# dfm/emcee

Hardware: AMD Instinct MI355X
Metric: walker-updates/sec (whole node), 64-dim correlated Gaussian, StretchMove a=2 (higher is better)
Workload: dtype f64

## Files before the change

emcee_amd/_lib.py:

```python
import ctypes as C
import os

import numpy as np

HERE = os.path.dirname(os.path.abspath(__file__))
LIB_PATH = os.path.join(HERE, "libemx.so")

TARGET_HOST, TARGET_ISO, TARGET_DIAG, TARGET_DENSE, TARGET_ROSENBROCK, TARGET_BOX, TARGET_CALLBACK = range(7)
TARGET_FUSED_USER = 8
TARGET_FUSED_PT = 9
TARGET_FUSED_ENSEMBLE = 10
MOVE_STRETCH, MOVE_DE, MOVE_SNOOKER, MOVE_GAUSS = range(4)
MOVE_WALK, MOVE_KDE = 5, 6
KDE_BW_SCOTT, KDE_BW_SILVERMAN, KDE_BW_SCALAR = range(3)
GAUSS_VECTOR, GAUSS_RANDOM, GAUSS_SEQUENTIAL = range(3)
RNG_INPUTS, RNG_MT19937, RNG_PHILOX = range(3)
EXCHANGE_ALLGATHER, EXCHANGE_PULL, EXCHANGE_DIRECT, EXCHANGE_LOGPROB, EXCHANGE_REPLAY = range(5)


class MoveDesc(C.Structure):
    _fields_ = [("kind", C.c_int32), ("nsplits", C.c_int32), ("randomize_split", C.c_int32), ("reserved", C.c_int32),
                ("a", C.c_double), ("sigma", C.c_double), ("g0", C.c_double), ("gammas", C.c_double)]


# ... 67 lines not shown
    "emx_snapshot_save": (C.c_int, [_P, C.c_int32]),
    "emx_snapshot_read": (C.c_int, [_P, C.c_int32, _P, _P]),
    "emx_snapshot_restore": (C.c_int, [_P, C.c_int32]),
    "emx_snapshot_free": (C.c_int, [_P, C.c_int32]),
    "emx_set_target": (C.c_int, [_P, C.c_int32, _P, _P, C.c_double]),
    "emx_set_target_callback": (C.c_int, [_P, DEVICE_LOG_PROB_FN, _P]),
    "emx_set_target_fused": (C.c_int, [_P, FUSED_ENSEMBLE_FN, _P]),
    "emx_set_target_fused_blobs": (C.c_int, [_P, FUSED_ENSEMBLE_BLOBS_FN, _P, C.c_int32]),
    "emx_set_target_fused_small": (C.c_int, [_P, FUSED_BATCH_FN]),
    "emx_set_target_fused_data": (C.c_int, [_P, FUSED_ENSEMBLE_DATA_FN, _P, C.c_int64]),
    "emx_small_fused_check": (C.c_int, [C.c_int64, C.c_int32, C.c_int32, C.POINTER(MoveDesc), C.c_int32, C.c_int32, C.c_char_p, C.c_int32]),
    "emx_small_fused_pays": (C.c_int, [C.c_int64, C.c_int32, C.c_int32]),
    "emx_small_info": (C.c_int, [_P, C.POINTER(C.c_int64)]),
    "emx_get_blobs": (C.c_int, [_P, _P, C.POINTER(C.c_int32)]),
    "emx_set_blobs": (C.c_int, [_P, _dp]),
    "emx_eval_log_prob_blobs": (C.c_int, [_P, _dp, C.c_int64, _dp, _dp]),
    "emx_snapshot_read_blobs": (C.c_int, [_P, C.c_int32, _dp]),
    "emx_eval_state_log_prob": (C.c_int, [_P]),
    "emx_eval_log_prob": (C.c_int, [_P, _dp, C.c_int64, _dp]),
    "emx_set_moves": (C.c_int, [_P, C.c_int32, C.POINTER(MoveDesc), _dp]),
    "emx_set_rng_mode": (C.c_int, [_P, C.c_int32]),
    "emx_rng_set_mt19937": (C.c_int, [_P, _u32p, C.c_int32, C.c_int32, C.c_double]),
    "emx_rng_get_mt19937": (C.c_int, [_P, _u32p, C.POINTER(C.c_int32), C.POINTER(C.c_int32), C.POINTER(C.c_double)]),
    "emx_rng_set_philox": (C.c_int, [_P, C.c_uint64, C.c_uint64]),
    "emx_rng_get_philox": (C.c_int, [_P, C.POINTER(C.c_uint64), C.POINTER(C.c_uint64)]),
    "emx_chain_config": (C.c_int, [_P, C.c_int64]),
    "emx_chain_reset": (C.c_int, [_P]),
    "emx_run": (C.c_int, [_P, C.c_int64, C.c_int32, C.c_int32]),
    "emx_iteration": (C.c_int, [_P, C.POINTER(C.c_int64), C.POINTER(C.c_int64)]),
    "emx_graph_state": (C.c_int, [_P, C.POINTER(C.c_int32), C.POINTER(C.c_int32)]),
    "emx_chain_read": (C.c_int, [_P, C.c_int32, C.c_int64, C.c_int64, C.c_int64, _dp]),
    "emx_accepted_counts": (C.c_int, [_P, _dp]),
    "emx_step_begin": (C.c_int, [_P, C.c_int32, C.POINTER(C.c_int32), C.POINTER(C.c_int32)]),
    "emx_step_begin_with": (C.c_int, [_P, C.c_int32, C.c_int32, C.POINTER(C.c_int32)]),
    "emx_accept_proposals": (C.c_int, [_P, C.c_int32, _dp, _dp, _dp]),
    "emx_halfstep": (C.c_int, [_P, C.c_int32]),
    "emx_propose": (C.c_int, [_P, C.c_int32, _P, _P, C.POINTER(C.c_int64)]),
    "emx_accept": (C.c_int, [_P, C.c_int32, _dp]),
    "emx_step_end": (C.c_int, [_P]),
    "emx_plan_set": (C.c_int, [_P, C.c_int32, _ip, _ip, _ip, _ip, _ip, _dp, _dp]),
    "emx_plan_get": (C.c_int, [_P, _ip, _ip, _ip, _ip, _ip, _dp, _dp]),
    "emx_set_shard": (C.c_int, [_P, C.c_int32, C.c_int32]),
    "emx_set_shard_buffers": (C.c_int, [_P, _P, _P, C.c_int64]),
    "emx_device_ptr": (C.c_int, [_P, C.c_int32, C.POINTER(_P), C.POINTER(C.c_int64)]),
    "emx_shard_slots": (C.c_int, [_P, C.c_int32, C.POINTER(C.c_int64), C.POINTER(C.c_int64), C.POINTER(C.c_int64)]),
    "emx_scatter_gathered": (C.c_int, [_P, C.c_int32]),
    "emx_set_move_scale": (C.c_int, [_P, C.c_int32, C.c_void_p, C.c_int32]),
    "emx_get_move": (C.c_int, [_P, C.c_int32, C.POINTER(MoveDesc)]),
    "emx_plan_set_noise": (C.c_int, [_P, _dp, C.c_double]),
    "emx_set_exchange": (C.c_int, [_P, C.c_int32]),
    "emx_exchange_layout": (C.c_int, [_P, C.POINTER(C.c_int64), C.POINTER(C.c_int64)]),
    "emx_set_exchange_buffers": (C.c_int, [_P, _P, C.c_int64, _P, C.c_int64]),
    "emx_own_walkers": (C.c_int, [_P, C.POINTER(C.c_int64), C.POINTER(C.c_int64)]),
    "emx_pull_prepare": (C.c_int, [_P, C.c_int32, C.POINTER(C.c_int64)]),
    "emx_pull_apply": (C.c_int, [_P, C.c_int32]),
    "emx_logprob_begin": (C.c_int, [_P, C.c_int32, C.POINTER(C.c_int64)]),
    "emx_logprob_finish": (C.c_int, [_P, C.c_int32]),
    "emx_replay_begin": (C.c_int, [_P, C.c_int32, C.POINTER(C.c_int64)]),
    "emx_replay_finish": (C.c_int, [_P, C.c_int32]),
    "emx_replay_exchange": (C.c_int, [_P, C.c_int32]),
    "emx_replica_pack": (C.c_int, [_P, C.POINTER(C.c_int64)]),
    "emx_replica_unpack": (C.c_int, [_P]),
    "emx_direct_export": (C.c_int, [_P, _u8p]),
    "emx_direct_import": (C.c_int, [_P, _u8p]),
    "emx_direct_attach": (C.c_int, [_P, C.POINTER(C.c_void_p), C.POINTER(C.c_void_p)]),
    "emx_direct_halfstep": (C.c_int, [_P, C.c_int32, C.c_int32]),
    "emx_fft_load": (C.c_int, [C.c_char_p]),
    "emx_autocorr": (C.c_int, [_P, C.c_int64, C.c_int64, C.c_double, _dp, _ip, C.POINTER(C.c_int64)]),
    "emx_walkers_independent": (C.c_int, [C.c_int32, _dp, C.c_int64, C.c_int32, C.POINTER(C.c_int32), C.POINTER(C.c_double)]),
    "emx_walkers_independent_resident": (C.c_int, [C.c_void_p, C.POINTER(C.c_int32), C.POINTER(C.c_double)]),
    "emx_host_pull_capacity": (C.c_int64, [C.c_int64, C.c_int32, C.c_int32, C.c_int32]),
    "emx_comm_load": (C.c_int, [C.c_char_p]),
    "emx_comm_get_unique_id": (C.c_int, [_u8p]),
    "emx_comm_init": (C.c_int, [_P, C.c_int32, C.c_int32, _u8p]),
    "emx_comm_destroy": (C.c_int, [_P]),
    "emx_comm_count": (C.c_int, [_P, C.POINTER(C.c_int32)]),
    "emx_pipeline_stats": (C.c_int, [_P, _dp, C.POINTER(C.c_int64), C.POINTER(C.c_int32)]),
    "emx_pipeline_handovers": (C.c_int, [_P, C.POINTER(C.c_int64), C.POINTER(C.c_int64)]),
    "emx_persist_info": (C.c_int, [_P, C.POINTER(C.c_int64)]),
    "emx_mtdev_info": (C.c_int, [_P, C.POINTER(C.c_int64)]),
    "emx_mtdev_debug": (C.c_int, [_P, C.c_int32, C.c_int64, C.c_void_p, C.c_int64]),
    "emx_mtdev_tok_stats": (C.c_int, [_P, C.POINTER(C.c_int64)]),
    "emx_persist_local_launches": (C.c_int, [_P, C.POINTER(C.c_int64)]),
    "emx_host_mt_jump": (C.c_int, [_u32p, C.c_uint64, C.c_int32, _u32p]),
    "emx_host_persist_shape": (C.c_int, [C.c_int64, C.c_int32, C.c_int32, C.POINTER(C.c_int32), C.POINTER(C.c_int32)]),
    "emx_timer_start": (C.c_int, [_P]),
    "emx_timer_stop": (C.c_int, [_P, C.POINTER(C.c_float)]),
    "emx_profile_enable": (C.c_int, [_P, C.c_int32]),
    "emx_profile_read": (C.c_int, [_P, _f32p, C.POINTER(C.c_int32)]),
    "emx_mt_create": (_P, [_u32p, C.c_int32, C.c_int32, C.c_double]),
    "emx_mt_destroy": (None, [_P]),
    "emx_mt_get_state": (None, [_P, _u32p, C.POINTER(C.c_int32), C.POINTER(C.c_int32), C.POINTER(C.c_double)]),
    "emx_mt_random_sample": (None, [_P, C.c_int64, _dp]),
    "emx_mt_randint": (None, [_P, C.c_uint64, C.c_int64, _i64p]),
    "emx_mt_randn": (None, [_P, C.c_int64, _dp]),
    "emx_mt_shuffle_labels": (None, [_P, C.c_int64, C.c_int32, _ip]),
    "emx_mt_choice_cdf": (C.c_int32, [_P, _dp, C.c_int32]),
    "emx_host_plan_mt": (C.c_int, [_P, C.c_int64, C.c_int32, C.POINTER(MoveDesc), _ip, _ip, _ip, _ip, _ip, _dp, _dp]),
    "emx_host_plan_mt_stream": (C.c_int, [_P, C.c_int64, C.c_int32, C.c_int32, C.POINTER(MoveDesc), _dp, C.c_int64, C.c_int32, C.c_int32,
                                          _P, _P, _P, _P, _P, _P, _P, C.POINTER(C.c_double)]),
    "emx_host_split_draws": (C.c_int, [_P, C.c_int64, C.POINTER(MoveDesc), _ip, _ip, C.c_int32, _ip, _ip, _ip, _dp]),
    "emx_host_plan_philox": (C.c_int, [C.c_uint64, C.c_uint64, C.c_int64, C.POINTER(MoveDesc), _ip, _ip, _ip, _ip, _ip, _dp, _dp]),
    "emx_host_walk_kde_draws": (C.c_int64, [C.c_uint64, C.c_uint64, C.c_int64, C.c_int32, C.POINTER(MoveDesc), C.c_int32, _P, _dp]),
    "emx_host_move_choice_philox": (C.c_int32, [C.c_uint64, C.c_uint64, _dp, C.c_int32]),
    "emx_batch_check": (C.c_int, [C.c_int64, C.c_int32, C.c_int32, C.c_int32, C.POINTER(MoveDesc), C.c_char_p, C.c_int32]),
    "emx_batch_create": (C.c_int, [C.c_int32, C.c_int32, C.c_int64, C.c_int32, C.POINTER(_P)]),
    "emx_batch_destroy": (C.c_int, [_P]),
    "emx_batch_last_error": (C.c_char_p, [_P]),
    "emx_batch_set_tuning": (C.c_int, [_P, C.c_char_p, C.c_int64]),
    "emx_batch_set_target": (C.c_int, [_P, C.c_int32, _P, _P, _P, C.c_int32]),
    "emx_batch_set_moves": (C.c_int, [_P, C.c_int32, C.POINTER(MoveDesc), _dp]),
    "emx_batch_set_move_scale": (C.c_int, [_P, C.c_int32, _dp, C.c_int32]),
    "emx_batch_get_move": (C.c_int, [_P, C.c_int32, C.POINTER(MoveDesc)]),
    "emx_batch_set_philox": (C.c_int, [_P, _u64p, C.c_uint64]),
    "emx_batch_get_philox": (C.c_int, [_P, _u64p, C.POINTER(C.c_uint64)]),
    "emx_batch_set_state": (C.c_int, [_P, _dp, _P]),
    "emx_batch_get_state": (C.c_int, [_P, _P, _P]),
    "emx_batch_eval_state_log_prob": (C.c_int, [_P]),
    "emx_batch_chain_config": (C.c_int, [_P, C.c_int64]),
    "emx_batch_run": (C.c_int, [_P, C.c_int64, C.c_int32, C.c_int32]),
    "emx_batch_iteration": (C.c_int, [_P, C.POINTER(C.c_int64), C.POINTER(C.c_int64)]),
    "emx_batch_chain_read": (C.c_int, [_P, C.c_int32, C.c_int32, C.c_int32, C.c_int64, C.c_int64, C.c_int64, _dp]),
    "emx_batch_accepted_counts": (C.c_int, [_P, _dp]),
    "emx_batch_status": (C.c_int, [_P, _u32p]),
    "emx_batch_launch_info": (C.c_int, [_P, C.POINTER(C.c_int32), C.POINTER(C.c_int32), C.POINTER(C.c_int64)]),
    "emx_set_batch_target_callback": (C.c_int, [_P, BATCH_LOG_PROB_FN, _P]),
    "emx_set_batch_target_fused": (C.c_int, [_P, FUSED_BATCH_FN, C.c_int32, _P]),
    "emx_pt_set_tempering": (C.c_int, [_P, C.c_int32, _dp, _P, _P]),
    "emx_set_batch_prior_callback": (C.c_int, [_P, BATCH_LOG_PROB_FN, _P]),
    "emx_pt_set_swap_every": (C.c_int, [_P, C.c_int64]),
    "emx_pt_swap": (C.c_int, [_P]),
    "emx_pt_swap_counts": (C.c_int, [_P, _u64p, _u64p]),
    "emx_pt_mean_loglike": (C.c_int, [_P, C.c_int64, C.c_int64, C.c_int64, _dp]),
    "emx_pt_set_state": (C.c_int, [_P, _dp, _dp, _dp]),
    "emx_pt_get_state": (C.c_int, [_P, _dp, _dp]),
    "emx_host_pt_swap_draws": (C.c_int, [C.c_uint64, C.c_uint64, C.c_int64, C.c_int32, _ip, _dp]),
    "emx_pt_set_adaptation": (C.c_int, [_P, C.c_int32, C.c_double, C.c_double]),
    "emx_pt_get_ladder": (C.c_int, [_P, _P, C.POINTER(C.c_int64)]),
    "emx_pt_set_ladder": (C.c_int, [_P, _dp, C.POINTER(C.c_int64)]),
    "emx_host_pt_adapt_ladder": (C.c_int, [_dp, _i64p, C.c_int32, C.c_int64, C.c_double, C.c_double, C.c_int64, _dp]),
    "emx_pt_set_target_fused": (C.c_int, [_P, PT_FUSED_FN, C.c_int32, _P]),
    "emx_pt_set_target_fused_data": (C.c_int, [_P, PT_FUSED_FN, C.c_int32, _P, _i64p]),
    "emx_pt_fused_check": (C.c_int, [C.c_int32, C.c_int64, C.c_int32, C.c_int32, C.POINTER(MoveDesc), C.c_char_p, C.c_int32]),
    "emx_autocorr_batch": (C.c_int, [_P, C.c_int32, C.c_int32, C.c_int64, C.c_int64, C.c_double, _dp, _ip, C.POINTER(C.c_int64)]),
    "emx_summary_batch": (C.c_int, [_P, C.c_int32, C.c_int32, C.c_int64, C.c_int64, C.c_int64, _P, _P, C.c_int32, _P, _P, _P, _P,
                                    C.POINTER(C.c_int64)]),
    "emx_summary": (C.c_int, [_P, C.c_int32, C.c_int64, C.c_int64, C.c_int64, _P, _P, C.c_int32, _P, _P, _P, _P, C.POINTER(C.c_int64)]),
    "emx_summary_info": (C.c_int, [_P, C.POINTER(C.c_int64), C.POINTER(C.c_int64), C.POINTER(C.c_int64)]),
    "emx_host_order_stats": (C.c_int, [_dp, C.c_int64, C.c_int64, C.c_int32, _i64p, _dp]),
    "emx_chain_minmax": (C.c_int, [_P, C.c_int32, C.c_int64, C.c_int64, C.c_int64, _P, _P, _P]),
    "emx_histograms": (C.c_int, [_P, C.c_int32, C.c_int64, C.c_int64, C.c_int64, _P, _P, _P, _P, _P, C.c_int64, _P, _P, _P,
                                 C.POINTER(C.c_int64)]),
    "emx_set_batch_target_fused_blobs": (C.c_int, [_P, FUSED_BATCH_FN, C.c_int32, _P, C.c_int32]),
    "emx_set_batch_target_fused_data": (C.c_int, [_P, FUSED_BATCH_DATA_FN, C.c_int32, _P, _i64p]),
    "emx_set_batch_target_callback_blobs": (C.c_int, [_P, BATCH_LOG_PROB_BLOBS_FN, _P, C.c_int32]),
    "emx_check_batch_blobs": (C.c_int, [C.c_int64, C.c_int32, C.c_int32, C.c_int32, C.POINTER(MoveDesc), C.c_int32, C.c_char_p, C.c_int32]),
    "emx_get_blobs_batch": (C.c_int, [_P, _P, C.POINTER(C.c_int32)]),
    "emx_summary_batch_plane": (C.c_int, [_P, C.c_int32, C.c_int32, C.c_int32, C.c_int64, C.c_int64, C.c_int64, _P, _P, C.c_int32, _P, _P,
                                          _P, _P, C.POINTER(C.c_int64)]),
    "emx_chain_minmax_batch": (C.c_int, [_P, C.c_int32, C.c_int32, C.c_int32, C.c_int64, C.c_int64, C.c_int64, _P, _P, _P]),
    "emx_histograms_batch": (C.c_int, [_P, C.c_int32, C.c_int32, C.c_int32, C.c_int64, C.c_int64, C.c_int64, _P, _P, C.c_int64, _P, _P, _P,
                                       C.c_int64, C.c_int64, _P, _P, _P, C.POINTER(C.c_int64)]),
    "emx_histograms_batch_info": (C.c_int, [_P, C.POINTER(C.c_int64)]),
    "emx_rhat_batch": (C.c_int, [_P, C.c_int32, C.c_int32, C.c_int32, C.c_int64, C.c_int64, C.c_int64, C.c_int32, _P, _P,
                                 C.POINTER(C.c_int64), C.POINTER(C.c_int64)]),
    "emx_rhat": (C.c_int, [_P, C.c_int64, C.c_int64, C.c_int64, C.c_int32, _P, _P, C.POINTER(C.c_int64), C.POINTER(C.c_int64)]),
# ... 42 lines not shown
```

emcee_amd/csrc/emx.hip:

```cpp
#include <hip/hip_runtime.h>

#include <dlfcn.h>

#include <algorithm>
#include <chrono>
#include <cmath>
#include <cstdint>
#include <cstdio>
#include <cstring>
#include <deque>
#include <mutex>
#include <string>
#include <type_traits>
#include <vector>

#include "../../include/emx.h"
#include "emx_fused_ensemble.hpp"
#include "emx_fused_ensemble_data.hpp"
#include "emx_internal.hpp"
#include "emx_kernels.hpp"
#include "emx_launch.hpp"
#include "emx_mtdev.hpp"
#include "emx_mtjump.hpp"
#include "emx_mtpipe.hpp"
// ... 255 lines not shown
    double* evalblobs = nullptr;
    double* blob_plane = nullptr;
    double* snap_blobs[NSNAPSHOT] = {};
    int snap_nb[NSNAPSHOT] = {};
    void* cb_user = nullptr;
    int target = EMX_TARGET_HOST;
    double *tp0 = nullptr, *tp1 = nullptr;
    double tscale = 1.0;
    int Dp = 0;
    std::vector<emx_move_desc> moves;
    std::vector<double> cdf;
    std::vector<double*> mscale;
    double* disp = nullptr;
    double* noise_host = nullptr;
    hipEvent_t noise_ev = nullptr;
    bool noise_busy = false;
    unsigned long long* dbg = nullptr;
    int64_t dbg_blocks = 0;
    struct BulkPlans {
        char* host = nullptr;
        char* dev = nullptr;
        size_t bytes = 0;
        hipEvent_t done = nullptr;
        bool busy = false;
    } bulk[2];
    int bulk_pos = 0;
    int64_t tune_small = 1;
    int64_t tune_gauss_materialize = 0;
    double gfac = 1.0;
    int rng_mode = EMX_RNG_PHILOX;
    MT19937Legacy mt;
    uint64_t ph_seed = 0, ph_step = 0;
    struct PlanSlot {
        int32_t *order = nullptr, *p0 = nullptr, *p1 = nullptr, *p2 = nullptr;
        double *s0 = nullptr, *uacc = nullptr, *logu = nullptr, *fac = nullptr;
        char* host = nullptr;
        hipEvent_t consumed = nullptr;
        hipEvent_t consumed_ref = nullptr;
        hipEvent_t uploaded = nullptr;
        hipEvent_t uploaded_ref = nullptr;
        unsigned last_seq = 0;
        int64_t fetch_step = -1;
        bool busy = false, host_written = false;
        int move_idx = 0;
        PipeStepInfo pinfo;
    } ring[PLAN_RING + MTDEV_SLOTS];
    MtPlanPipeline* pipe = nullptr;
    int64_t pipe_taken = 0;
    int pipe_ring0 = 0;
    int pipe_nsinks = PIPE_SINKS;
    std::deque<int64_t> pipe_uploads;
    bool pipe_defer = false;
    std::vector<std::pair<int64_t, int>> pipe_deferred;
    hipEvent_t pipe_batch_ev[8] = {};
    int pipe_batch_n = 0, pipe_cons_n = 0;
    unsigned long long* pipe_done = nullptr;
    unsigned* pipe_arrived = nullptr;
    hipStream_t up_stream = nullptr;
    int64_t tune_mt_device_finish = 1;
    int64_t tune_persist_exact_mix = 1;
    int64_t pipe_raw_steps = 0;
    int64_t tune_mt_pipeline = -1;
    MtDevProducer* mtdev = nullptr;
    int64_t mtdev_taken = 0;
    int64_t tune_persist_local = 1;
    int64_t tune_persist_exact_max = 32768;
    int64_t tune_persist_exact_regen_max = 131072;
    int64_t tune_persist_exact_steps = 16;
    int64_t tune_fetch_avoid = 1;
    int64_t tune_fetch_blocks = 64;
    bool pipe_fetch_local = false;
    int64_t tune_fetch_delay_us = 0;
    int64_t tune_persist_span = 1;
    int64_t tune_persist_mix = 1;
    int persist_mix_fits = -1;
    int64_t tune_persist_slab = 1;
    int64_t persist_slab_launches = 0;
    int64_t tune_persist_rows_late = 1;
    int64_t tune_persist_stagger = -1;
    int64_t tune_persist_max_halfsteps = PERSIST_MAX_ITERS;
    int64_t tune_mt_device_min_regen = 786432;
    int64_t tune_mt_regen_min = 16384;
    int64_t pipe_regen_steps = 0;
    int64_t tune_persist_odd = 1;
    int64_t tune_persist_slab_skew = 1;
    int64_t tune_persist_slab_local_max = 4096;
    int64_t call_steps = 1;
    int64_t tune_persist_exact = 1;
    int64_t tune_persist_valu = 1;
    int64_t tune_persist_local_max = 8192;
    int64_t tune_slab = 1;
    int64_t tune_slab_skew = 1;
    int64_t tune_mt_device = 1;
    int64_t tune_mt_device_min = 147456;
    int64_t tune_mt_lookahead = 2;
    int64_t tune_mt_tok_wshift = 11, tune_mt_tok_tail = 2048;
    int64_t mtdev_steps_total = 0, mtdev_starts = 0;
    bool mtdev_defer_release = false;
    int64_t mtdev_release_pending = -1;
    MtDevStats mtdev_stats_last;
    int ring_pos = 0;
    struct Prepared {
        int move, S, slot;
        bool lean;
        int gcol;
        uint64_t step;
        NativeArgs nat;
        double cursor_before;
    };
    std::deque<Prepared> prepared;
    int64_t prep_hint = 1;
    std::vector<uint8_t> labels_scratch;
    struct Cur {
        bool active = false;
        int move = 0, S = 2, slot = 0;
        bool store = false;
        bool native = false;
        bool lean = false;
        bool devplan = false;
        int gcol = 0;
        std::vector<int32_t> off;
        NativeArgs nat{};
    } cur;
    double *chain = nullptr, *chain_lp = nullptr;
    int64_t cap = 0, stored = 0, proposals = 0;
    EnsSummary* summary = nullptr;
    RhatScratch* rhat = nullptr;
    int64_t tune_summary_compact = 1;
    int64_t tune_hist_chunk_rows = 0;
    double *qout = nullptr, *fout = nullptr, *newlp = nullptr;
    double* tp1_full = nullptr;
    double *evalX = nullptr, *evallp = nullptr;
    double* wk_work = nullptr;
    int rank = 0, world = 1;
    double *sendbuf = nullptr, *gathered = nullptr;
    int64_t sendbuf_rows = 0, gathered_rows = 0;
    bool own_shard_bufs = false;
    void* comm = nullptr;
    int64_t send_doubles = 0, recv_doubles = 0;
    int exchange = EMX_EXCHANGE_ALLGATHER;
    PlanSlot cplan;
    int64_t cplan_rows = 0;
    int32_t* pull_counts = nullptr;
    int pull_parity = 0;
    int64_t pull_cap_armed = 0;
    double* pull_armed_buf = nullptr;
    int64_t pull_cap_cur = 0;
    int pull_split = -1;
    double* peerX[EMX_MAX_PEERS] = {};
    unsigned long long* peer_flags[EMX_MAX_PEERS] = {};
    bool peer_ipc_x[EMX_MAX_PEERS] = {}, peer_ipc_f[EMX_MAX_PEERS] = {};
    unsigned long long* my_flags = nullptr;
    bool peers_ready = false;
    PeerTable* peer_table = nullptr;
    unsigned long long direct_epoch = 0;
    int32_t* direct_counts = nullptr;
    bool direct_planned = false;
    int64_t tune_direct_timeout_ms = 5000;
    int32_t* replay_counts = nullptr;
    int replay_parity = 0;
    int replay_split = -1;
    int64_t replay_recv_off = 0;
    int64_t replay_buf = 0;
    int replay_push_parity = 0;
    double* launch_declp = nullptr;
    bool launch_push = false;
    bool replay_pushed = false;
    int64_t launch_push_off = 0;
    bool eval_check_bad = false;
    bool direct_dead = false;
    bool direct_first_barrier = false;
    struct GraphSlot {
        hipGraph_t graph = nullptr;
        hipGraphExec_t exec = nullptr;
        bool valid = false;
        int64_t spw = -1, wpb = -1, bpc = -1;
        int target = -1;
    } gslot[2];
    StepDesc* d_desc = nullptr;
    GraphCounters* d_ctr = nullptr;
    GraphCounters* h_ctr = nullptr;
    hipEvent_t thr_ev[4] = {nullptr, nullptr, nullptr, nullptr};
    int64_t tune_throttle = 64;
    bool graph_disabled = false;
    bool graph_warm = false;
    int64_t tune_graph = 0;
    int64_t tune_persist_gauss_wpb = 0;
    int64_t tune_persist_test_skew = 0;
    int64_t tune_persist = 1, tune_persist_timeout_ms = 2000, tune_persist_min_walkers = 512;
    int persist_wpb = 8;
    int64_t persist_launches = 0, persist_halfsteps = 0;
    struct PersistCapture {
        HalfStepArgs a;
        dim3 grid, block;
        size_t lds;
        int move, dpb, lean;
        bool dense, got;
    };
    PersistCapture* persist_cap = nullptr;
    unsigned* persist_bar = nullptr;
    unsigned* persist_started = nullptr;
    unsigned persist_lepoch = 0;
    unsigned persist_hepoch = 0;
    int64_t persist_local_launches = 0;
    unsigned* persist_ver = nullptr;
    unsigned persist_epoch = 0;
    unsigned persist_grid = 0;
    struct PersistLog {
        unsigned seq;
        uint64_t ph_step;
        int64_t i0, steps, stored0, proposals0;
        int32_t thin_by, store;
        int64_t pipe_step0 = -1;
        const void* pipe_id = nullptr;
    };
    std::deque<PersistLog> plog;
    unsigned persist_seq = 0;
    int64_t persist_recovered = 0;
    int8_t persist_fits[4] = {-1, -1, -1, -1};
    int64_t tune_replay_two_pass = 0;
    int64_t tune_full_plan = 0;
    int64_t tune_spw = 0, tune_bpc = 2, tune_wpb = 0, tune_ablate = 0, tune_dense_wide = 0;
    hipEvent_t ev0 = nullptr, ev1 = nullptr;
    std::vector<hipEvent_t> prof;
    int prof_max = 0, prof_n = 0;
    std::string err;
    emx_fused_ensemble_data_fn fused_data_fn = nullptr;
    int64_t fused_ndata = 0;
    int64_t tune_fused_data_rows = 0;
};

static void graph_invalidate(emx_ctx* c);
static void apply_env_tuning(emx_ctx* c);
static int pipe_stop(emx_ctx* c);
#define PIPE_STOP(ctx)                        \
    do {                                      \
        const int _rps = pipe_stop(ctx);      \
        if (_rps) return _rps;                \
    } while (0)
static void direct_detach(emx_ctx* c);
static int direct_ensure(emx_ctx* c);
static void exchange_free(emx_ctx* c);
static int replay_ensure(emx_ctx* c);
static int flags_ensure(emx_ctx* c);
static int persist_settle(emx_ctx* c);
static hipError_t wait_stream(hipStream_t s);

static void drop_prepared(emx_ctx* c) {
    for (auto it = c->prepared.rbegin(); it != c->prepared.rend(); ++it)
        if (it->move < (int)c->moves.size() && c->moves[it->move].kind == EMX_MOVE_GAUSS) c->moves[it->move].gammas = it->cursor_before;
    c->prepared.clear();
}

#define FAIL(ctx, code, ...)                         \
    do {                                             \
        char _b[512];                                \
        snprintf(_b, sizeof(_b), __VA_ARGS__);       \
        if (ctx) (ctx)->err = _b; else g_err = _b;   \
        return (code);                               \
    } while (0)

#define HIPOK(ctx, expr)                                                                          \
    do {                                                                                          \
        hipError_t _e = (expr);                                                                   \
        if (_e != hipSuccess) FAIL(ctx, -2, "%s failed: %s (%s:%d)", #expr, hipGetErrorString(_e), __FILE__, __LINE__); \
    } while (0)

#define NEED(ctx, cond, ...)               \
    do {                                   \
        if (!(cond)) FAIL(ctx, -1, __VA_ARGS__); \
    } while (0)

namespace {

int prefetch_depth_host(int G, int V, int CH, int move, bool dense);

inline int lean_kind(const HalfStepArgs& a, int G, int V, int CH, int move, bool dense) {
    const int WPW = 64 / G, PF = prefetch_depth_host(G, V, CH, move, dense);
    const int spw = (dense && PF * WPW < 16) ? 16 : PF * WPW;
    const bool common = !a.ablate && !a.desc && !a.sendbuf && !a.disp && !a.skew_sleep && (EMX_OPT_STAMPS || !a.dbg) && (a.target != TGT_NONE || !dense) &&
                        (!EMX_LEAN_FOLD_D || a.D == G * V * CH) && a.spw == spw && a.t_lo == 0;
    if (!common) return 0;
    if (a.npeer) return a.declp ? 0 : 2;
    if (a.declp) return 4;
    return a.t_hi_dev ? 3 : 1;
}

template <int MOVE>
hipError_t launch_valu(const Shape& sh, dim3 grid, dim3 block, hipStream_t st, const HalfStepArgs& a) {
    if constexpr (MOVE == MOVE_STRETCH) {
        if (sh.G == 8 && sh.V == 2 && sh.CH == 2) {
            const int lk = lean_kind(a, 8, 2, 2, MOVE, false);
            if (lk == 1) return launch_one<8, 2, 2, MOVE, 0, 1>(grid, block, 0, st, a);
            if (lk == 2 || lk == 3) return launch_one<8, 2, 2, MOVE, 0, 2>(grid, block, 0, st, a);
            if (lk == 4) return launch_one<8, 2, 2, MOVE, 0, 4>(grid, block, 0, st, a);
        }
        if (sh.G == 8 && sh.V == 2 && sh.CH == 4) {
            const int lk = lean_kind(a, 8, 2, 4, MOVE, false);
            if (lk == 2 || lk == 3) return launch_one<8, 2, 4, MOVE, 0, 2>(grid, block, 0, st, a);
        }
        if (sh.G == 64 && sh.V == 2 && sh.CH == 8) {
            const int lk = lean_kind(a, 64, 2, 8, MOVE, false);
            if (lk == 1) return launch_one<64, 2, 8, MOVE, 0, 1>(grid, block, 0, st, a);
            if (lk == 2 || lk == 3) return launch_one<64, 2, 8, MOVE, 0, 2>(grid, block, 0, st, a);
            if (lk == 4) return launch_one<64, 2, 8, MOVE, 0, 4>(grid, block, 0, st, a);
        }
    }
    if constexpr (MOVE != MOVE_EVAL) {
#define EMX_LEAN_CASE(g, v, c)                                                                         \
    if (sh.G == g && sh.V == v && sh.CH == c && lean_kind(a, g, v, c, MOVE, false) == 1)                \
        return launch_one<g, v, c, MOVE, 0, 1>(grid, block, 0, st, a);
        EMX_LEAN_CASE(4, 1, 1) EMX_LEAN_CASE(8, 1, 1) EMX_LEAN_CASE(8, 1, 2) EMX_LEAN_CASE(8, 1, 4) EMX_LEAN_CASE(16, 1, 4)
        EMX_LEAN_CASE(32, 1, 4) EMX_LEAN_CASE(64, 1, 4) EMX_LEAN_CASE(64, 1, 8) EMX_LEAN_CASE(4, 2, 1) EMX_LEAN_CASE(8, 2, 1)
        EMX_LEAN_CASE(8, 2, 4) EMX_LEAN_CASE(16, 2, 4) EMX_LEAN_CASE(32, 2, 4) EMX_LEAN_CASE(64, 2, 4)
        if constexpr (MOVE == MOVE_STRETCH || MOVE == MOVE_GAUSS) {
            EMX_LEAN_CASE(64, 1, 16) EMX_LEAN_CASE(64, 2, 16)
        }
        if constexpr (MOVE != MOVE_STRETCH) {
            EMX_LEAN_CASE(8, 2, 2) EMX_LEAN_CASE(64, 2, 8)
        }
#undef EMX_LEAN_CASE
    }
#define EMX_CASE(g, v, c) \
    if (sh.G == g && sh.V == v && sh.CH == c) return launch_one<g, v, c, MOVE, 0>(grid, block, 0, st, a);
    EMX_CASE(4, 1, 1) EMX_CASE(8, 1, 1) EMX_CASE(8, 1, 2) EMX_CASE(8, 1, 4) EMX_CASE(16, 1, 4) EMX_CASE(32, 1, 4)
    EMX_CASE(64, 1, 4) EMX_CASE(64, 1, 8)
    EMX_CASE(4, 2, 1) EMX_CASE(8, 2, 1) EMX_CASE(8, 2, 2) EMX_CASE(8, 2, 4) EMX_CASE(16, 2, 4) EMX_CASE(32, 2, 4)
    EMX_CASE(64, 2, 4) EMX_CASE(64, 2, 8)
    if constexpr (MOVE == MOVE_STRETCH || MOVE == MOVE_EVAL || MOVE == MOVE_GAUSS) {
        EMX_CASE(64, 1, 16) EMX_CASE(64, 2, 16)
    }
#undef EMX_CASE
    return hipErrorInvalidValue;
}
// ... 663 lines not shown
    c->cdf.assign(1, 1.0);
    apply_env_tuning(c);
    *out = c;
    return 0;
}

static void apply_env_tuning(emx_ctx* c) {
    const char* e = getenv("EMX_TUNE");
    if (!e || !*e) return;
    std::string s(e);
    size_t pos = 0;
    while (pos < s.size()) {
        size_t end = s.find(',', pos);
        if (end == std::string::npos) end = s.size();
        const std::string kv = s.substr(pos, end - pos);
        const size_t eq = kv.find('=');
        if (eq != std::string::npos) emx_set_tuning(c, kv.substr(0, eq).c_str(), atoll(kv.c_str() + eq + 1));
        pos = end + 1;
    }
}

int emx_destroy(emx_ctx* c) {
    if (!c) return 0;
    pipe_stop(c);
    c->plog.clear();
    hipSetDevice(c->device);
    if (c->stream) hipStreamSynchronize(c->stream);
    if (c->comm && g_rccl.CommDestroy) g_rccl.CommDestroy(c->comm), c->comm = nullptr;
    if (c->status_host) hipHostFree(c->status_host);
    if (c->xfer_host) hipHostFree(c->xfer_host);
    for (int k = 0; k < 2; ++k) {
        if (c->bounce[k]) hipHostFree(c->bounce[k]);
        if (c->bounce_ev[k]) hipEventDestroy(c->bounce_ev[k]);
    }
    void* ptrs[] = {c->X, c->lp, c->acc, c->acc_count, c->iota, c->qout, c->fout, c->newlp, c->evalX, c->wk_work,
                    c->evallp, c->tp0, c->tp1, c->tp1_full, c->chain, c->chain_lp, c->own_shard_bufs ? c->sendbuf : nullptr,
                    c->own_shard_bufs ? c->gathered : nullptr};
    for (void* p : ptrs)
        if (p) hipFree(p);
    for (double* s : c->snap)
        if (s) hipFree(s);
    for (double* s : c->snap_blobs)
        if (s) hipFree(s);
    for (double* s : {c->blobs, c->evalblobs, c->blob_plane})
        if (s) hipFree(s);
    emx_internal_ens_summary_release(c->summary);
    emx_internal_rhat_release(c->rhat);

    for (auto& s : c->ring) {
        if (s.order) hipFree(s.order);
        if (s.host) hipHostFree(s.host);
        if (s.uploaded) hipEventDestroy(s.uploaded);
        s.uploaded_ref = nullptr;
        if (s.consumed) hipEventDestroy(s.consumed);
    }
    for (auto& e : c->pipe_batch_ev)
        if (e) hipEventDestroy(e);
    if (c->pipe_done) hipHostFree(c->pipe_done);
    if (c->pipe_arrived) hipFree(c->pipe_arrived);
    for (auto& g : c->gslot) {
        if (g.exec) hipGraphExecDestroy(g.exec);
        if (g.graph) hipGraphDestroy(g.graph);
    }
    {
        auto& p = c->cplan;
        void* q[] = {p.order, p.p0, p.p1, p.p2, p.s0, p.uacc, p.logu, p.fac, c->pull_counts, c->replay_counts};
        for (void* x : q)
            if (x) hipFree(x);
    }
    for (double* q : c->mscale)
        if (q) hipFree(q);
    for (auto& bp : c->bulk) {
        if (bp.host) hipHostFree(bp.host);
        if (bp.dev) hipFree(bp.dev);
        if (bp.done) hipEventDestroy(bp.done);
    }
    if (c->disp) hipFree(c->disp);
    if (c->dbg) hipFree(c->dbg);
    if (c->noise_host) hipHostFree(c->noise_host);
    if (c->noise_ev) hipEventDestroy(c->noise_ev);
    if (c->persist_bar) hipFree(c->persist_bar);
    if (c->persist_started) hipHostFree(c->persist_started);
    if (c->persist_ver) hipFree(c->persist_ver);
    if (c->d_desc) hipFree(c->d_desc);
    if (c->d_ctr) hipFree(c->d_ctr);
    if (c->h_ctr) hipHostFree(c->h_ctr);
    for (auto e : c->thr_ev)
        if (e) hipEventDestroy(e);
    if (c->ev0) hipEventDestroy(c->ev0);
    if (c->ev1) hipEventDestroy(c->ev1);
    for (auto e : c->prof) hipEventDestroy(e);
    direct_detach(c);
    if (c->my_flags) hipFree(c->my_flags);
    if (c->peer_table) hipFree(c->peer_table);
    if (c->direct_counts) hipFree(c->direct_counts);
    if (c->up_stream) hipStreamDestroy(c->up_stream);
    if (c->own_stream) hipStreamDestroy(c->own_stream);
    delete c;
    return 0;
}

int emx_set_stream(emx_ctx* c, void* s) {
    NEED(c, c, "null ctx");
    HIPOK(c, hipStreamSynchronize(c->stream));
    c->stream = s ? (hipStream_t)s : c->own_stream;
    return 0;
}

static const bool g_spin_sync = !(getenv("EMX_SPIN_SYNC") && atoi(getenv("EMX_SPIN_SYNC")) == 0);

static hipError_t wait_stream(hipStream_t s) {
    if (g_spin_sync) {
        const auto t0 = std::chrono::steady_clock::now();
        for (int it = 0;; ++it) {
            const hipError_t e = hipStreamQuery(s);
            if (e != hipErrorNotReady) return e;
            if ((it & 63) == 63 && std::chrono::steady_clock::now() - t0 > std::chrono::milliseconds(2)) break;
        }
    }
    return hipStreamSynchronize(s);
}

static hipError_t wait_event(hipEvent_t ev) {
    if (g_spin_sync) {
        const auto t0 = std::chrono::steady_clock::now();
        for (int it = 0;; ++it) {
            const hipError_t e = hipEventQuery(ev);
            if (e != hipErrorNotReady) return e;
            if ((it & 63) == 63 && std::chrono::steady_clock::now() - t0 > std::chrono::milliseconds(2)) break;
        }
    }
    return hipEventSynchronize(ev);
}

int emx_sync(emx_ctx* c) {
    HIPOK(c, hipSetDevice(c->device));
    HIPOK(c, wait_stream(c->stream));
    return persist_settle(c);
}

int emx_status(emx_ctx* c, uint32_t* bits) {
    HIPOK(c, wait_stream(c->stream));
    {
        const int rcs = persist_settle(c);
        if (rcs) return rcs;
    }
    uint32_t b = 0;
    for (int k = 0; k < 6; ++k)
        if (__atomic_exchange_n(&c->status_host[k], 0u, __ATOMIC_ACQ_REL)) b |= 1u << k;
    if (b & ST_EXCHANGE_TIMEOUT) c->direct_dead = true;
    if (b & ST_EXCHANGE_TIMEOUT) c->persist_grid = 0;
    *bits = b;
    return 0;
}

int emx_set_tuning(emx_ctx* c, const char* key, int64_t v) {
    if (!strcmp(key, "spw")) {
        c->tune_spw = v;
        return 0;
    }
    if (!strcmp(key, "phase_clock")) {
        if (v && !c->dbg) {
            c->dbg_blocks = 4096;
            HIPOK(c, hipMalloc((void**)&c->dbg, (size_t)c->dbg_blocks * 16 * 8));
            HIPOK(c, hipMemset(c->dbg, 0, (size_t)c->dbg_blocks * 16 * 8));
        }
// ... 42 lines not shown
    if (!strcmp(key, "waves_per_block")) {
        c->tune_wpb = (v == 1 || v == 2 || v == 4 || v == 8) ? v : 0;
        return 0;
    }
    if (!strcmp(key, "dense_wide")) {
        c->tune_dense_wide = v == 2 ? 2 : (v ? 1 : 0);
        graph_invalidate(c);
        return 0;
    }
    if (!strcmp(key, "mt_device")) {
        PIPE_STOP(c);
        c->tune_mt_device = v < 0 ? 0 : (v > 2 ? 2 : v);
        return 0;
    }
    if (!strcmp(key, "mt_device_min_walkers")) {
        PIPE_STOP(c);
        c->tune_mt_device_min = v < 8192 ? 8192 : v;
        return 0;
    }
    if (!strcmp(key, "mt_tok_wshift") || !strcmp(key, "mt_tok_tail")) {
        PIPE_STOP(c);
        (key[7] == 'w' ? c->tune_mt_tok_wshift : c->tune_mt_tok_tail) = v;
        return 0;
    }
    if (!strcmp(key, "mt_device_lookahead")) {
        c->tune_mt_lookahead = v < 0 ? 0 : (v > 2 ? 2 : v);
        return 0;
    }
    if (!strcmp(key, "slab")) {
        c->tune_slab = v < 0 ? 0 : (v > 2 ? 2 : v);
        return 0;
    }
    if (!strcmp(key, "persist_exact_mix")) {
        PIPE_STOP(c);
        c->tune_persist_exact_mix = v ? 1 : 0;
        return 0;
    }
    if (!strcmp(key, "mt_device_finish")) {
        PIPE_STOP(c);
        c->tune_mt_device_finish = v ? 1 : 0;
        return 0;
    }
    if (!strcmp(key, "slab_skew")) {
        c->tune_slab_skew = v < 0 ? 0 : (v > 4 ? 4 : v);
        return 0;
    }
    if (!strcmp(key, "persist")) {
        c->tune_persist = v ? 1 : 0;
        return 0;
    }
    if (!strcmp(key, "persist_slab_skew")) {
        c->tune_persist_slab_skew = v < 0 ? 0 : (v > 4 ? 4 : v);
        return 0;
    }
    if (!strcmp(key, "persist_slab_local_max_walkers")) {
        c->tune_persist_slab_local_max = v;
        return 0;
    }
    if (!strcmp(key, "summary_compact")) {
        c->tune_summary_compact = v < 0 ? 0 : (v > 2 ? 2 : v);
        return 0;
    }
    if (!strcmp(key, "hist_chunk_rows")) {
        c->tune_hist_chunk_rows = v < 0 ? 0 : v;
        return 0;
    }
    if (!strcmp(key, "persist_odd")) {
        c->tune_persist_odd = v ? 1 : 0;
        return 0;
    }
    if (!strcmp(key, "persist_exact_regen_max_walkers")) {
        PIPE_STOP(c);
        c->tune_persist_exact_regen_max = v;
        return 0;
    }
    if (!strcmp(key, "mt_device_min_walkers_regen")) {
        PIPE_STOP(c);
        c->tune_mt_device_min_regen = v;
        return 0;
    }
    if (!strcmp(key, "mt_regen_min_walkers")) {
        PIPE_STOP(c);
        c->tune_mt_regen_min = v < 0 ? 0 : v;
        return 0;
    }
    if (!strcmp(key, "persist_rows_late")) {
        c->tune_persist_rows_late = v < 0 ? 0 : v > 2 ? 2 : v;
        return 0;
    }
    if (!strcmp(key, "persist_stagger")) {
        c->tune_persist_stagger = v < 0 ? -1 : v > 1279 ? 1279 : v;
        return 0;
    }
    if (!strcmp(key, "persist_max_halfsteps")) {
        c->tune_persist_max_halfsteps = v;
        return 0;
    }
    if (!strcmp(key, "persist_slab")) {
        c->tune_persist_slab = (v == 1 || v == 2) ? v : 0;
        return 0;
    }
    if (!strcmp(key, "persist_local")) {
        c->tune_persist_local = v ? 1 : 0;
        return 0;
    }
    if (!strcmp(key, "persist_exact")) {
        PIPE_STOP(c);
        c->tune_persist_exact = v ? 1 : 0;
        return 0;
    }
    if (!strcmp(key, "persist_exact_max_walkers")) {
        PIPE_STOP(c);
        c->tune_persist_exact_max = v;
        return 0;
    }
    if (!strcmp(key, "persist_exact_steps")) {
        c->tune_persist_exact_steps = std::max<int64_t>(1, std::min<int64_t>(v, 16));
        return 0;
    }
    if (!strcmp(key, "fetch_blocks")) {
        c->tune_fetch_blocks = std::max<int64_t>(0, std::min<int64_t>(v, 65536));
        return 0;
    }
    if (!strcmp(key, "fetch_avoid")) {
        c->tune_fetch_avoid = v ? 1 : 0;
        return 0;
    }
    if (!strcmp(key, "test_fetch_delay_us")) {
        c->tune_fetch_delay_us = std::max<int64_t>(0, std::min<int64_t>(v, 100000));
        return 0;
    }
    if (!strcmp(key, "persist_span")) {
        c->tune_persist_span = v ? 1 : 0;
        return 0;
    }
    if (!strcmp(key, "persist_mix")) {
        c->tune_persist_mix = v ? 1 : 0;
        return 0;
    }
    if (!strcmp(key, "persist_valu")) {
        c->tune_persist_valu = v ? 1 : 0;
        return 0;
    }
    if (!strcmp(key, "persist_local_max_walkers")) {
        c->tune_persist_local_max = v;
        return 0;
    }
    if (!strcmp(key, "persist_gauss_wpb")) {
        c->tune_persist_gauss_wpb = (v == 1 || v == 2 || v == 4 || v == 8) ? v : 0;
        return 0;
    }
    if (!strcmp(key, "persist_test_skew")) {
        c->tune_persist_test_skew = v;
        return 0;
    }
    if (!strcmp(key, "persist_timeout_ms")) {
        c->tune_persist_timeout_ms = v > 0 ? v : 2000;
        return 0;
    }
    if (!strcmp(key, "persist_min_walkers")) {
        c->tune_persist_min_walkers = v > 0 ? v : 2;
        return 0;
    }
    if (!strcmp(key, "replay_two_pass")) {
        c->tune_replay_two_pass = v ? 1 : 0;
        return 0;
// ... 991 lines not shown
    bool any_raw = false;
    int max_nseg = 0;
    F.N = (int32_t)c->N;
    F.D = c->D;
    F.n = (int)c->pipe_deferred.size();
    hipEvent_t waited = nullptr;
    for (int k = 0; k < F.n; ++k) {
        auto& s = c->ring[c->pipe_deferred[k].second];
        bool by_event = s.busy && s.consumed_ref != waited;
        if (s.busy && s.last_seq != 0u && c->persist_started && (int)(c->persist_seq - s.last_seq) > 0) {
            const double w0 = tr_now();
            const double limit = 2e6 * (double)std::max<int64_t>(1, c->tune_persist_timeout_ms);
            while ((int)(__atomic_load_n(c->persist_started, __ATOMIC_ACQUIRE) - s.last_seq) <= 0 && tr_now() - w0 < limit) {}
            if ((int)(__atomic_load_n(c->persist_started, __ATOMIC_ACQUIRE) - s.last_seq) > 0) by_event = false;
        }
        if (by_event) {
            HIPOK(c, hipStreamWaitEvent(c->up_stream, s.consumed_ref, 0));
            waited = s.consumed_ref;
        }
        F.host[k] = s.host;
        F.dev[k] = (char*)s.order;
        F.stretch[k] = c->moves[(size_t)std::max(0, s.move_idx)].kind == EMX_MOVE_STRETCH;
        F.peers[k] = !(F.stretch[k] && c->world == 1);
        const PipeStepInfo& pi = s.pinfo;
        F.kind[k] = pi.regen ? 2 : (pi.raw ? 1 : 0);
        F.nkey[k] = pi.regen ? pi.regen_nseg * 624 : 0;
        if (pi.raw) {
            any_raw = true;
            PlanRawArgs& R = RB.st[k];
            R.dev = (char*)s.order;
            R.a = c->moves[(size_t)std::max(0, s.move_idx)].a;
            R.N = (int32_t)c->N;
            R.D = c->D;
            R.S = pi.S;
            R.wr_words = pi.wr_ring;
            R.wr_p1 = pi.regen ? 1 : 0;
            for (int q = 0; q <= pi.S && q <= PLAN_RAW_SPLITS; ++q) R.off[q] = pi.off[q];
            c->pipe_raw_steps++;
        }
        if (pi.regen) {
            PlanRegenArgs& G = GB.st[k];
            G.dev = (char*)s.order;
            G.N = (int32_t)c->N;
            G.ns0 = pi.off[1] - pi.off[0];
            G.off = pi.regen_off;
            G.nseg = pi.regen_nseg;
            max_nseg = std::max(max_nseg, pi.regen_nseg);
            c->pipe_regen_steps++;
        }
    }
    F.delay_ticks = (unsigned)(c->tune_fetch_delay_us * 100);
    F.arrived = c->pipe_arrived;
    F.avoid_xcc = (c->persist_bar && c->tune_fetch_avoid) ? c->persist_bar + 9 * PERSIST_BAR_STRIDE + 4 : nullptr;
    F.host_done = c->pipe_done;
    F.done_value = (unsigned long long)(c->pipe_deferred.back().first + 1);
    F.pieces_x = (int32_t)((c->N + 255) / 256);
    unsigned nwg = (unsigned)F.pieces_x * (unsigned)F.n;
    if (!c->pipe_fetch_local && c->tune_fetch_blocks > 0) nwg = std::min<unsigned>(nwg, (unsigned)c->tune_fetch_blocks);
    hipLaunchKernelGGL(k_plan_fetch, dim3(nwg), dim3(256), 0, c->up_stream, F);
    if (max_nseg > 0) hipLaunchKernelGGL(k_plan_regen_batch, dim3((unsigned)max_nseg, (unsigned)F.n), dim3(256), 0, c->up_stream, GB);
    if (any_raw) hipLaunchKernelGGL(k_plan_raw_batch, dim3((unsigned)F.pieces_x, (unsigned)F.n), dim3(256), 0, c->up_stream, RB);
    HIPOK(c, hipGetLastError());
    hipEvent_t& ev = c->pipe_batch_ev[c->pipe_batch_n & 3];
    if (!ev) HIPOK(c, hipEventCreateWithFlags(&ev, hipEventDisableTiming));
    c->pipe_batch_n++;
    HIPOK(c, hipEventRecord(ev, c->up_stream));
    HIPOK(c, hipStreamWaitEvent(c->stream, ev, 0));
    for (auto& d : c->pipe_deferred) {
        c->ring[d.second].uploaded_ref = ev;
    }
    c->pipe_deferred.clear();
    return 0;
}

int emx_step_begin(emx_ctx* c, int32_t store, int32_t* move_out, int32_t* S_out) {
    return step_begin_impl(c, store, -1, move_out, S_out);
}

int emx_step_begin_with(emx_ctx* c, int32_t store, int32_t move_index, int32_t* S_out) {
    NEED(c, move_index >= 0 && move_index < (int)c->moves.size(), "bad move index");
    return step_begin_impl(c, store, move_index, nullptr, S_out);
}

static int native_prepare_batch(emx_ctx* c, uint64_t first_step, int nb, int forced_move, hipStream_t st) {
    const int nm = (int)c->moves.size();
    NativeBatchArgs B{};
    B.N = (int32_t)c->N;
    B.D = c->D;
    B.nb = nb;
    B.lean = (c->target != EMX_TARGET_HOST && c->world == 1 && !c->sendbuf && !c->comm && !c->tune_full_plan) ? 1 : 0;
    B.ablate = (int32_t)(c->tune_ablate >> 8);
    bool only_stretch = true;
    for (int b = 0; b < nb; ++b) {
        const uint64_t step = first_step + (uint64_t)b;
        const int mi = forced_move >= 0 ? forced_move : philox_move_choice(c->ph_seed, step, c->cdf.data(), nm);
        const emx_move_desc& m = c->moves[mi];
        only_stretch = only_stretch && m.kind == EMX_MOVE_STRETCH;
        emx_ctx::PlanSlot* ps;
        int rc = acquire_slot(c, &ps, false);
        if (rc) return rc;
        emx_ctx::Prepared pr{};
        pr.move = mi;
        pr.S = m.nsplits;
        pr.slot = c->ring_pos;
        pr.step = step;
        pr.nat.seed = c->ph_seed;
        pr.nat.step = step;
        pr.nat.pk = make_perm_key((uint64_t)c->N, c->ph_seed, step);
        pr.cursor_before = m.gammas;
        pr.lean = B.lean != 0;
        if (m.kind == EMX_MOVE_GAUSS) {
            B.gmode[b] = m.reserved;
            B.gcol[b] = (int32_t)((int64_t)m.gammas % c->D);
            pr.gcol = B.gcol[b];
            if (m.reserved == EMX_GAUSS_SEQUENTIAL) c->moves[mi].gammas = (double)(((int64_t)m.gammas + 1) % c->D);
        }
        c->prepared.push_back(pr);
        B.nat[b] = pr.nat;
        B.order[b] = ps->order;
        B.p0[b] = ps->p0;
        B.p1[b] = ps->p1;
        B.p2[b] = ps->p2;
        B.s0[b] = ps->s0;
        B.uacc[b] = ps->uacc;
        B.logu[b] = ps->logu;
        B.fac[b] = ps->fac;
        B.a[b] = m.a;
        B.sigma[b] = m.sigma;
        B.g0[b] = m.g0;
        B.move[b] = m.kind;
        B.S[b] = m.nsplits;
    }
    if (only_stretch && B.lean && !B.ablate && !B.desc)
        hipLaunchKernelGGL(k_native_plan_batch_stretch, dim3((unsigned)((c->N + 255) / 256), (unsigned)nb), dim3(256), 0, st, B);
    else
        hipLaunchKernelGGL(k_native_plan_batch, dim3((unsigned)((c->N + 255) / 256), (unsigned)nb), dim3(256), 0, st, B);
    HIPOK(c, hipGetLastError());
    return 0;
}

static int step_begin_impl(emx_ctx* c, int32_t store, int32_t forced_move, int32_t* move_out, int32_t* S_out) {
    HIPOK(c, hipSetDevice(c->device));
    NEED(c, !c->cur.active, "emx_step_begin: previous step not ended");
    if (store) NEED(c, c->stored < c->cap, "chain capacity exhausted (call emx_chain_config)");
    auto& cur = c->cur;
    cur.store = store != 0;
    cur.native = false;
    cur.devplan = false;
    const int nm = (int)c->moves.size();
    const bool devp = forced_move < 0 && mtdev_eligible(c);
    if (c->mtdev && !devp) {
        const int rcm = mtdev_stop(c);
        if (rcm) return rcm;
    }
    if (c->pipe && (devp || forced_move >= 0 || !pipe_eligible(c))) PIPE_STOP(c);
    if (devp) {
        if (!c->mtdev) {
            int rc0 = mtdev_start(c);
            if (rc0) return rc0;
        }
        int rc = mtdev_take(c);
        if (rc) return rc;
    } else if (c->rng_mode == EMX_RNG_MT19937 && forced_move < 0 && (c->pipe || ((c->N >= 8192 || persist_exact_ok(c)) && pipe_eligible(c)))) {
        if (!c->pipe) {
            int rc0 = pipe_start(c);
            if (rc0) return rc0;
        }
        int rc = pipe_take(c);
        if (rc) return rc;
    } else if (c->rng_mode == EMX_RNG_MT19937) {
        cur.move = forced_move >= 0 ? forced_move : c->mt.choice_cdf(c->cdf.data(), nm);
        const emx_move_desc& mv = c->moves[cur.move];
        NEED(c, !is_walk_kde(mv.kind), "WalkMove / KDEMove steps run on the device in the Philox rng mode only");
        cur.S = mv.nsplits;
        NEED(c, c->N >= 2 && (mv.kind != EMX_MOVE_DE || c->N - (c->N + cur.S - 1) / cur.S >= 2),
             "complement too small for this move");
        emx_ctx::PlanSlot* ps;
        int rc = acquire_slot(c, &ps, true);
        if (rc) return rc;
        cur.slot = c->ring_pos;
        cur.off.assign(cur.S + 1, 0);
        const size_t N = (size_t)c->N;
        const HostPlan hp(ps->host, N);
        if (mv.kind == EMX_MOVE_GAUSS) {
            if (!c->noise_host) {
                HIPOK(c, hipHostMalloc((void**)&c->noise_host, N * (size_t)c->D * 8, hipHostMallocDefault));
                HIPOK(c, hipEventCreateWithFlags(&c->noise_ev, hipEventDisableTiming));
            }
            if (c->noise_busy) {
                HIPOK(c, hipEventSynchronize(c->noise_ev));
                c->noise_busy = false;
            }
            const double f = make_exact_gauss(c->mt, c->N, c->D, mv, c->moves[cur.move].gammas, cur.off.data(), hp.order, hp.p0,
                                              hp.p1, hp.p2, hp.s0, hp.uacc, c->noise_host);
            rc = upload_plan(c, *ps);
            if (rc) return rc;
            rc = gauss_upload_normals(c, cur.move, c->noise_host, f, true);
            if (rc) return rc;
        } else {
            rc = make_exact_plan(c->mt, c->N, c->D, mv, c->labels_scratch, cur.off.data(), hp.order, hp.p0, hp.p1, hp.p2, hp.s0,
                                 hp.uacc);
            NEED(c, rc == 0, "plan generation failed");
            rc = upload_plan(c, *ps);
            if (rc) return rc;
        }
    } else if (c->rng_mode == EMX_RNG_PHILOX) {
        if (forced_move >= 0) drop_prepared(c);
        if (!c->prepared.empty() && c->prepared.front().step != c->ph_step) drop_prepared(c);
        if (c->prepared.empty()) {
            int64_t nbw = forced_move >= 0 ? 1 : c->prep_hint;
            const int nb = (int)std::max<int64_t>(1, std::min<int64_t>(nbw, NATIVE_BATCH_MAX));
            const int rc = native_prepare_batch(c, c->ph_step, nb, forced_move, c->stream);
            if (rc) return rc;
        }
        const emx_ctx::Prepared pr = c->prepared.front();
        c->prepared.pop_front();
        cur.move = pr.move;
        cur.S = pr.S;
        cur.native = true;
        cur.lean = pr.lean;
        cur.gcol = pr.gcol;
        cur.nat = pr.nat;
        cur.slot = pr.slot;
        cur.off.assign(cur.S + 1, 0);
        for (int s = 0; s < cur.S; ++s) cur.off[s + 1] = cur.off[s] + (int32_t)((c->N - s + cur.S - 1) / cur.S);
        if (c->moves[cur.move].kind == EMX_MOVE_GAUSS) {
            int rc = gauss_native_disp(c, cur.move, pr.step, c->ring[pr.slot].p0);
            if (rc) return rc;
        }
    } else {
        cur.move = -1;
        cur.S = 0;
        cur.slot = -1;
    }
    cur.active = true;
    if (move_out) *move_out = cur.move;
    if (S_out) *S_out = cur.S;
    return 0;
}

static int complete_lean_plan(emx_ctx* c) {
    auto& cur = c->cur;
    if (!cur.active || !cur.native || !cur.lean) return 0;
    NEED(c, cur.move >= 0 && cur.slot >= 0, "no plan available");
    auto& ps = c->ring[cur.slot];
    const emx_move_desc& m = c->moves[cur.move];
    NativeBatchArgs B{};
    B.N = (int32_t)c->N;
    B.D = c->D;
    B.nb = 1;
    B.lean = 0;
    B.nat[0] = cur.nat;
    B.order[0] = ps.order;
    B.p0[0] = ps.p0;
    B.p1[0] = ps.p1;
    B.p2[0] = ps.p2;
    B.s0[0] = ps.s0;
    B.uacc[0] = ps.uacc;
    B.logu[0] = ps.logu;
    B.fac[0] = ps.fac;
    B.a[0] = m.a;
    B.sigma[0] = m.sigma;
    B.g0[0] = m.g0;
    B.move[0] = m.kind;
    B.S[0] = m.nsplits;
    if (m.kind == EMX_MOVE_GAUSS) {
        B.gmode[0] = m.reserved;
        B.gcol[0] = cur.gcol;
    }
    hipLaunchKernelGGL(k_native_plan_batch, dim3((unsigned)((c->N + 255) / 256), 1u), dim3(256), 0, c->stream, B);
    HIPOK(c, hipGetLastError());
    cur.lean = false;
    return 0;
}

int emx_plan_set(emx_ctx* c, int32_t move_index, const int32_t* off, const int32_t* order, const int32_t* p0,
                 const int32_t* p1, const int32_t* p2, const double* s0, const double* uacc) {
    NEED(c, c->cur.active, "emx_plan_set outside a step");
    NEED(c, move_index >= 0 && move_index < (int)c->moves.size(), "bad move index");
    NEED(c, !is_walk_kde(c->moves[move_index].kind), "WalkMove / KDEMove steps run on the device in the Philox rng mode only");
    auto& cur = c->cur;
    cur.move = move_index;
    cur.S = c->moves[move_index].nsplits;
    cur.native = false;
    cur.off.assign(off, off + cur.S + 1);
    NEED(c, cur.off[0] == 0 && cur.off[cur.S] == c->N, "plan offsets must cover all walkers");
    emx_ctx::PlanSlot* ps;
    int rc = acquire_slot(c, &ps, true);
    if (rc) return rc;
    cur.slot = c->ring_pos;
    const size_t N = (size_t)c->N;
    const HostPlan hp(ps->host, N);
    memcpy(hp.order, order, N * 4);
    memcpy(hp.p0, p0, N * 4);
    memcpy(hp.p1, p1 ? p1 : order, N * 4);
    memcpy(hp.p2, p2 ? p2 : order, N * 4);
    if (s0) memcpy(hp.s0, s0, N * 8); else memset(hp.s0, 0, N * 8);
    memcpy(hp.uacc, uacc, N * 8);
    return upload_plan(c, *ps);
}

int emx_plan_get(emx_ctx* c, int32_t* off, int32_t* order, int32_t* p0, int32_t* p1, int32_t* p2, double* s0,
                 double* uacc) {
    NEED(c, c->cur.active, "emx_plan_get outside a step");
    auto& cur = c->cur;
    const size_t N = (size_t)c->N;
    memcpy(off, cur.off.data(), (cur.S + 1) * 4);
    if (cur.native) {
        NEED(c, cur.slot >= 0, "no plan available");
        auto& ps = c->ring[cur.slot];
        {
            const int rcl = complete_lean_plan(c);
            if (rcl) return rcl;
        }
        HIPOK(c, hipMemcpyAsync(order, ps.order, N * 4, hipMemcpyDeviceToHost, c->stream));
        HIPOK(c, hipMemcpyAsync(p0, ps.p0, N * 4, hipMemcpyDeviceToHost, c->stream));
        HIPOK(c, hipMemcpyAsync(p1, ps.p1, N * 4, hipMemcpyDeviceToHost, c->stream));
        HIPOK(c, hipMemcpyAsync(p2, ps.p2, N * 4, hipMemcpyDeviceToHost, c->stream));
        HIPOK(c, hipMemcpyAsync(s0, ps.s0, N * 8, hipMemcpyDeviceToHost, c->stream));
        HIPOK(c, hipMemcpyAsync(uacc, ps.uacc, N * 8, hipMemcpyDeviceToHost, c->stream));
        HIPOK(c, hipStreamSynchronize(c->stream));
        return 0;
    }
    NEED(c, cur.slot >= 0, "no plan available");
    auto& ps = c->ring[cur.slot];
    if (cur.devplan) {
        HIPOK(c, hipMemcpyAsync(order, ps.order, N * 4, hipMemcpyDeviceToHost, c->stream));
        HIPOK(c, hipMemcpyAsync(p0, ps.p0, N * 4, hipMemcpyDeviceToHost, c->stream));
        HIPOK(c, hipMemcpyAsync(s0, ps.s0, N * 8, hipMemcpyDeviceToHost, c->stream));
        HIPOK(c, hipMemcpyAsync(uacc, ps.uacc, N * 8, hipMemcpyDeviceToHost, c->stream));
        HIPOK(c, hipStreamSynchronize(c->stream));
        memcpy(p1, order, N * 4);
        memcpy(p2, order, N * 4);
        return 0;
    }
    const HostPlan hp(ps.host, N);
    memcpy(order, hp.order, N * 4);
    memcpy(p0, hp.p0, N * 4);
    if (cur.move >= 0 && c->moves[cur.move].kind == EMX_MOVE_STRETCH) {
        memcpy(p1, hp.order, N * 4);
        memcpy(p2, hp.order, N * 4);
    } else {
        memcpy(p1, hp.p1, N * 4);
        memcpy(p2, hp.p2, N * 4);
    }
    memcpy(s0, hp.s0, N * 8);
    memcpy(uacc, hp.uacc, N * 8);
    return 0;
}

int emx_plan_set_noise(emx_ctx* c, const double* normals, double factor) {
    HIPOK(c, hipSetDevice(c->device));
    auto& cur = c->cur;
    NEED(c, cur.active && cur.move >= 0 && c->moves[cur.move].kind == EMX_MOVE_GAUSS,
         "emx_plan_set_noise follows emx_plan_set of a Gaussian move");
// ... 606 lines not shown
    if (persist_local_ok(c, m)) return true;
    if (c->target != EMX_TARGET_DENSE_GAUSS) return persist_valu_wide_ok(c, m);
    const int wpb = persist_shape(c, m.nsplits);
    return wpb != 0 && persist_grid_fits(c, m, wpb);
}

static bool persist_mix_member(const emx_move_desc& m) {
    return (m.kind == EMX_MOVE_DE && m.nsplits == 2) || (m.kind == EMX_MOVE_SNOOKER && m.nsplits == 4);
}
static bool persist_mix_local(const emx_ctx* c) {
    for (const auto& m : c->moves)
        if (persist_mix_member(m) && !persist_local_ok(c, m)) return false;
    return persist_shape_local_of(c->N, 2, c->num_cu) != 0;
}
static bool persist_mix_ok(const emx_ctx* cc) {
    emx_ctx* c = const_cast<emx_ctx*>(cc);
    if (!c->tune_persist_mix || c->target != EMX_TARGET_DENSE_GAUSS || c->Dp > 64 || (c->D & 1)) return false;
    if (c->rng_mode != EMX_RNG_PHILOX && !(c->rng_mode == EMX_RNG_MT19937 && persist_exact_ok(c))) return false;
    bool de = false, sn = false;
    for (const auto& m : c->moves) {
        if (!persist_mix_member(m)) continue;
        if (!persist_move_ok(c, m)) return false;
        de = de || m.kind == EMX_MOVE_DE;
        sn = sn || m.kind == EMX_MOVE_SNOOKER;
    }
    if (!de || !sn || (c->N % 64) != 0) return false;
    if (persist_mix_local(c)) return true;
    const int wpb = persist_shape(c, 2);
    if (wpb == 0) return false;
    if (c->persist_mix_fits < 0) {
        int per_cu = 0;
        const hipError_t e = persist_mix_occupancy(c->Dp / 16, 64 * wpb, dense_lds_bytes(c->Dp, wpb), &per_cu);
        c->persist_mix_fits = (e != hipSuccess || (int64_t)per_cu * c->num_cu >= c->N / 2 / 16 / wpb) ? 1 : 0;
    }
    return c->persist_mix_fits != 0;
}

static bool persist_exact_ok(const emx_ctx* c) {
    if (small_eligible(c) && c->call_steps < 4) return false;
    {
        const bool dense = c->target == EMX_TARGET_DENSE_GAUSS && (c->Dp <= 64 || persist_slab_ok(c)) && !dense_is_wide(c);
        bool valu = c->target == EMX_TARGET_ISO_GAUSS || c->target == EMX_TARGET_DIAG_GAUSS || c->target == EMX_TARGET_ROSENBROCK || c->target == EMX_TARGET_BOX;
        if (valu) {
            const Shape sh = pick_shape(c->D, c->D);
            valu = persist_valu_shape(sh);
        }
        if (!dense && !valu) return false;
    }
    if (!(c->rng_mode == EMX_RNG_MT19937 && c->tune_persist_exact != 0 && !c->moves.empty() && c->tune_mt_pipeline != 0 &&
          c->N >= c->tune_persist_min_walkers && !mtdev_eligible(c) &&
          MtPlanPipeline::supports((int32_t)c->moves.size(), c->moves.data())))
        return false;
    if (c->moves.size() > 1 && !c->tune_persist_exact_mix) return false;
    for (const auto& m : c->moves) {
        const bool known = ((m.kind == EMX_MOVE_STRETCH || m.kind == EMX_MOVE_DE) && m.nsplits == 2) || (m.kind == EMX_MOVE_SNOOKER && m.nsplits == 4);
        if (!known && c->moves.size() > 1) return false;
        if (persist_local_ok(c, m)) continue;
        const int64_t nmax = (regen_ctx_ok(c) && m.kind == EMX_MOVE_STRETCH) ? std::max(c->tune_persist_exact_max, c->tune_persist_exact_regen_max) : c->tune_persist_exact_max;
        if (c->N > nmax || persist_shape(c, m.nsplits) == 0) return false;
        if (!(c->target == EMX_TARGET_DENSE_GAUSS || persist_valu_wide_ok(c, m))) return false;
    }
    return true;
}

static bool persist_wanted(const emx_ctx* c) {
    if (!c->tune_persist) return false;
    if (!(c->rng_mode == EMX_RNG_PHILOX || persist_exact_ok(c)) || c->world != 1 || c->comm || c->sendbuf || c->peers_ready || c->moves.empty()) return false;
    if (c->target != EMX_TARGET_DENSE_GAUSS || dense_is_wide(c) || (c->Dp > 64 && !persist_slab_ok(c))) return false;
    if (c->tune_ablate || (c->dbg && !EMX_OPT_STAMPS) || c->tune_spw || c->tune_wpb || c->tune_graph) return false;
    if (c->N < c->tune_persist_min_walkers) return false;
    bool any = false;
    for (const auto& m : c->moves) {
        if (is_walk_kde(m.kind)) return false;
        any = any || persist_move_ok(c, m);
    }
    if (!any) return false;
    if (c->Dp > 64) return true;
    const Shape sh = pick_shape(c->D, c->Dp);
    const int dpb = c->Dp / 16;
    if (sh.V == 1) return c->tune_persist_odd != 0 && (dpb <= 2 ? (sh.G == 8 && sh.CH == 2 * dpb) : (sh.G == 16 && sh.CH == 4));
    return sh.G == 8 && sh.V == 2 && sh.CH == (dpb == 1 ? 1 : dpb == 2 ? 2 : 4);
}

static bool persist_valu_wanted(const emx_ctx* c) {
    if (!c->tune_persist || !c->tune_persist_local || !c->tune_persist_valu) return false;
    if (!(c->rng_mode == EMX_RNG_PHILOX || persist_exact_ok(c)) || c->world != 1 || c->comm || c->sendbuf || c->peers_ready || c->moves.empty()) return false;
    if (c->target != EMX_TARGET_ISO_GAUSS && c->target != EMX_TARGET_DIAG_GAUSS && c->target != EMX_TARGET_ROSENBROCK && c->target != EMX_TARGET_BOX)
        return false;
    if (c->tune_ablate || c->dbg || c->tune_spw || c->tune_wpb || c->tune_graph) return false;
    if (c->N < c->tune_persist_min_walkers) return false;
    const Shape sh = pick_shape(c->D, c->D);
    if (!persist_valu_shape(sh)) return false;
    bool any = false;
    for (const auto& m : c->moves) {
        if (is_walk_kde(m.kind)) return false;
        any = any || persist_local_ok(c, m) || persist_valu_wide_ok(c, m);
    }
    return any;
}

static bool persist_gauss_wanted(const emx_ctx* c) {
    if (!c->tune_persist || c->tune_gauss_materialize) return false;
    if (c->rng_mode != EMX_RNG_PHILOX || c->world != 1 || c->comm || c->sendbuf || c->peers_ready || c->moves.size() != 1) return false;
    if (c->moves[0].kind != EMX_MOVE_GAUSS) return false;
    if (c->target != EMX_TARGET_DENSE_GAUSS || c->Dp > 64 || dense_is_wide(c)) return false;
    if (c->tune_ablate || c->dbg || c->tune_spw || c->tune_wpb || c->tune_graph) return false;
    if (c->N < c->tune_persist_min_walkers || (c->N % 16) != 0) return false;
    const Shape sh = pick_shape(c->D, c->Dp);
    const int dpb = c->Dp / 16;
    return sh.G == 8 && sh.V == 2 && sh.CH == (dpb == 1 ? 1 : dpb == 2 ? 2 : 4);
}

static int run_persist_gauss(emx_ctx* c, int64_t i0, int64_t total, int32_t thin_by, int32_t store, int64_t* done) {
    *done = 0;
    const int64_t tiles = c->N / 16;
    int wpb = c->tune_persist_gauss_wpb > 0 ? (int)c->tune_persist_gauss_wpb : 4;
    while (wpb > 1 && (tiles % wpb) != 0) wpb >>= 1;
    c->persist_wpb = wpb;
    PersistGaussArgs P{};
    emx_ctx::PersistCapture cap{};
    int64_t steps = 0;
    while (i0 + steps < total && steps < PERSIST_GAUSS_MAX_STEPS) {
        if (steps > 0 && c->prepared.empty()) break;
        c->prep_hint = NATIVE_BATCH_MAX;
        const int st = store && ((i0 + steps + 1) % thin_by == 0);
        int mvi, S;
        int rc = emx_step_begin(c, st, &mvi, &S);
        if (rc) return rc;
        cap.got = false;
        c->persist_cap = &cap;
        rc = do_halfstep(c, 0, c->target);
        c->persist_cap = nullptr;
        if (!rc && (S != 1 || !cap.dense || cap.move != MOVE_GAUSS || cap.a.disp || cap.dpb != c->Dp / 16)) {
            c->err = "persistent Gaussian steps: launch shape not eligible";
            rc = -1;
        }
        if (rc) {
            c->cur.active = false;
            return rc;
        }
        if (steps == 0) P.base = cap.a;
        PersistGaussStep& G = P.st[steps];
        G.p0 = cap.a.p0;
        G.logu = cap.a.logu;
        G.chain = cap.a.chain;
        G.chain_lp = cap.a.chain_lp;
        G.gstep = cap.a.gstep;
        G.gfac = cap.a.gfac;
        rc = emx_step_end(c);
        if (rc) return rc;
        ++steps;
    }
    P.nsteps = (int32_t)steps;
    const dim3 grid((unsigned)(tiles / wpb)), block(64u * (unsigned)wpb);
    const size_t lds = dense_lds_bytes(c->Dp, wpb);
    hipEvent_t e0 = nullptr, e1 = nullptr;
    const bool prof = c->prof_max > 0 && c->prof_n < c->prof_max;
    if (prof) {
        e0 = c->prof[2 * c->prof_n];
        e1 = c->prof[2 * c->prof_n + 1];
        HIPOK(c, hipEventRecord(e0, c->stream));
    }
    const hipError_t e = launch_hot_persist_gauss(c->Dp / 16, grid, block, lds, c->stream, P);
    if (e != hipSuccess) FAIL(c, -2, "persistent Gaussian launch failed: %s", hipGetErrorString(e));
    if (prof) {
        HIPOK(c, hipEventRecord(e1, c->stream));
        c->prof_n++;
    }
    c->persist_launches++;
    c->persist_halfsteps += steps;
    *done = steps;
    return 0;
}

static std::mutex g_persist_mu;
static hipEvent_t g_persist_ev[MAX_DEVICES] = {};
static const emx_ctx* g_persist_last[MAX_DEVICES] = {};

static int run_persist(emx_ctx* c, int64_t i0, int64_t total, int32_t thin_by, int32_t store, int64_t* done) {
    *done = 0;
    if (__atomic_load_n(&c->status_host[3], __ATOMIC_ACQUIRE)) {
        const int rcs = persist_settle(c);
        if (rcs) return rcs;
        if (__atomic_load_n(&c->status_host[3], __ATOMIC_ACQUIRE)) {
            c->persist_grid = 0;
            FAIL(c, -8, "persistent kernel: a device-wide barrier timed out in the middle of a launch; read emx_status, "
                        "or turn the persistent path off with tuning \"persist\" = 0");
        }
        return 0;
    }
    if (c->plog.size() >= 4096) {
        if (hipStreamQuery(c->stream) == hipSuccess && !__atomic_load_n(&c->status_host[3], __ATOMIC_ACQUIRE)) {
            c->plog.clear();
        } else if (c->plog.size() >= 65536) {
            const int rcs = persist_settle(c);
            if (rcs) return rcs;
        }
    }
    if (!c->persist_bar) {
        HIPOK(c, hipMalloc((void**)&c->persist_bar, PERSIST_BAR_WORDS * sizeof(unsigned)));
        HIPOK(c, hipHostMalloc((void**)&c->persist_started, 64, hipHostMallocDefault));
        *c->persist_started = 0u;
        HIPOK(c, hipMemsetAsync(c->persist_bar, 0, PERSIST_BAR_WORDS * sizeof(unsigned), c->stream));
        c->persist_epoch = 0;
    }
    if (!c->persist_ver) {
        HIPOK(c, hipMalloc((void**)&c->persist_ver, (size_t)c->N * 4));
        HIPOK(c, hipMemsetAsync(c->persist_ver, 0, (size_t)c->N * 4, c->stream));
    }
    PersistArgs P{};
    emx_ctx::PersistCapture cap{};
    dim3 grid, block;
    size_t lds = 0;
    int n = 0;
    int64_t steps = 0;
    const bool mtmode = c->rng_mode == EMX_RNG_MT19937;
    const bool devp = mtmode && mtdev_eligible(c);
    std::vector<int> used_slots;
    c->pipe_defer = mtmode && !devp;
    struct Undefer2 {
        emx_ctx* c;
        ~Undefer2() { c->pipe_defer = false; }
    } undefer2{c};
    c->mtdev_defer_release = devp;
    c->mtdev_release_pending = -1;
    struct Undefer {
        emx_ctx* c;
        ~Undefer() { c->mtdev_defer_release = false; }
    } undefer{c};
    emx_ctx::PersistLog lg{};
    lg.ph_step = c->ph_step;
    lg.i0 = i0;
    lg.stored0 = c->stored;
    lg.proposals0 = c->proposals;
    lg.thin_by = thin_by;
    lg.store = store;
    if (mtmode && !devp) {
        lg.pipe_step0 = c->pipe ? c->pipe_taken : 0;
        lg.pipe_id = c->pipe;
    }
    int launch_move = -1;
    int launch_S = 2;
    bool launch_local = false;
    bool launch_mix = false;
    double launch_gammas = 0.0;
    int batches_touched = (!mtmode && !c->prepared.empty() && c->prepared.front().step == c->ph_step) ? 1 : 0;
    while (i0 + steps < total) {
        if (!mtmode && (c->prepared.empty() || c->prepared.front().step != c->ph_step)) {
            if (batches_touched >= 2) break;
            ++batches_touched;
        }
        int next_move = -1;
        if (steps > 0 && !mtmode)
            next_move = !c->prepared.empty() ? c->prepared.front().move : philox_move_choice(c->ph_seed, c->ph_step, c->cdf.data(), (int)c->moves.size());
        if (steps > 0 && mtmode && !devp && c->moves.size() > 1) {
            PipeStepInfo peek;
            if (!c->pipe || !c->pipe->wait_ready(c->pipe_taken, peek, pipe_poll, c))
                FAIL(c, -7, "exact-mode plan pipeline stopped before step %lld", (long long)c->pipe_taken);
            next_move = peek.move;
        }
        int need = launch_S;
        if (launch_mix && next_move >= 0) need = c->moves[next_move].nsplits;
        if (n + need > (int)std::min<int64_t>(PERSIST_MAX_ITERS, std::max<int64_t>(4, c->tune_persist_max_halfsteps))) break;
        if (devp) {
            if (steps > 0 && c->mtdev && c->mtdev_taken % MTDEV_BATCH == 0) break;
        } else if (mtmode) {
            if (steps >= std::min<int64_t>(c->tune_persist_exact_steps, c->pipe_nsinks / 2)) break;
            if (steps > 0 && next_move >= 0) {
                if (!launch_mix && c->moves[next_move].kind != launch_move) break;
                if (!launch_mix && launch_move == EMX_MOVE_SNOOKER && c->moves[next_move].gammas != launch_gammas) break;
                if (launch_mix && !persist_mix_member(c->moves[next_move])) break;
                if (!persist_move_ok(c, c->moves[next_move])) break;
            }
        } else {
            if (steps > 0 && c->prepared.empty() && !c->tune_persist_span) break;
            if (steps > 0 && !launch_mix && c->moves[next_move].kind != launch_move) break;
            if (steps > 0 && !launch_mix && launch_move == EMX_MOVE_SNOOKER && c->moves[next_move].gammas != launch_gammas) break;
            if (steps > 0 && launch_mix && !persist_mix_member(c->moves[next_move])) break;
            if (steps > 0 && !persist_move_ok(c, c->moves[next_move])) break;
        }
        c->prep_hint = NATIVE_BATCH_MAX;
        const int st = store && ((i0 + steps + 1) % thin_by == 0);
        int mvi, S;
        int rc = emx_step_begin(c, st, &mvi, &S);
        if (rc) return rc;
        if (launch_move < 0) {
            launch_move = c->moves[mvi].kind;
            launch_gammas = c->moves[mvi].gammas;
            launch_S = S;
            launch_local = persist_local_ok(c, c->moves[mvi]);
            c->persist_wpb = launch_local ? persist_shape_local_of(c->N, S, c->num_cu) : persist_shape(c, S);
            if (persist_mix_ok(c) && (launch_move == EMX_MOVE_DE || launch_move == EMX_MOVE_SNOOKER)) {
                launch_mix = true;
                launch_local = persist_mix_local(c);
                c->persist_wpb = launch_local ? persist_shape_local_of(c->N, 2, c->num_cu) : persist_shape(c, 2);
            }
        }
        for (int s = 0; s < S; ++s) {
            cap.got = false;
            c->persist_cap = &cap;
            rc = do_halfstep(c, s, c->target);
            c->persist_cap = nullptr;
            const bool valu = c->target != EMX_TARGET_DENSE_GAUSS;
            const bool move_ok = launch_mix ? (cap.move == MOVE_DE || cap.move == MOVE_SNOOKER) : cap.move == launch_move;
            if (!rc && (!cap.got || cap.dense == valu || (!valu && cap.dpb != c->Dp / 16) || !move_ok ||
                        (int)cap.block.x != 64 * c->persist_wpb || (valu && !launch_local && !persist_valu_wide_ok(c, c->moves[mvi])))) {
                c->err = "persistent half-steps: launch shape not eligible";
                rc = -1;
            }
            if (rc) {
                c->cur.active = false;
                return rc;
            }
            if (n == 0) {
                P.base = cap.a;
                grid = cap.grid;
                block = cap.block;
                lds = cap.lds;
            }
            PersistIter& I = P.it[n++];
            {
                const char* blk = reinterpret_cast<const char*>(cap.a.order);
                const size_t NN = (size_t)c->N;
                NEED(c, (const void*)cap.a.p0 == (const void*)(blk + NN * 4) && (const void*)cap.a.s0 == (const void*)(blk + NN * 8) &&
                            (const void*)cap.a.p1 == (const void*)(blk + NN * 24) && (const void*)cap.a.p2 == (const void*)(blk + NN * 28) &&
                            (const void*)cap.a.logu == (const void*)(blk + NN * 32) && (const void*)cap.a.fac == (const void*)(blk + NN * 40),
                     "persistent half-steps: the plan slot is not one block in the expected layout");
                I.plan = blk;
            }
            I.chain = cap.a.chain;
            I.chain_lp = cap.a.chain_lp;
            I.pos0 = cap.a.pos0;
            I.split = cap.a.split;
            I.kind = cap.move;
            I.gammas = cap.a.gammas;
            I.shift = (launch_mix && S == 4) ? 1 : 0;
        }
        if (mtmode && !devp && c->cur.slot >= 0) used_slots.push_back(c->cur.slot);
        rc = emx_step_end(c);
        if (rc) return rc;
        ++steps;
    }
    if (mtmode && !devp) {
        c->pipe_fetch_local = launch_local;
        const int rcf = pipe_fetch_deferred(c);
        if (rcf) return rcf;
    }
    c->pipe_defer = false;
    if (launch_mix) grid = dim3((unsigned)(c->N / 2 / 16 / c->persist_wpb));
    if (launch_local) grid.x *= 8;
    if (grid.x != c->persist_grid) {
        HIPOK(c, hipMemsetAsync(c->persist_bar, 0, PERSIST_BAR_WORDS * sizeof(unsigned), c->stream));
        c->persist_epoch = 0;
        c->persist_lepoch = 0;
        c->persist_hepoch = 0;
        c->persist_grid = grid.x;
    }
    P.niter = n;
    P.bar = c->persist_bar;
    P.started_host = c->persist_started;
    P.ver = c->persist_ver;
    P.epoch0 = c->persist_epoch + (unsigned)c->tune_persist_test_skew;
    P.lepoch0 = c->persist_lepoch;
    P.hepoch0 = c->persist_hepoch + (unsigned)c->tune_persist_test_skew;
    if (launch_local) {
        c->persist_lepoch += (unsigned)(n - 1);
        c->persist_hepoch += 1u;
    }
    P.timeout_ticks = 100000000ull * (unsigned long long)std::max<int64_t>(1, c->tune_persist_timeout_ms) / 1000ull;
    const bool fam_dense64 = c->target == EMX_TARGET_DENSE_GAUSS && c->Dp <= 64;
    P.stagger = c->tune_persist_stagger >= 0 ? (int32_t)c->tune_persist_stagger
                : (launch_local || store || !fam_dense64) ? 0
                : (launch_mix || launch_move == EMX_MOVE_DE) ? 528
                : launch_move == EMX_MOVE_STRETCH ? 516 : 0;
    c->persist_epoch += (unsigned)n;
    P.seq = ++c->persist_seq;
    lg.seq = P.seq;
    lg.steps = steps;
    if (!mtmode || (!devp && lg.pipe_id != nullptr)) c->plog.push_back(lg);
    hipEvent_t e0 = nullptr, e1 = nullptr;
    const bool prof = c->prof_max > 0 && c->prof_n < c->prof_max;
    if (prof) {
        e0 = c->prof[2 * c->prof_n];
        e1 = c->prof[2 * c->prof_n + 1];
    }
    {
        std::lock_guard<std::mutex> lk(g_persist_mu);
        const int dev = c->device;
        if (dev >= 0 && dev < MAX_DEVICES) {
            if (!g_persist_ev[dev]) HIPOK(c, hipEventCreateWithFlags(&g_persist_ev[dev], hipEventDisableTiming));
            if (g_persist_last[dev] && g_persist_last[dev] != c) HIPOK(c, hipStreamWaitEvent(c->stream, g_persist_ev[dev], 0));
        }
        if (prof) HIPOK(c, hipEventRecord(e0, c->stream));
        hipError_t e;
        const bool rows_late = store && (c->tune_persist_rows_late == 2 ||
                                         (c->tune_persist_rows_late == 1 && (launch_local || c->N / 2 / 16 >= 8 * (int64_t)c->num_cu)));
        if (c->target != EMX_TARGET_DENSE_GAUSS) {
            const Shape shv = pick_shape(c->D, c->D);
            e = launch_persist_valu(shv.G, shv.V, shv.CH, launch_move, launch_local ? 1 : 0, grid, block, c->stream, P);
        } else if (launch_mix) {
            e = launch_persist_mix(c->Dp / 16, launch_local ? 1 : 0, grid, block, lds, c->stream, P);
        } else if (c->Dp > 64) {
            P.base.ablate = c->tune_persist_slab_skew ? 256 | (int32_t)((c->tune_persist_slab_skew - 1) << 9) : 0;
            e = launch_persist_slab(c->Dp / 16, launch_move, launch_local ? 1 : 0, c->D & 1, grid, block, lds, c->stream, P);
            c->persist_slab_launches++;
        } else if (c->D & 1) {
            e = launch_persist_dense_odd(c->Dp / 16, launch_move, launch_local ? 1 : 0, grid, block, lds, c->stream, P);
        } else {
            e = launch_hot_persist_dense(c->Dp / 16, launch_move, launch_local ? 1 : 0, rows_late ? 1 : 0, grid, block, lds, c->stream, P);
        }
        if (launch_local) c->persist_local_launches++;
        if (e != hipSuccess) FAIL(c, -2, "persistent half-step launch failed: %s", hipGetErrorString(e));
        if (prof) {
            HIPOK(c, hipEventRecord(e1, c->stream));
            c->prof_n++;
        }
        if (dev >= 0 && dev < MAX_DEVICES) {
            HIPOK(c, hipEventRecord(g_persist_ev[dev], c->stream));
            g_persist_last[dev] = c;
        }
    }
    if (!used_slots.empty()) {
        hipEvent_t& ev = c->pipe_batch_ev[4 + (c->pipe_cons_n & 3)];
        if (!ev) HIPOK(c, hipEventCreateWithFlags(&ev, hipEventDisableTiming));
        c->pipe_cons_n++;
        HIPOK(c, hipEventRecord(ev, c->stream));
        for (int sl : used_slots) {
            c->ring[sl].consumed_ref = ev;
            c->ring[sl].busy = true;
            c->ring[sl].last_seq = P.seq;
        }
    }
    if (mtmode && !devp) pipe_poll(c);
    c->mtdev_defer_release = false;
    if (c->mtdev_release_pending >= 0 && c->mtdev) {
        const int rcr = c->mtdev->release_batch(c->mtdev_release_pending, c->stream);
        c->mtdev_release_pending = -1;
        if (rcr) FAIL(c, rcr, "%s", c->mtdev->error().c_str());
    }
    c->persist_launches++;
    c->persist_halfsteps += n;
    *done = steps;
    return 0;
}

static int persist_settle(emx_ctx* c) {
    if (c->plog.empty()) return 0;
    HIPOK(c, hipSetDevice(c->device));
    HIPOK(c, wait_stream(c->stream));
    if (!__atomic_load_n(&c->status_host[3], __ATOMIC_ACQUIRE) || !c->persist_bar) {
        c->plog.clear();
        return 0;
    }
    unsigned w[4] = {0, 0, 0, 0};
    HIPOK(c, hipMemcpy(w, c->persist_bar + 9 * PERSIST_BAR_STRIDE, sizeof(w), hipMemcpyDeviceToHost));
    if (w[1] != 1u) {
        c->plog.clear();
        return 0;
    }
    const unsigned done_seq = w[3];
    std::deque<emx_ctx::PersistLog> redo;
    for (const auto& e : c->plog)
        if ((int)(e.seq - done_seq) > 0) redo.push_back(e);
    c->plog.clear();
    const bool exact_redo = !redo.empty() && redo.front().pipe_step0 >= 0;
    if (exact_redo && (c->pipe == nullptr || c->pipe != redo.front().pipe_id || c->pipe_taken - redo.front().pipe_step0 > 60 || c->cur.active))
        return 0;
    HIPOK(c, hipMemsetAsync(c->persist_bar, 0, PERSIST_BAR_WORDS * sizeof(unsigned), c->stream));
    c->persist_epoch = 0;
    c->persist_lepoch = 0;
    c->persist_hepoch = 0;
    c->persist_grid = 0;
    __atomic_store_n(&c->status_host[3], 0u, __ATOMIC_RELEASE);
    if (redo.empty()) return 0;
    NEED(c, !c->cur.active, "persistent launches to redo, but a step is open");
    const int64_t stored_end = c->stored, proposals_end = c->proposals;
    const uint64_t ph_end = c->ph_step;
    for (const auto& m : c->moves) NEED(c, m.kind != EMX_MOVE_GAUSS, "persistent launches to redo in a mixture with a Gaussian move");
    drop_prepared(c);
    if ((w[2] & (w[2] - 1u)) != 0u)
        c->tune_persist_local = 0;
    else
        c->tune_persist = 0;
    if (exact_redo) {
        MT19937Legacy before = c->mt;
        c->pipe->finish(redo.front().pipe_step0, before);
        delete c->pipe;
        c->pipe = nullptr;
        c->pipe_uploads.clear();
        c->pipe_deferred.clear();
        c->mt = before;
    }
// ... 39 lines not shown
    const MtDevStats& st = c->mtdev ? c->mtdev->stats() : c->mtdev_stats_last;
    out[0] = st.windows;
    out[1] = st.tok_rounds;
    out[2] = st.tail_groups;
    out[3] = st.tail_rounds;
    for (int k = 0; k < 4; ++k) out[4 + k] = st.tok_ticks[k];
    return 0;
}

int emx_mtdev_debug(emx_ctx* c, int32_t what, int64_t arg, void* out, int64_t n) {
    NEED(c, c->mtdev != nullptr, "emx_mtdev_debug: no device producer is alive");
    int rc = -1;
    if (what == 0) {
        rc = c->mtdev->debug_stream((uint64_t)arg, n, (uint32_t*)out);
    } else if (what == 1) {
        NEED(c, n >= c->N, "emx_mtdev_debug: output too small");
        rc = c->mtdev->debug_targets(arg, (uint32_t*)out);
    } else if (what == 2) {
        const int S = c->moves[0].nsplits;
        NEED(c, n >= 3 * S + 1, "emx_mtdev_debug: output too small");
        rc = c->mtdev->debug_positions(arg, (uint64_t*)out, (uint64_t*)out + 3 * S);
    } else {
        FAIL(c, -1, "emx_mtdev_debug: unknown item %d", what);
    }
    if (rc) FAIL(c, rc, "%s", c->mtdev->error().c_str());
    return 0;
}

int emx_host_mt_jump(const uint32_t key[624], uint64_t stride_words, int32_t k, uint32_t out_key[624]) {
    if (k < 1 || stride_words < 1) return -1;
    const uint32_t* g = nullptr;
    if (!mt_jump_polys(stride_words, k, &g)) return -1;
    std::vector<uint32_t> win((size_t)MT_WINDOW + MT_N), cur(key, key + MT_N), nxt(MT_N);
    for (size_t have = 0; have < win.size(); have += MT_N) {
        mt_twist_block(cur.data(), nxt.data());
        cur.swap(nxt);
        memcpy(win.data() + have, cur.data(), std::min<size_t>(MT_N, win.size() - have) * 4);
    }
    mt_apply_jump(g + (size_t)(k - 1) * MT_POLY_WORDS, win.data(), out_key);
    return 0;
}

int emx_host_persist_shape(int64_t nwalkers, int32_t nsplits, int32_t num_cu, int32_t* waves_per_group, int32_t* groups) {
    const int wpb = persist_shape_of(nwalkers, nsplits, num_cu);
    *waves_per_group = wpb;
    *groups = wpb ? (int32_t)(nwalkers / nsplits / 16 / wpb) : 0;
    return 0;
}

int emx_persist_info(emx_ctx* c, int64_t out[4]) {
    const int64_t keep = c->call_steps;
    c->call_steps = (int64_t)1 << 40;
    out[0] = (persist_wanted(c) || persist_gauss_wanted(c) || persist_valu_wanted(c)) ? 1 : 0;
    c->call_steps = keep;
    out[1] = c->persist_launches;
    out[2] = c->persist_halfsteps;
    out[3] = c->persist_recovered;
    return 0;
}

int emx_small_info(emx_ctx* c, int64_t out[4]) {
    out[0] = c->small_launches;
    out[1] = c->small_steps;
    out[2] = out[3] = 0;
    return 0;
}

int emx_small_fused_pays(int64_t nwalkers, int32_t ndim, int32_t rng_mode) { return small_fused_pays(nwalkers, ndim, rng_mode) ? 1 : 0; }

int emx_small_fused_check(int64_t nwalkers, int32_t ndim, int32_t nmoves, const emx_move_desc* moves, int32_t rng_mode, int32_t nblobs,
                          char* msg, int32_t msglen) {
    char buf[320];
    const char* why = small_fused_refusal(nwalkers, ndim, nmoves, moves, rng_mode, nblobs, buf, sizeof buf);
    if (!why) return 0;
    if (msg && msglen > 0) snprintf(msg, (size_t)msglen, "%s", why);
    return -1;
}

int emx_persist_local_launches(emx_ctx* c, int64_t* n) {
    *n = c->persist_local_launches;
    return 0;
}

int emx_run(emx_ctx* c, int64_t nsteps, int32_t thin_by, int32_t store) {
    HIPOK(c, hipSetDevice(c->device));
    NEED(c, thin_by >= 1, "Invalid thinning argument");
    NEED(c, !c->cur.active, "emx_run: a step begun with emx_step_begin is still open");
    const int64_t total = nsteps * thin_by;
    c->call_steps = total;
    const bool devp = mtdev_eligible(c);
    if (c->mtdev && !devp) {
        const int rcm = mtdev_stop(c);
        if (rcm) return rcm;
    }
    const bool piped = !devp && pipe_eligible(c) && c->target != EMX_TARGET_HOST && (c->pipe || total >= 2);
    if (c->pipe && !piped) PIPE_STOP(c);
    if (c->pipe && persist_exact_ok(c) != (c->pipe_nsinks == PLAN_RING)) PIPE_STOP(c);
    if (piped && !c->pipe) {
        const int rc = pipe_start(c);
        if (rc) return rc;
    }
    const int rc = run_impl(c, nsteps, thin_by, store);
    c->call_steps = 1;
    if (rc && (c->pipe || c->mtdev)) pipe_stop(c);
    return rc;
}

static int run_impl(emx_ctx* c, int64_t nsteps, int32_t thin_by, int32_t store) {
    NEED(c, thin_by >= 1, "Invalid thinning argument");
    NEED(c, c->rng_mode != EMX_RNG_INPUTS, "emx_run needs an RNG mode that generates plans");
    NEED(c, c->target != EMX_TARGET_HOST, "emx_run needs a device target");
    const bool push_replay = c->exchange == EMX_EXCHANGE_REPLAY && c->peers_ready;
    NEED(c, (c->world == 1 && !c->sendbuf) || c->comm || push_replay || (c->world == 1 && c->exchange == EMX_EXCHANGE_REPLAY),
         "emx_run on a sharded context needs emx_comm_init (or drive emx_halfstep / the collective from the host layer)");
    NEED(c, c->exchange != EMX_EXCHANGE_DIRECT || c->world == 1 || c->peers_ready,
         "direct exchange: the peers' arrays are not mapped yet (emx_direct_export / emx_direct_import, or emx_direct_attach)");
    c->direct_first_barrier = true;
    if (store) NEED(c, c->stored + nsteps <= c->cap, "chain capacity exhausted (call emx_chain_config)");
    const int64_t total = nsteps * thin_by;
    const bool valu_on = persist_valu_wanted(c);
    const bool small_on = small_eligible(c) && !valu_on;
    const bool persist_on = (persist_wanted(c) && !small_on && !(store && c->Dp == 16)) || valu_on;
    const bool persist_gauss_on = persist_gauss_wanted(c) && !small_on;
    bool ctr_synced = false;
    int64_t next_mark = c->tune_throttle > 0 ? c->tune_throttle : total + 1;
    int marks = 0;
    for (int64_t i = 0; i < total;) {
        if (i >= next_mark) {
            const int slot = marks & 3;
            if (!c->thr_ev[slot]) HIPOK(c, hipEventCreateWithFlags(&c->thr_ev[slot], hipEventDisableTiming));
            HIPOK(c, hipEventRecord(c->thr_ev[slot], c->stream));
            if (marks >= 2) {
                hipEvent_t old = c->thr_ev[(marks - 2) & 3];
                while (hipEventQuery(old) == hipErrorNotReady) {
                }
            }
            ++marks;
            next_mark += c->tune_throttle;
        }
        if (small_on) {
            drop_prepared(c);
            int64_t chunk = std::min<int64_t>(total - i, 4096);
            if (c->rng_mode == EMX_RNG_MT19937)
                chunk = std::min<int64_t>(chunk, std::max<int64_t>(8, (4 << 20) / (32 * c->N)));
            const int rc = run_small(c, i, chunk, thin_by, store);
            if (rc) return rc;
            i += chunk;
            ctr_synced = false;
            continue;
        }
        if (persist_gauss_on) {
            int64_t done = 0;
            const int rc = run_persist_gauss(c, i, total, thin_by, store, &done);
            if (rc) return rc;
            i += done;
            ctr_synced = false;
            continue;
        }
        if (persist_on && c->tune_persist && c->rng_mode == EMX_RNG_MT19937) {
            if (persist_move_ok(c, c->moves[0])) {
                int64_t done = 0;
                const int rc = run_persist(c, i, total, thin_by, store, &done);
                if (rc) return rc;
                i += done;
                ctr_synced = false;
                if (done > 0) continue;
            }
        } else if (persist_on && c->tune_persist) {
            if (!c->prepared.empty() && c->prepared.front().step != c->ph_step) drop_prepared(c);
            if (c->prepared.empty()) {
                const int rcp = native_prepare_batch(c, c->ph_step, NATIVE_BATCH_MAX, -1, c->stream);
                if (rcp) return rcp;
// ... 875 lines not shown
        c->direct_planned = true;
    }
    if (barrier && G > 1) {
        PeerBarrierArgs b{};
        for (int q = 0; q < G; ++q) {
            NEED(c, c->peer_flags[q], "direct exchange: no barrier flags for rank %d", q);
            b.peer_flags[q] = c->peer_flags[q];
        }
        b.my_flags = c->my_flags;
        b.dead = c->direct_counts + 64;
        b.status = c->status;
        b.epoch = ++c->direct_epoch;
        b.timeout_ticks = (unsigned long long)c->tune_direct_timeout_ms * (c->direct_first_barrier ? 6ull : 1ull) * 100000ull;
        c->direct_first_barrier = false;
        b.rank = c->rank;
        b.npeer = (int32_t)G;
        hipLaunchKernelGGL(k_peer_barrier, dim3(1), dim3(64), 0, c->stream, b);
        HIPOK(c, hipGetLastError());
    }
    const int ns = cur.off[split + 1] - cur.off[split];
    if (ns <= 0) return 0;
    const int64_t bmax = (N + G - 1) / G;
    const double mean = (double)ns / G;
    int64_t bound = (int64_t)std::ceil(mean + 8.0 * std::sqrt(mean) + 64.0);
    bound = std::max<int64_t>(1, std::min<int64_t>(bound, std::min<int64_t>(bmax, ns)));
    double *chain = nullptr, *chain_lp = nullptr;
    if (cur.store) {
        chain = c->chain + (size_t)c->stored * N * c->D;
        chain_lp = c->chain_lp + (size_t)c->stored * N;
    }
    return launch_split(c, mv.kind, c->target, cur.S, split, cur.off[split], (int)bound, 0, (int)bound, &mv, &c->cplan, nullptr, c->X,
                        c->lp, chain, chain_lp, nullptr, nullptr, c->direct_counts + split);
}

static void block_args(emx_ctx* c, BlockArgs& a, double* rec) {
    a.X = c->X;
    a.lp = c->lp;
    a.acc = c->acc;
    a.acc_count = c->acc_count;
    a.rec = rec;
    a.N = (int32_t)c->N;
    a.D = c->D;
    a.G = c->world;
    a.rank = c->rank;
    a.bmax = (int32_t)((c->N + c->world - 1) / c->world);
}

int emx_replica_pack(emx_ctx* c, int64_t* records_per_rank) {
    HIPOK(c, hipSetDevice(c->device));
    NEED(c, c->exchange != EMX_EXCHANGE_ALLGATHER, "emx_replica_pack is for the block-ownership exchanges (pull, direct)");
    int rc = c->exchange == EMX_EXCHANGE_PULL ? pull_ensure(c) : direct_ensure(c);
    if (rc) return rc;
    BlockArgs a{};
    block_args(c, a, c->sendbuf);
    hipLaunchKernelGGL(k_block_pack, dim3((unsigned)((a.bmax + 15) / 16)), dim3(256), 0, c->stream, a);
    HIPOK(c, hipGetLastError());
    if (records_per_rank) *records_per_rank = a.bmax;
    return 0;
}

int emx_replica_unpack(emx_ctx* c) {
    HIPOK(c, hipSetDevice(c->device));
    NEED(c, c->exchange != EMX_EXCHANGE_ALLGATHER && c->gathered, "emx_replica_unpack is for the block-ownership exchanges (pull, direct)");
    BlockArgs a{};
    block_args(c, a, c->gathered);
    const int64_t nrec = (int64_t)a.G * a.bmax;
    hipLaunchKernelGGL(k_block_unpack, dim3((unsigned)((nrec + 15) / 16)), dim3(256), 0, c->stream, a);
    HIPOK(c, hipGetLastError());
    return 0;
}

int emx_device_ptr(emx_ctx* c, int32_t which, void** ptr, int64_t* nbytes) {
    switch (which) {
        case 0: *ptr = c->X; *nbytes = c->N * c->D * 8; return 0;
        case 1: *ptr = c->lp; *nbytes = c->N * 8; return 0;
        case 2: *ptr = c->sendbuf; *nbytes = c->send_doubles * 8; return 0;
        case 3: *ptr = c->gathered; *nbytes = c->recv_doubles * 8; return 0;
        case 4: *ptr = c->chain; *nbytes = c->stored * c->N * c->D * 8; return 0;
        case 5: *ptr = c->chain_lp; *nbytes = c->stored * c->N * 8; return 0;
        case 6: *ptr = c->disp; *nbytes = c->disp ? c->N * c->D * 8 : 0; return 0;
        case 7: *ptr = c->dbg; *nbytes = c->dbg ? c->dbg_blocks * 16 * 8 : 0; return 0;
        case 8: *ptr = c->my_flags; *nbytes = c->my_flags ? EMX_MAX_PEERS * 8 : 0; return 0;
    }
    FAIL(c, -1, "unknown device pointer id %d", which);
}

int emx_shard_slots(emx_ctx* c, int32_t split, int64_t* lo, int64_t* hi, int64_t* ns) {
    auto& cur = c->cur;
    NEED(c, cur.active && split >= 0 && split < cur.S, "emx_shard_slots outside a planned step");
    *ns = cur.off[split + 1] - cur.off[split];
    shard_range(*ns, c->rank, c->world, *lo, *hi);
    return 0;
}

int emx_scatter_gathered(emx_ctx* c, int32_t split) { return scatter_gathered(c, split, c->sendbuf_rows); }

static int scatter_gathered(emx_ctx* c, int32_t split, int64_t block_rows) {
    HIPOK(c, hipSetDevice(c->device));
    auto& cur = c->cur;
    NEED(c, cur.active && c->gathered, "emx_scatter_gathered needs an active sharded step");
    NEED(c, split >= 0 && split < cur.S, "split out of range");
    const int ns = cur.off[split + 1] - cur.off[split];
    const int64_t rec = c->D + 2;
    for (int r = 0; r < c->world; ++r) {
        if (r == c->rank) continue;
        int64_t lo, hi;
        shard_range(ns, r, c->world, lo, hi);
        if (hi <= lo) continue;
        ScatterArgs a{};
        a.X = c->X;
        a.lp = c->lp;
        a.acc = c->acc;
        a.acc_count = c->acc_count;
        if (cur.store) {
            a.chain = c->chain + (size_t)c->stored * c->N * c->D;
            a.chain_lp = c->chain_lp + (size_t)c->stored * c->N;
        }
        a.gathered = c->gathered + ((int64_t)r * block_rows - lo) * rec;
        a.order = cur.slot >= 0 ? c->ring[cur.slot].order : nullptr;
        a.N = (int32_t)c->N;
        a.D = c->D;
        a.S = cur.S;
        a.split = split;
        a.pos0 = cur.off[split];
        a.t_lo = (int32_t)lo;
        a.t_hi = (int32_t)hi;
        hipLaunchKernelGGL(k_scatter_rows, dim3((unsigned)((hi - lo + 3) / 4)), dim3(256), 0, c->stream, a);
        HIPOK(c, hipGetLastError());
    }
    return 0;
}

int emx_comm_load(const char* librccl_path) {
    std::string err;
    const int rc = rccl_load(librccl_path, err);
    if (rc) g_err = err;
    return rc;
}

int emx_comm_get_unique_id(uint8_t id[128]) {
    std::string err;
    if (rccl_load(nullptr, err)) {
        g_err = err;
        return -5;
    }
    RcclId u;
    const int e = g_rccl.GetUniqueId(&u);
    if (e != 0) {
        g_err = "ncclGetUniqueId failed";
        return -6;
    }
    memcpy(id, u.internal, 128);
    return 0;
}

int emx_comm_init(emx_ctx* c, int32_t rank, int32_t world, const uint8_t id[128]) {
    HIPOK(c, hipSetDevice(c->device));
    std::string err;
    if (rccl_load(nullptr, err)) FAIL(c, -5, "%s", err.c_str());
    NEED(c, !c->comm, "communicator already initialised");
    int rc = emx_set_shard(c, rank, world);
    if (rc) return rc;
    if (c->exchange == EMX_EXCHANGE_PULL) {
        rc = pull_ensure(c);
        if (rc) return rc;
    } else if (c->exchange == EMX_EXCHANGE_DIRECT) {
// ... 314 lines not shown
```

emcee_amd/csrc/emx_hot.hip:

```cpp
#include "emx_launch.hpp"

namespace emx {

hipError_t launch_hot_stretch_dense64(int lean, dim3 grid, dim3 block, size_t lds, hipStream_t st, const HalfStepArgs& a) {
    if (lean == 2) return launch_one<8, 2, 4, MOVE_STRETCH, 4, 2>(grid, block, lds, st, a);
    if (lean == 3) return launch_one<8, 2, 4, MOVE_STRETCH, 4, 3>(grid, block, lds, st, a);
    if (lean == 4) return launch_one<8, 2, 4, MOVE_STRETCH, 4, 4>(grid, block, lds, st, a);
    return launch_one<8, 2, 4, MOVE_STRETCH, 4, 1>(grid, block, lds, st, a);
}

template <int G, int V, int CH, int DPB, int MOVE, bool LOCAL = false, bool ROWS_LATE = false>
static hipError_t launch_persist(dim3 grid, dim3 block, size_t lds, hipStream_t st, const PersistArgs& P) {
    auto kern = k_persist<G, V, CH, DPB, MOVE, LOCAL, ROWS_LATE>;
    static size_t lds_granted[MAX_DEVICES] = {};
    int dev = 0;
    if (lds > 48 * 1024 && hipGetDevice(&dev) == hipSuccess && dev >= 0 && dev < MAX_DEVICES && lds > lds_granted[dev]) {
        hipError_t e = hipFuncSetAttribute((const void*)kern, hipFuncAttributeMaxDynamicSharedMemorySize, (int)lds);
        if (e != hipSuccess) return e;
        lds_granted[dev] = lds;
    }
    hipLaunchKernelGGL(kern, grid, block, lds, st, P);
    return hipGetLastError();
}

hipError_t launch_hot_persist_dense(int dpb, int move, int local, int rows_late, dim3 grid, dim3 block, size_t lds, hipStream_t st, const PersistArgs& P) {
    if (rows_late && move == MOVE_STRETCH) {
#define EMX_SCASE(b, ch)                                                                                       \
    if (dpb == b)                                                                                              \
        return local ? launch_persist<8, 2, ch, b, MOVE_STRETCH, true, true>(grid, block, lds, st, P)          \
                     : launch_persist<8, 2, ch, b, MOVE_STRETCH, false, true>(grid, block, lds, st, P);
        EMX_SCASE(1, 1) EMX_SCASE(2, 2) EMX_SCASE(3, 4) EMX_SCASE(4, 4)
#undef EMX_SCASE
        return hipErrorInvalidValue;
    }
    if (local) {
#define EMX_LCASE(b, ch)                                                                                           \
    if (dpb == b)                                                                                                  \
        return move == MOVE_DE        ? launch_persist<8, 2, ch, b, MOVE_DE, true>(grid, block, lds, st, P)        \
               : move == MOVE_SNOOKER ? launch_persist<8, 2, ch, b, MOVE_SNOOKER, true>(grid, block, lds, st, P)   \
                                      : launch_persist<8, 2, ch, b, MOVE_STRETCH, true>(grid, block, lds, st, P);
        EMX_LCASE(1, 1) EMX_LCASE(2, 2) EMX_LCASE(3, 4) EMX_LCASE(4, 4)
#undef EMX_LCASE
        return hipErrorInvalidValue;
    }
#define EMX_CASE(b, ch)                                                                                            \
    if (dpb == b)                                                                                                  \
        return move == MOVE_DE        ? launch_persist<8, 2, ch, b, MOVE_DE>(grid, block, lds, st, P)              \
               : move == MOVE_SNOOKER ? launch_persist<8, 2, ch, b, MOVE_SNOOKER>(grid, block, lds, st, P)         \
                                      : launch_persist<8, 2, ch, b, MOVE_STRETCH>(grid, block, lds, st, P);
    EMX_CASE(1, 1) EMX_CASE(2, 2) EMX_CASE(3, 4) EMX_CASE(4, 4)
#undef EMX_CASE
    return hipErrorInvalidValue;
}

template <int G, int V, int CH, int DPB, int MOVE>
static hipError_t persist_occupancy(int threads, size_t lds, int* per_cu) {
    auto kern = k_persist<G, V, CH, DPB, MOVE>;
    if (lds > 48 * 1024) {
        const hipError_t e = hipFuncSetAttribute((const void*)kern, hipFuncAttributeMaxDynamicSharedMemorySize, (int)lds);
        if (e != hipSuccess) return e;
    }
    return hipOccupancyMaxActiveBlocksPerMultiprocessor(per_cu, kern, threads, lds);
}

hipError_t hot_persist_occupancy(int dpb, int move, int threads, size_t lds, int* per_cu) {
#define EMX_CASE(b, ch)                                                                                     \
    if (dpb == b)                                                                                           \
        return move == MOVE_DE        ? persist_occupancy<8, 2, ch, b, MOVE_DE>(threads, lds, per_cu)       \
               : move == MOVE_SNOOKER ? persist_occupancy<8, 2, ch, b, MOVE_SNOOKER>(threads, lds, per_cu)  \
                                      : persist_occupancy<8, 2, ch, b, MOVE_STRETCH>(threads, lds, per_cu);
    EMX_CASE(1, 1) EMX_CASE(2, 2) EMX_CASE(3, 4) EMX_CASE(4, 4)
#undef EMX_CASE
    return hipErrorInvalidValue;
}

hipError_t launch_hot_persist_gauss(int dpb, dim3 grid, dim3 block, size_t lds, hipStream_t st, const PersistGaussArgs& P) {
#define EMX_CASE(b, ch)                                                                                              \
    if (dpb == b) {                                                                                                  \
        auto kern = k_persist_gauss<8, 2, ch, b>;                                                                    \
        static size_t lds_granted[MAX_DEVICES] = {};                                                                 \
        int dev = 0;                                                                                                 \
        if (lds > 48 * 1024 && hipGetDevice(&dev) == hipSuccess && dev >= 0 && dev < MAX_DEVICES && lds > lds_granted[dev]) { \
            hipError_t e = hipFuncSetAttribute((const void*)kern, hipFuncAttributeMaxDynamicSharedMemorySize, (int)lds); \
            if (e != hipSuccess) return e;                                                                           \
            lds_granted[dev] = lds;                                                                                  \
        }                                                                                                            \
        hipLaunchKernelGGL(kern, grid, block, lds, st, P);                                                           \
        return hipGetLastError();                                                                                    \
    }
    EMX_CASE(1, 1) EMX_CASE(2, 2) EMX_CASE(3, 4) EMX_CASE(4, 4)
#undef EMX_CASE
    return hipErrorInvalidValue;
}

}
```

emcee_amd/csrc/emx_kernels.hpp:

```cpp
#pragma once
#include <hip/hip_runtime.h>

#include <cstdint>
#include <type_traits>

#include "emx_planlog.hpp"
#include "emx_rng.hpp"

#ifndef EMX_OPT_RED4
#define EMX_OPT_RED4 1
#endif
#ifndef EMX_OPT_RTILE
#define EMX_OPT_RTILE 1
#endif
#ifndef EMX_LEAN_FOLD_D
#define EMX_LEAN_FOLD_D 0
#endif
#ifndef EMX_LEAN_FOLD_SPW
#define EMX_LEAN_FOLD_SPW 1
#endif
#ifndef EMX_OPT_SKEW
#define EMX_OPT_SKEW 1
#endif
#ifndef EMX_SNOOKER_BUDGET
// ... 1148 lines not shown
            if (wall_clock64() - t0 > P.timeout_ticks) {
                raise_status(P.base.status, ST_EXCHANGE_TIMEOUT);
                __hip_atomic_store(go + 1, 2u, __ATOMIC_RELAXED, __HIP_MEMORY_SCOPE_AGENT);
                break;
            }
        }
        if (wall) wall[1] = wall_clock64();
    }
    __syncthreads();
}

__device__ __forceinline__ void persist_stagger_wait(int stagger, int wib) {
    const int how = stagger >> 8, cnt = stagger & 255;
    const int units = how == 0 ? (wib >> 2) : how == 1 ? (wib & 1) : how == 2 ? ((wib >> 1) & 1) : (wib & 3);
    for (int s = 0; s < cnt * units; ++s) __builtin_amdgcn_s_sleep(1);
}

template <bool LOCAL = false>
__device__ __forceinline__ bool persist_handshake(const PersistArgs& P) {
    __shared__ int ok_s;
    if (threadIdx.x == 0) {
        const unsigned k = LOCAL ? P.hepoch0 + 1u : P.epoch0 + 1u;
        const int xcd = LOCAL ? 0 : (int)(blockIdx.x & 7);
        const unsigned per = LOCAL ? gridDim.x >> 3 : (gridDim.x + 7 - xcd) / 8;
        unsigned* xctr = P.bar + xcd * PERSIST_BAR_STRIDE;
        unsigned* gctr = P.bar + 8 * PERSIST_BAR_STRIDE;
        unsigned* go = P.bar + 9 * PERSIST_BAR_STRIDE;
        int ok = 1;
        const unsigned long long v0 = __hip_atomic_load(reinterpret_cast<unsigned long long*>(go), __ATOMIC_RELAXED, __HIP_MEMORY_SCOPE_AGENT);
        if ((v0 >> 32) != 0ull) {
            ok = 0;
        } else {
            unsigned xcc = 0;
            if constexpr (LOCAL) {
                asm volatile("s_getreg_b32 %0, hwreg(HW_REG_XCC_ID)" : "=s"(xcc));
                __hip_atomic_fetch_or(go + 2, 1u << (xcc & 15u), __ATOMIC_RELAXED, __HIP_MEMORY_SCOPE_AGENT);
                asm volatile("s_waitcnt vmcnt(0)" ::: "memory");
            }
            const unsigned old = __hip_atomic_fetch_add(xctr, 1u, __ATOMIC_RELAXED, __HIP_MEMORY_SCOPE_AGENT);
            if (old == k * per - 1) {
                bool open = true;
                unsigned o2 = k * 8 - 1;
                if constexpr (LOCAL) {
                    const unsigned m = __hip_atomic_load(go + 2, __ATOMIC_RELAXED, __HIP_MEMORY_SCOPE_AGENT);
                    open = (m & (m - 1u)) == 0u;
                    if (open) {
                        __hip_atomic_store(go + 2, 0u, __ATOMIC_RELAXED, __HIP_MEMORY_SCOPE_AGENT);
                    } else {
                        raise_status(P.base.status, ST_EXCHANGE_TIMEOUT);
                        __hip_atomic_store(go + 1, 1u, __ATOMIC_RELAXED, __HIP_MEMORY_SCOPE_AGENT);
                    }
                } else {
                    o2 = __hip_atomic_fetch_add(gctr, 1u, __ATOMIC_RELAXED, __HIP_MEMORY_SCOPE_AGENT);
                }
                if (open && o2 == k * 8 - 1) {
                    __hip_atomic_store(go + 4, LOCAL ? (xcc & 15u) + 1u : 0u, __ATOMIC_RELAXED, __HIP_MEMORY_SCOPE_AGENT);
                    __hip_atomic_store(go + 3, P.seq, __ATOMIC_RELAXED, __HIP_MEMORY_SCOPE_AGENT);
                    if (P.started_host) __hip_atomic_store(P.started_host, P.seq, __ATOMIC_RELAXED, __HIP_MEMORY_SCOPE_SYSTEM);
                    __hip_atomic_store(go, k, __ATOMIC_RELAXED, __HIP_MEMORY_SCOPE_AGENT);
                }
            }
            const unsigned long long t0 = wall_clock64();
            for (;;) {
                const unsigned long long v = __hip_atomic_load(reinterpret_cast<unsigned long long*>(go), __ATOMIC_RELAXED, __HIP_MEMORY_SCOPE_AGENT);
                if ((v >> 32) != 0ull) {
                    ok = 0;
                    break;
                }
                if ((int)((unsigned)v - k) >= 0) break;
                if (wall_clock64() - t0 > P.timeout_ticks) {
                    raise_status(P.base.status, ST_EXCHANGE_TIMEOUT);
                    __hip_atomic_store(go + 1, 1u, __ATOMIC_RELAXED, __HIP_MEMORY_SCOPE_AGENT);
                    ok = 0;
                    break;
                }
            }
        }
        ok_s = ok;
    }
    __syncthreads();
    return ok_s != 0;
}

template <int G, int V, int CH, int DPB, int MOVE = MOVE_STRETCH, bool LOCAL = false, bool ROWS_LATE = false>
static __global__ __launch_bounds__(512) void k_persist(const PersistArgs P) {
    static_assert(MOVE == MOVE_STRETCH || MOVE == MOVE_DE || MOVE == MOVE_SNOOKER, "the red / blue moves");
    if (LOCAL && (blockIdx.x & 7u) != 0u) return;
    const unsigned bid = LOCAL ? blockIdx.x >> 3 : blockIdx.x, ngroups = LOCAL ? gridDim.x >> 3 : gridDim.x;
    constexpr int CPOL = EMX_CPOL_SC1;
    constexpr int CPOL_ST = LOCAL ? 0 : EMX_CPOL_SC1;
    constexpr bool DE = MOVE == MOVE_DE || MOVE == MOVE_SNOOKER;
    constexpr bool SN = MOVE == MOVE_SNOOKER;
    constexpr bool DEFER = !DE;
    constexpr int WPW = 64 / G;
    constexpr int PPT = 16 / WPW;
    constexpr int PF = PPT;
    static_assert(EMX_OPT_RTILE && EMX_OPT_RED4, "the persistent kernel is the one-tile-per-batch form");
    constexpr int Dp = DPB * 16, KK = Dp / 4, RT = Dp + 2;
    static_assert(G * V * CH >= Dp, "row layout must cover the padded dimension");
    extern __shared__ __attribute__((aligned(16))) double smem[];
    const HalfStepArgs& A = P.base;
    const int lane = threadIdx.x & 63;
    const int wib = threadIdx.x >> 6;
    const int sub = lane / G;
    const int gl = lane % G;
    const int D = A.D;
    double* Sfrag = smem;
    double* muS = smem + dense_img_doubles(Dp);
    double* tile = muS + Dp + (size_t)wib * (16 * RT + 32);
    double* qfS = tile + 16 * RT;
    double* facS = qfS + 16;
    {
        constexpr int IMG2 = (dense_img_doubles(Dp) + Dp) / 2;
        const double2* img = reinterpret_cast<const double2*>(A.tp1);
        double2* dst = reinterpret_cast<double2*>(smem);
        for (int e = threadIdx.x; e < IMG2; e += blockDim.x) dst[e] = img[e];
    }
    Row<G, V, CH> mu;
    load_row<G, V, CH>(mu, A.tp0, D, gl);
    if (!persist_handshake<LOCAL>(P)) return;
    const int wave = (int)bid * (blockDim.x >> 6) + wib;
    const int t0 = wave * 16;
    unsigned long long pst[6] = {0, 0, 0, 0, 0, 0}, pt = 0;
    const bool prof = EMX_OPT_STAMPS && A.dbg && wib == EMX_STAMP_WAVE;
    if (prof) {
        pt = __builtin_readcyclecounter();
        if (lane == 0) A.dbg[(size_t)bid * 16 + 11] = wall_clock64();
    }
#define EMX_PSTAMP(k_)                                                   \
    do {                                                                 \
        if (prof) {                                                      \
            const unsigned long long t_ = __builtin_readcyclecounter(); \
            pst[k_] += t_ - pt;                                          \
            pt = t_;                                                     \
        }                                                                \
    } while (0)
    const __amdgpu_buffer_rsrc_t Xr = __builtin_amdgcn_make_buffer_rsrc((void*)A.X, 0, A.N * D * 8, 0x00020000);
    const int myrow = (lane >> 4) + 4 * (lane & 3);
    const bool mine = (lane & 15) < 4;

    int wi[PF], ja[PF], jb[DE ? PF : 1], jc[SN ? PF : 1], my_i;
    double s0v[PF], facv[PF], my_logu, my_lpo;
    Row<G, V, CH> xi[PF];
    {
        const PersistCols I(P.it[0], (size_t)P.base.N);
        const int pbase = I.pos0 + t0;
#pragma unroll
        for (int k = 0; k < PF; ++k) {
            const int pos = pbase + k * WPW + sub;
            wi[k] = I.order[pos];
            ja[k] = I.p0[pos];
            if constexpr (DE) jb[k] = I.p1[pos];
            if constexpr (SN) jc[k] = I.p2[pos];
            s0v[k] = SN ? 0.0 : I.s0[pos];
            facv[k] = I.fac[pos];
        }
        my_i = I.order[pbase + myrow];
        my_logu = I.logu[pbase + myrow];
#pragma unroll
        for (int k = 0; k < PF; ++k) load_row_agent<G, V, CH, CPOL>(xi[k], Xr, wi[k], D, gl);
        my_lpo = load_agent(A.lp + my_i);
    }
    Row<G, V, CH> crow[DEFER ? PF : 1];
    int cwi[PF], cmy_i = 0;
    double clp = 0.0;
    double *cchain = nullptr, *cchain_lp = nullptr;
#pragma unroll
    for (int k = 0; k < PF; ++k) {
        if (DEFER || k == 0) crow[DEFER ? k : 0] = xi[k];
        cwi[k] = 0;
    }
    for (int n = 0; n < P.niter; ++n) {
        const PersistCols I(P.it[n], (size_t)P.base.N);
        Row<G, V, CH> xa[PF], xb[DE ? PF : 1], xc[SN ? PF : 1];
        persist_stagger_wait(P.stagger, wib);
#pragma unroll
        for (int k = 0; k < PF; ++k) {
            load_row_agent<G, V, CH, CPOL>(xa[k], Xr, ja[k], D, gl);
            if constexpr (DE) load_row_agent<G, V, CH, CPOL>(xb[k], Xr, jb[k], D, gl);
            if constexpr (SN) load_row_agent<G, V, CH, CPOL>(xc[k], Xr, jc[k], D, gl);
        }
        const bool more = n + 1 < P.niter;
        const PersistCols J(P.it[more ? n + 1 : n], (size_t)P.base.N);
        const bool pre = more && J.split != 0;
        const unsigned stamp = P.epoch0 + (unsigned)n + 1u;
        int wi_n[PF], ja_n[PF], jb_n[DE ? PF : 1], jc_n[SN ? PF : 1], my_i_n;
        double s0_n[PF], fac_n[PF], my_logu_n;
        {
            const int pbase = J.pos0 + t0;
#pragma unroll
            for (int k = 0; k < PF; ++k) {
                const int pos = pbase + k * WPW + sub;
                wi_n[k] = J.order[pos];
                ja_n[k] = J.p0[pos];
                if constexpr (DE) jb_n[k] = J.p1[pos];
                if constexpr (SN) jc_n[k] = J.p2[pos];
                s0_n[k] = SN ? 0.0 : J.s0[pos];
                fac_n[k] = J.fac[pos];
            }
            my_i_n = J.order[pbase + myrow];
            my_logu_n = J.logu[pbase + myrow];
        }
        if (prof) { asm volatile("s_waitcnt vmcnt(0)" ::: "memory"); }
        EMX_PSTAMP(0);
        Row<G, V, CH> qk[PF];
#pragma unroll
        for (int k = 0; k < PF; ++k) {
            const int srow = k * WPW + sub;
            double factor = facv[k];
            Row<G, V, CH> q;
            make_proposal<G, V, CH, MOVE>(xi[k], xa[k], xb[DE ? k : 0], xc[SN ? k : 0], s0v[k], A.gammas, D, gl, q, factor, ja[k]);
            bool bl = false;
#pragma unroll
            for (int c = 0; c < CH; ++c)
#pragma unroll
                for (int v = 0; v < V; ++v) bl |= !(fabs(q.x[c][v]) <= 1.79769313486231570815e308);
            const bool badq = group_any<G>(bl, sub);
            if (badq && gl == 0) raise_status(A.status, ST_BAD_COORD);
            const int trow = srow & 15;
#pragma unroll
            for (int c = 0; c < CH; ++c)
#pragma unroll
                for (int v = 0; v < V; ++v) {
                    const int d = (c * G + gl) * V + v;
                    if (d < Dp) tile[trow * RT + d] = !badq ? q.x[c][v] - mu.x[c][v] : 0.0;
                }
            qk[k] = q;
            if (gl == 0) facS[trow] = badq ? -__builtin_inf() : factor;
        }
        if (DEFER && cchain) {
#pragma unroll
            for (int k = 0; k < PF; ++k) store_row_stream<G, V, CH>(crow[k], cchain + (size_t)cwi[k] * D, D, gl);
            if (mine) cchain_lp[cmy_i] = clp;
            cchain = nullptr;
        }
        if (I.chain) {
#pragma unroll
            for (int k = 0; k < PF; ++k) {
                if constexpr (DEFER)
                    crow[k] = xi[k];
                else
                    store_row_stream<G, V, CH>(xi[k], I.chain + (size_t)wi[k] * D, D, gl);
            }
        }
        double my_lpo_n = 0.0;
        if (!ROWS_LATE && more) {
#pragma unroll
            for (int k = 0; k < PF; ++k) load_row_agent<G, V, CH, CPOL>(xi[k], Xr, wi_n[k], D, gl);
            my_lpo_n = load_agent(A.lp + my_i_n);
        }
        EMX_WAVE_SYNC();
        EMX_PSTAMP(1);
        double my_qf;
        {
            const int am = lane & 15, ak = lane >> 4;
            typedef double d4 __attribute__((ext_vector_type(4)));
            double afr[KK];
#pragma unroll
            for (int kk = 0; kk < KK; ++kk) afr[kk] = tile[am * RT + 4 * kk + ak];
            double part[4] = {0.0, 0.0, 0.0, 0.0};
#pragma unroll
            for (int nb = 0; nb < DPB; ++nb) {
                d4 accv = {0.0, 0.0, 0.0, 0.0};
#pragma unroll
                for (int kk = 4 * nb; kk < KK; ++kk)
                    accv = __builtin_amdgcn_mfma_f64_16x16x4f64(afr[kk], Sfrag[(dense_block(DPB, nb, kk >> 2) * 4 + (kk & 3)) * 64 + lane], accv, 0, 0, 0);
#pragma unroll
                for (int r = 0; r < 4; ++r) part[r] = fma(accv[r], accv[r], part[r]);
            }
            my_qf = row16_sum4(part[0], part[1], part[2], part[3], lane);
        }
        if (ROWS_LATE && more) {
            __builtin_amdgcn_sched_barrier(0);
#pragma unroll
            for (int k = 0; k < PF; ++k) load_row_agent<G, V, CH, CPOL>(xi[k], Xr, wi_n[k], D, gl);
            my_lpo_n = load_agent(A.lp + my_i_n);
            __builtin_amdgcn_sched_barrier(0);
        }
        if (prof) { asm volatile("s_nop 0" ::: "memory"); }
        EMX_PSTAMP(2);
        bool acc = false;
        if (mine) {
            const double lpn = -0.5 * my_qf;
            if (lpn != lpn) raise_status(A.status, ST_NAN_LOGP);
            const double lnpdiff = facS[myrow] + lpn - my_lpo;
            acc = lnpdiff > my_logu;
            store_scope<LOCAL>(A.acc + my_i, (uint8_t)(acc ? 1 : 0));
            if (acc) {
                store_scope<LOCAL>(A.lp + my_i, lpn);
                store_scope<LOCAL>(P.ver + my_i, stamp);
            }
            if (I.chain_lp) {
                if constexpr (DEFER)
                    clp = acc ? lpn : my_lpo;
                else
                    I.chain_lp[my_i] = acc ? lpn : my_lpo;
                if (acc) store_scope<LOCAL>(A.acc_count + my_i, load_agent(A.acc_count + my_i) + 1u);
            }
        }
        const unsigned long long am64 = __ballot(acc);
#pragma unroll
        for (int pp = 0; pp < PPT; ++pp) {
            const int row = pp * WPW + sub;
            const bool ac = (am64 >> ((row & 3) * 16 + (row >> 2))) & 1ull;
            if (ac) {
                store_row_agent<G, V, CH, CPOL_ST>(qk[pp], Xr, wi[pp], D, gl);
                if (I.chain) {
                    if constexpr (DEFER)
                        crow[pp] = qk[pp];
                    else
                        store_row_stream<G, V, CH>(qk[pp], I.chain + (size_t)wi[pp] * D, D, gl);
                }
            }
        }
        if (DEFER && I.chain) {
            cchain = I.chain;
            cchain_lp = I.chain_lp;
            cmy_i = my_i;
#pragma unroll
            for (int k = 0; k < PF; ++k) cwi[k] = wi[k];
        }
        EMX_WAVE_SYNC();
        EMX_PSTAMP(3);
        if (prof) {
            asm volatile("s_waitcnt vmcnt(0)" ::: "memory");
            EMX_PSTAMP(4);
        }
        if (!more) break;
        if constexpr (LOCAL)
            persist_barrier_local(P, P.lepoch0 + (unsigned)n + 1u, bid, ngroups);
        else
            persist_barrier(P, P.epoch0 + (unsigned)n + 2u,
                            (EMX_OPT_STAMPS && A.dbg) ? A.dbg + 4096 + ((size_t)n * ngroups + bid) * 2 : nullptr);
        EMX_PSTAMP(5);
#pragma unroll
        for (int k = 0; k < PF; ++k) {
            wi[k] = wi_n[k];
            ja[k] = ja_n[k];
            if constexpr (DE) jb[k] = jb_n[k];
            if constexpr (SN) jc[k] = jc_n[k];
            s0v[k] = s0_n[k];
            facv[k] = fac_n[k];
        }
        my_i = my_i_n;
        my_logu = my_logu_n;
        my_lpo = my_lpo_n;
        if (!pre) {
            unsigned vk[PF];
#pragma unroll
            for (int k = 0; k < PF; ++k) vk[k] = load_agent(P.ver + wi[k]);
            const unsigned vm = load_agent(P.ver + my_i);
#pragma unroll
            for (int k = 0; k < PF; ++k)
                if (vk[k] == stamp) load_row_agent<G, V, CH, CPOL>(xi[k], Xr, wi[k], D, gl);
            if (vm == stamp) my_lpo = load_agent(A.lp + my_i);
        }
    }
    if (DEFER && cchain) {
#pragma unroll
        for (int k = 0; k < PF; ++k) store_row_stream<G, V, CH>(crow[k], cchain + (size_t)cwi[k] * D, D, gl);
        if (mine) cchain_lp[cmy_i] = clp;
    }
    if (prof && lane == 0) {
        unsigned long long* o = A.dbg + (size_t)bid * 16;
#pragma unroll
        for (int k = 0; k < 6; ++k) o[k] = pst[k];
        o[6] = (unsigned long long)P.niter;
        o[12] = wall_clock64();
    }
#undef EMX_PSTAMP
}

constexpr int SMALL_MAX_MOVES = 8;
struct GaussGen {
    unsigned long long gseed, gstep;
    double gfac, gsigma;
    const double* gscale;
};
constexpr int PERSIST_GAUSS_MAX_STEPS = 16;
struct PersistGaussStep {
    const int32_t* p0;
    const double* logu;
    double *chain, *chain_lp;
    unsigned long long gstep;
    double gfac;
};
struct PersistGaussArgs {
    HalfStepArgs base;
    PersistGaussStep st[PERSIST_GAUSS_MAX_STEPS];
    int32_t nsteps;
};

template <int G, int V, int CH, int DPB>
static __global__ __launch_bounds__(512) void k_persist_gauss(const PersistGaussArgs P) {
    constexpr int MOVE = MOVE_GAUSS;
    constexpr int WPW = 64 / G;
    constexpr int PPT = 16 / WPW;
    constexpr int Dp = DPB * 16, KK = Dp / 4, RT = Dp + 2;
    static_assert(EMX_OPT_RTILE && EMX_OPT_RED4 && G * V * CH >= Dp, "the one-tile-per-batch form");
    extern __shared__ __attribute__((aligned(16))) double smem[];
    const HalfStepArgs& A = P.base;
    const int lane = threadIdx.x & 63;
    const int wib = threadIdx.x >> 6;
    const int sub = lane / G;
    const int gl = lane % G;
    const int D = A.D;
    double* Sfrag = smem;
    double* muS = smem + dense_img_doubles(Dp);
    double* tile = muS + Dp + (size_t)wib * (16 * RT + 32);
    double* facS = tile + 16 * RT + 16;
    {
        constexpr int IMG2 = (dense_img_doubles(Dp) + Dp) / 2;
        const double2* img = reinterpret_cast<const double2*>(A.tp1);
        double2* dst = reinterpret_cast<double2*>(smem);
        for (int e = threadIdx.x; e < IMG2; e += blockDim.x) dst[e] = img[e];
    }
    Row<G, V, CH> mu;
    load_row<G, V, CH>(mu, A.tp0, D, gl);
    __syncthreads();
    const int wave = blockIdx.x * (blockDim.x >> 6) + wib;
    const int w0 = wave * 16;
    const int myrow = (lane >> 4) + 4 * (lane & 3);
    const bool mine = (lane & 15) < 4;
    const int my_i = w0 + myrow;
    Row<G, V, CH> xi[PPT];
#pragma unroll
    for (int k = 0; k < PPT; ++k) load_row<G, V, CH>(xi[k], A.X + (size_t)(w0 + k * WPW + sub) * D, D, gl);
    double my_lp = A.lp[my_i];
    bool my_acc = false;
    for (int s = 0; s < P.nsteps; ++s) {
        const PersistGaussStep& S = P.st[s];
        GaussGen gg;
        gg.gseed = A.gseed;
        gg.gstep = S.gstep;
        gg.gfac = S.gfac;
        gg.gsigma = A.gsigma;
        gg.gscale = A.gscale;
        const double my_logu = S.logu[my_i];
        Row<G, V, CH> qk[PPT];
#pragma unroll
        for (int k = 0; k < PPT; ++k) {
            const int i = w0 + k * WPW + sub;
            const int col = S.p0[i];
            Row<G, V, CH> xa, q;
            gauss_disp_row<G, V, CH>(xa, gg, i, col, D, gl);
            double factor = 0.0;
            make_proposal<G, V, CH, MOVE>(xi[k], xa, xa, xa, 0.0, A.gammas, D, gl, q, factor, col);
            bool bl = false;
#pragma unroll
            for (int c = 0; c < CH; ++c)
// ... 901 lines not shown
    const double lp_old = A.lp[i];
    if (nlp != nlp) raise_status(A.status, ST_NAN_LOGP);
    const double lnpdiff = A.fout[t] + nlp - lp_old;
    const bool accept = lnpdiff > plan_log(uacc);
    const double* q = A.qout + (size_t)t * A.D;
    double* xr = A.X + (size_t)i * A.D;
    if (accept)
        for (int d = lane; d < A.D; d += 64) xr[d] = q[d];
    if (A.chain)
        for (int d = lane; d < A.D; d += 64) __builtin_nontemporal_store(accept ? q[d] : xr[d], &A.chain[(size_t)i * A.D + d]);
    if (lane == 0) {
        if (accept) A.lp[i] = nlp;
        A.acc[i] = accept ? 1 : 0;
        if (A.chain_lp) {
            A.chain_lp[i] = accept ? nlp : lp_old;
            if (accept) A.acc_count[i] += 1u;
        }
    }
}

struct GaussDispArgs {
    double* disp;
    const double* scale;
    const int32_t* col;
    double sigma, f;
    uint64_t seed, step;
    int32_t N, D, mode;
};

static __global__ __launch_bounds__(256) void k_gauss_disp(const GaussDispArgs A) {
    const long long tid = (long long)blockIdx.x * blockDim.x + threadIdx.x;
    const int npair = (A.D + 1) / 2;
    if (A.mode == GAUSS_VECTOR) {
        if (tid >= (long long)A.N * npair) return;
        const int w = (int)(tid / npair), pr = (int)(tid - (long long)w * npair);
        double n0, n1;
        native_gauss_pair(A.seed, A.step, w, pr, n0, n1);
        const int d0 = 2 * pr, d1 = d0 + 1;
        const double s0 = A.f * (A.scale ? A.scale[d0] : A.sigma);
        A.disp[(size_t)w * A.D + d0] = s0 * n0;
        if (d1 < A.D) {
            const double s1 = A.f * (A.scale ? A.scale[d1] : A.sigma);
            A.disp[(size_t)w * A.D + d1] = s1 * n1;
        }
    } else {
        if (tid >= A.N) return;
        const int w = (int)tid, d = A.col[w];
        double n0, n1;
        native_gauss_pair(A.seed, A.step, w, d >> 1, n0, n1);
        const double sc = A.f * (A.scale ? A.scale[d] : A.sigma);
        A.disp[(size_t)w * A.D + d] = sc * ((d & 1) ? n1 : n0);
    }
}

static __global__ __launch_bounds__(256) void k_gauss_scale(const GaussDispArgs A) {
    const long long tid = (long long)blockIdx.x * blockDim.x + threadIdx.x;
    if (tid >= (long long)A.N * A.D) return;
    const int d = (int)(tid % A.D);
    const double sc = A.f * (A.scale ? A.scale[d] : A.sigma);
    A.disp[tid] = sc * A.disp[tid];
}

#ifndef EMX_NATIVE_BATCH
#define EMX_NATIVE_BATCH 16
#endif
constexpr int NATIVE_BATCH_MAX = EMX_NATIVE_BATCH;
struct NativeBatchArgs {
    NativeArgs nat[NATIVE_BATCH_MAX];
    int32_t* order[NATIVE_BATCH_MAX];
    int32_t* p0[NATIVE_BATCH_MAX];
    int32_t* p1[NATIVE_BATCH_MAX];
    int32_t* p2[NATIVE_BATCH_MAX];
    double* s0[NATIVE_BATCH_MAX];
    double* uacc[NATIVE_BATCH_MAX];
    double* logu[NATIVE_BATCH_MAX];
    double* fac[NATIVE_BATCH_MAX];
    double a[NATIVE_BATCH_MAX], sigma[NATIVE_BATCH_MAX], g0[NATIVE_BATCH_MAX];
    int32_t move[NATIVE_BATCH_MAX], S[NATIVE_BATCH_MAX];
    int32_t gmode[NATIVE_BATCH_MAX], gcol[NATIVE_BATCH_MAX];
    int32_t N, D, nb;
    int32_t lean;
    int32_t ablate;
    const StepDesc* desc;
};

template <bool ONLY_STRETCH>
static __device__ __forceinline__ void native_plan_batch_body(const NativeBatchArgs& B) {
    const int b = blockIdx.y;
    const int pos = blockIdx.x * blockDim.x + threadIdx.x;
    if (pos >= B.N || (EMX_EXPERIMENTS && !ONLY_STRETCH && (B.ablate & 4))) return;
    const int N = B.N, S = B.S[b];
    int split = 0, t = pos;
    const SplitSizes sz = split_sizes(N, S);
    for (int s = 0; s < S; ++s) {
        const int n = sz.of(s);
        if (t < n) { split = s; break; }
        t -= n;
    }
    int i, a0, a1, a2;
    double z, u;
    const int mv = ONLY_STRETCH ? MOVE_STRETCH : B.move[b];
    const NativeArgs nat = (!ONLY_STRETCH && B.desc) ? B.desc[b].nat : B.nat[b];
    if (mv == MOVE_GAUSS)
        native_gauss_slot(nat, B.D, B.gmode[b], B.gcol[b], pos, i, a0, a1, a2, z, u);
    else if (mv == MOVE_WALK || mv == MOVE_KDE)
        native_slot<MOVE_EVAL>(nat, N, S, split, t, B.a[b], B.sigma[b], B.g0[b], i, a0, a1, a2, z, u);
    else if (mv == MOVE_STRETCH)
        native_slot<MOVE_STRETCH>(nat, N, S, split, t, B.a[b], B.sigma[b], B.g0[b], i, a0, a1, a2, z, u);
    else if (mv == MOVE_DE)
        native_slot<MOVE_DE>(nat, N, S, split, t, B.a[b], B.sigma[b], B.g0[b], i, a0, a1, a2, z, u);
    else
        native_slot<MOVE_SNOOKER>(nat, N, S, split, t, B.a[b], B.sigma[b], B.g0[b], i, a0, a1, a2, z, u);
    const bool full = ONLY_STRETCH ? false : !B.lean;
    if (EMX_EXPERIMENTS && !ONLY_STRETCH && (B.ablate & 2)) {
        if (i + a0 + a1 + a2 == -12345 && z + u == 1.2345e-300) B.order[b][pos] = i;
        return;
    }
    if (EMX_EXPERIMENTS && !ONLY_STRETCH && (B.ablate & 1)) {
        B.order[b][pos] = i;
        B.p0[b][pos] = a0;
        B.s0[b][pos] = z;
        B.logu[b][pos] = u;
        B.fac[b][pos] = z;
        return;
    }
    B.order[b][pos] = i;
    B.p0[b][pos] = a0;
    if (full || mv == MOVE_DE || mv == MOVE_SNOOKER) B.p1[b][pos] = a1;
    if (full || mv == MOVE_SNOOKER) B.p2[b][pos] = a2;
    if (full || mv != MOVE_SNOOKER) B.s0[b][pos] = z;
    if (full) B.uacc[b][pos] = u;
    B.logu[b][pos] = plan_log_uniform(u);
    B.fac[b][pos] = (mv == MOVE_STRETCH) ? ((double)B.D - 1.0) * plan_log(z) : 0.0;
}

static __global__ __launch_bounds__(256) void k_native_plan_batch(const NativeBatchArgs B) { native_plan_batch_body<false>(B); }

static __global__ __launch_bounds__(256) void k_native_plan_batch_stretch(const NativeBatchArgs B) { native_plan_batch_body<true>(B); }

static __global__ void k_graph_set(GraphCounters* ctr, unsigned long long step_base, long long stored_base) {
    ctr->step_base = step_base;
    ctr->stored_base = stored_base;
}

static __global__ void k_graph_advance(GraphCounters* ctr, StepDesc* desc, unsigned long long seed, int N, int nb, int store) {
    const int b = threadIdx.x;
    const unsigned long long base = ctr->step_base;
    const long long sb = ctr->stored_base;
    __syncthreads();
    if (b < nb) {
        desc[b].nat.seed = seed;
        desc[b].nat.step = base + (unsigned long long)b;
        desc[b].nat.pk = make_perm_key((uint64_t)N, seed, base + (unsigned long long)b);
        desc[b].stored_idx = store ? sb + b : -1;
    }
    if (b == 0) {
        ctr->step_base = base + (unsigned long long)nb;
        if (store) ctr->stored_base = sb + nb;
    }
}

struct ScatterArgs {
    double* X;
    double* lp;
    uint8_t* acc;
    uint32_t* acc_count;
    double* chain;
    double* chain_lp;
    const double* gathered;
    const int32_t* order;
    int32_t N, D, S, split, pos0, t_lo, t_hi;
};

static __global__ __launch_bounds__(256) void k_scatter_rows(const ScatterArgs A) {
    const int lane = threadIdx.x & 63;
    const int t = A.t_lo + blockIdx.x * (blockDim.x >> 6) + (threadIdx.x >> 6);
    if (t >= A.t_hi) return;
    const int i = A.order[A.pos0 + t];
    const double* src = A.gathered + (size_t)t * (A.D + 2);
    double* dst = A.X + (size_t)i * A.D;
    for (int d = lane; d < A.D; d += 64) dst[d] = src[d];
// ... 379 lines not shown
```

emcee_amd/csrc/emx_launch.hpp:

```cpp
#pragma once
#include <hip/hip_runtime.h>

#include "emx_kernels.hpp"

namespace emx {

constexpr int MAX_DEVICES = 64;

template <int G, int V, int CH, int MOVE, int DPB, int LEAN = 0>
hipError_t launch_one(dim3 grid, dim3 block, size_t lds, hipStream_t st, const HalfStepArgs& a) {
    auto kern = k_halfstep<G, V, CH, MOVE, DPB, LEAN>;
    static size_t lds_granted[MAX_DEVICES] = {};
    int dev = 0;
    if (lds > 48 * 1024 && hipGetDevice(&dev) == hipSuccess && dev >= 0 && dev < MAX_DEVICES && lds > lds_granted[dev]) {
        hipError_t e = hipFuncSetAttribute((const void*)kern, hipFuncAttributeMaxDynamicSharedMemorySize, (int)lds);
        if (e != hipSuccess) return e;
        lds_granted[dev] = lds;
    }
    hipLaunchKernelGGL(kern, grid, block, lds, st, a);
    return hipGetLastError();
}

hipError_t launch_hot_stretch_dense64(int lean, dim3 grid, dim3 block, size_t lds, hipStream_t st, const HalfStepArgs& a);
hipError_t launch_hot_persist_dense(int dpb, int move, int local, int rows_late, dim3 grid, dim3 block, size_t lds, hipStream_t st, const PersistArgs& P);
hipError_t hot_persist_occupancy(int dpb, int move, int threads, size_t lds, int* per_cu);
hipError_t launch_hot_persist_gauss(int dpb, dim3 grid, dim3 block, size_t lds, hipStream_t st, const PersistGaussArgs& P);
hipError_t launch_persist_mix(int dpb, int local, dim3 grid, dim3 block, size_t lds, hipStream_t st, const PersistArgs& P);
hipError_t persist_mix_occupancy(int dpb, int threads, size_t lds, int* per_cu);
hipError_t launch_persist_valu(int G, int V, int CH, int move, int local, dim3 grid, dim3 block, hipStream_t st, const PersistArgs& P);
hipError_t launch_slab_dense(int dpb, int move, dim3 grid, dim3 block, size_t lds, hipStream_t st, const HalfStepArgs& a);
size_t slab_lds_bytes(int Dp, int waves);
hipError_t launch_persist_dense_odd(int dpb, int move, int local, dim3 grid, dim3 block, size_t lds, hipStream_t st, const PersistArgs& P);
hipError_t persist_dense_odd_occupancy(int dpb, int move, int threads, size_t lds, int* per_cu);
hipError_t launch_persist_slab(int dpb, int move, int local, int odd, dim3 grid, dim3 block, size_t lds, hipStream_t st, const PersistArgs& P);
hipError_t persist_slab_occupancy(int dpb, int move, int odd, int threads, size_t lds, int* per_cu);

struct WideLpArgs {
    const double* rows;
    const int32_t* order;
    const double* img;
    double* out;
    uint32_t* status;
    const int32_t* t_hi_dev;
    int32_t D, Dp, pos0, t_lo, t_hi, scatter, check_bad;
    int32_t single_role;
};
struct WideCommitArgs {
    double* X;
    double* lp;
    uint8_t* acc;
    uint32_t* acc_count;
    double* chain;
    double* chain_lp;
    double* sendbuf;
    const double* qout;
    const double* fout;
    const double* newlp;
    const int32_t* order;
    const double* logu;
    const int32_t* t_hi_dev;
    uint32_t* status;
    double* declp;
    int32_t D, pos0, t_lo, t_hi;
};
hipError_t launch_wide_lp(const WideLpArgs& a, int nrows_bound, int num_cu, hipStream_t st);
hipError_t launch_wide_commit(const WideCommitArgs& a, int nrows_bound, int num_cu, hipStream_t st);

}
```

emcee_amd/device.py:

```python
import ctypes as C

import numpy as np

from . import _lib
from ._lib import EmxError, MoveDesc

__all__ = ["DeviceEnsemble", "EmxError"]

_STATUS_NAN_LOGP = 1
_STATUS_BAD_COORD = 2
_STATUS_EXCHANGE_OVERFLOW = 4
_STATUS_EXCHANGE_TIMEOUT = 8
_STATUS_PLAN_PRODUCER = 16
_STATUS_SINGULAR_COV = 32


def _blob_shape(b):
    return b[..., 0] if b.shape[-1] == 1 else b


def _as_f64(a, shape=None):
    a = np.ascontiguousarray(a, dtype=np.float64)
    if shape is not None and a.shape != shape:
        raise ValueError("expected array of shape %s, got %s" % (shape, a.shape))
# ... 548 lines not shown

    def replay_finish(self, split):
        self._ck(self.lib.emx_replay_finish(self.ctx, int(split)))

    def direct_export(self):
        h = np.zeros(128, dtype=np.uint8)
        self._ck(self.lib.emx_direct_export(self.ctx, h))
        return h

    def direct_import(self, handles):
        h = np.ascontiguousarray(handles, dtype=np.uint8).reshape(-1)
        self._ck(self.lib.emx_direct_import(self.ctx, h))

    def direct_attach(self, coords_ptrs, flags_ptrs=None):
        n = len(coords_ptrs)
        a = (C.c_void_p * n)(*[C.c_void_p(p) for p in coords_ptrs])
        f = None if flags_ptrs is None else (C.c_void_p * n)(*[C.c_void_p(p) for p in flags_ptrs])
        self._ck(self.lib.emx_direct_attach(self.ctx, a, f))

    def direct_halfstep(self, split, barrier=False):
        self._ck(self.lib.emx_direct_halfstep(self.ctx, int(split), int(bool(barrier))))

    def replica_pack(self):
        n = C.c_int64()
        self._ck(self.lib.emx_replica_pack(self.ctx, C.byref(n)))
        return n.value

    def replica_unpack(self):
        self._touch()
        self._ck(self.lib.emx_replica_unpack(self.ctx))

    @staticmethod
    def rccl_unique_id():
        lib = _lib.load()
        DeviceEnsemble._load_rccl(lib)
        uid = np.zeros(128, dtype=np.uint8)
        rc = lib.emx_comm_get_unique_id(uid)
        if rc != 0:
            raise EmxError((lib.emx_last_error(None) or b"ncclGetUniqueId failed").decode())
        return uid

    @staticmethod
    def _load_rccl(lib):
        import os
        path = os.environ.get("EMX_RCCL_LIB")
        if not path:
            try:
                import torch
                cand = os.path.join(os.path.dirname(torch.__file__), "lib", "librccl.so")
                path = cand if os.path.exists(cand) else None
            except Exception:
                path = None
        rc = lib.emx_comm_load(path.encode() if path else None)
        if rc != 0:
            raise EmxError((lib.emx_last_error(None) or b"cannot load librccl").decode())

    def comm_init(self, rank, world, unique_id):
        self._load_rccl(self.lib)
        uid = np.ascontiguousarray(unique_id, dtype=np.uint8)
        self._ck(self.lib.emx_comm_init(self.ctx, int(rank), int(world), uid))

    def comm_destroy(self):
        self._ck(self.lib.emx_comm_destroy(self.ctx))

    def pipeline_stats(self):
        out = np.zeros(6)
        n, k = C.c_int64(0), C.c_int32(0)
        self._ck(self.lib.emx_pipeline_stats(self.ctx, out, C.byref(n), C.byref(k)))
        if n.value <= 0:
            return None
        return {"steps_produced": n.value, "finisher_threads": k.value, "wall_us": out[0], "generator_us": out[1], "tokenizer_us": out[2],
                "finishers_us_summed": out[3], "tokenizer_waited_for_words_us": out[4], "tokenizer_waited_for_consumer_us": out[5]}

    def pipeline_handovers(self):
        raw, regen = C.c_int64(0), C.c_int64(0)
        self._ck(self.lib.emx_pipeline_handovers(self.ctx, C.byref(raw), C.byref(regen)))
        return {"raw_steps": int(raw.value), "regen_steps": int(regen.value)}

    def persist_info(self):
        out = (C.c_int64 * 4)()
        self._ck(self.lib.emx_persist_info(self.ctx, out))
        loc = C.c_int64(0)
        self._ck(self.lib.emx_persist_local_launches(self.ctx, C.byref(loc)))
        return {"qualifies": bool(out[0]), "launches": int(out[1]), "halfsteps": int(out[2]), "recovered": int(out[3]),
                "local_launches": int(loc.value)}

    def small_info(self):
        out = (C.c_int64 * 4)()
        self._ck(self.lib.emx_small_info(self.ctx, out))
        return {"launches": int(out[0]), "steps": int(out[1])}

    def mtdev_info(self):
        out = (C.c_int64 * 8)()
        self._ck(self.lib.emx_mtdev_info(self.ctx, out))
        return {"qualifies": bool(out[0]), "alive": bool(out[1]), "steps": int(out[2]), "rounds": int(out[3]), "segments": int(out[4]),
                "batches": int(out[5]), "windows": int(out[6]), "poly_us": int(out[7])}

    def mtdev_tok_stats(self):
        out = (C.c_int64 * 8)()
        self._ck(self.lib.emx_mtdev_tok_stats(self.ctx, out))
        return {"windows": int(out[0]), "rounds": int(out[1]), "tail_groups": int(out[2]), "tail_rounds": int(out[3]),
                "wait_us": out[4] / 100.0, "chunk_us": out[5] / 100.0, "tail_us": out[6] / 100.0, "kernel_us": out[7] / 100.0}

    def mtdev_debug(self, what, arg, n=0):
        if what == 0:
            out = np.empty(int(n), dtype=np.uint32)
        elif what == 1:
            out = np.empty(self.nwalkers, dtype=np.uint32)
        else:
            out = np.empty(int(n), dtype=np.uint64)
        self._ck(self.lib.emx_mtdev_debug(self.ctx, int(what), int(arg), out.ctypes.data, out.size))
        return out

    def comm_count(self):
        n = C.c_int32(0)
        self._ck(self.lib.emx_comm_count(self.ctx, C.byref(n)))
        return n.value

    def timer_start(self):
        self._ck(self.lib.emx_timer_start(self.ctx))

    def timer_stop(self):
        ms = C.c_float()
        self._ck(self.lib.emx_timer_stop(self.ctx, C.byref(ms)))
        return ms.value

    def profile_enable(self, max_launches):
        self._ck(self.lib.emx_profile_enable(self.ctx, int(max_launches)))

    def profile_read(self, max_launches):
        out = np.empty(max_launches, dtype=np.float32)
        n = C.c_int32(max_launches)
        self._ck(self.lib.emx_profile_read(self.ctx, out, C.byref(n)))
        return out[: n.value]
```

include/emx.h:

```cpp
#ifndef EMX_H
#define EMX_H
#include <stdint.h>

#ifdef __cplusplus
extern "C" {
#endif

typedef struct emx_ctx emx_ctx;

enum emx_target_kind {
    EMX_TARGET_HOST = 0,
    EMX_TARGET_ISO_GAUSS = 1,
    EMX_TARGET_DIAG_GAUSS = 2,
    EMX_TARGET_DENSE_GAUSS = 3,
    EMX_TARGET_ROSENBROCK = 4,
    EMX_TARGET_BOX = 5,
    EMX_TARGET_DEVICE_CALLBACK = 6,
    EMX_TARGET_FUSED_USER = 8,
    EMX_TARGET_FUSED_PT = 9,
    EMX_TARGET_FUSED_ENSEMBLE = 10
};

enum emx_move_kind {
    EMX_MOVE_STRETCH = 0, EMX_MOVE_DE = 1, EMX_MOVE_SNOOKER = 2,
// ... 117 lines not shown
int emx_halfstep(emx_ctx* ctx, int32_t split);
int emx_propose(emx_ctx* ctx, int32_t split, double* q_out, double* factors_out , int64_t* ns_out);
int emx_accept(emx_ctx* ctx, int32_t split, const double* new_log_prob);
int emx_accept_proposals(emx_ctx* ctx, int32_t split, const double* q, const double* factors,
                         const double* new_log_prob);
int emx_step_end(emx_ctx* ctx);
int emx_plan_set(emx_ctx* ctx, int32_t move_index, const int32_t* off, const int32_t* order, const int32_t* p0,
                 const int32_t* p1, const int32_t* p2, const double* s0, const double* uacc);
int emx_plan_get(emx_ctx* ctx, int32_t* off, int32_t* order, int32_t* p0, int32_t* p1, int32_t* p2, double* s0,
                 double* uacc);
int emx_plan_set_noise(emx_ctx* ctx, const double* normals, double factor);

int emx_set_shard(emx_ctx* ctx, int32_t rank, int32_t world);
int emx_set_shard_buffers(emx_ctx* ctx, void* sendbuf, void* gathered, int64_t rows_per_rank);
int emx_device_ptr(emx_ctx* ctx, int32_t which, void** ptr, int64_t* nbytes);
int emx_shard_slots(emx_ctx* ctx, int32_t split, int64_t* t_lo, int64_t* t_hi, int64_t* ns);
int emx_scatter_gathered(emx_ctx* ctx, int32_t split);

#define EMX_EXCHANGE_ALLGATHER 0
#define EMX_EXCHANGE_PULL 1
#define EMX_EXCHANGE_DIRECT 2
#define EMX_EXCHANGE_LOGPROB 3
#define EMX_EXCHANGE_REPLAY 4
int emx_set_exchange(emx_ctx* ctx, int32_t kind);
int emx_exchange_layout(emx_ctx* ctx, int64_t* send_doubles, int64_t* recv_doubles);
int emx_set_exchange_buffers(emx_ctx* ctx, void* send, int64_t send_doubles, void* recv, int64_t recv_doubles);
int emx_own_walkers(emx_ctx* ctx, int64_t* lo, int64_t* hi);
int emx_pull_prepare(emx_ctx* ctx, int32_t split, int64_t* records_per_peer);
int emx_pull_apply(emx_ctx* ctx, int32_t split);
int emx_replica_pack(emx_ctx* ctx, int64_t* records_per_rank);
int emx_replica_unpack(emx_ctx* ctx);

int emx_direct_export(emx_ctx* ctx, uint8_t handles[128]);
int emx_direct_import(emx_ctx* ctx, const uint8_t* handles );
int emx_direct_attach(emx_ctx* ctx, void* const* peer_coords , void* const* peer_flags );
int emx_direct_halfstep(emx_ctx* ctx, int32_t split, int32_t barrier);

int emx_logprob_begin(emx_ctx* ctx, int32_t split, int64_t* per_rank);
int emx_logprob_finish(emx_ctx* ctx, int32_t split);

int emx_replay_begin(emx_ctx* ctx, int32_t split, int64_t* rows_per_rank);
int emx_replay_finish(emx_ctx* ctx, int32_t split);
int emx_replay_exchange(emx_ctx* ctx, int32_t split);

int emx_comm_load(const char* librccl_path );
int emx_comm_get_unique_id(uint8_t id[128]);
int emx_comm_init(emx_ctx* ctx, int32_t rank, int32_t world, const uint8_t id[128]);
int emx_comm_destroy(emx_ctx* ctx);
int emx_comm_count(emx_ctx* ctx, int32_t* ranks_out);

int emx_fft_load(const char* libhipfft_path );
int emx_autocorr(emx_ctx* ctx, int64_t discard, int64_t thin, double c, double* tau_out, int32_t* window_out,
                 int64_t* nsamples_out);
int emx_summary(emx_ctx* ctx, int32_t plane, int64_t start, int64_t stop, int64_t stride, double* mean_out, double* cov_out,
                int32_t nranks, const int64_t* ranks, double* order_out, double* map_coords_out, double* map_log_prob_out,
                int64_t* nsamples_out);
int emx_summary_info(emx_ctx* ctx, int64_t* selection_reads_out, int64_t* listed_out, int64_t* list_reads_out);
int emx_rhat(emx_ctx* ctx, int64_t start, int64_t stop, int64_t stride, int32_t log_prob, double* within_out, double* between_out,
             int64_t* nchains_out, int64_t* length_out);
int emx_chain_minmax(emx_ctx* ctx, int32_t plane, int64_t start, int64_t stop, int64_t stride, double* lo_out, double* hi_out,
                     int64_t* nonfinite_out);
int emx_histograms(emx_ctx* ctx, int32_t plane, int64_t start, int64_t stop, int64_t stride, const int64_t* edge_off,
                   const double* edges, int64_t* counts_out, const int64_t* pedge_off, const double* pedges, int64_t npairs,
                   const int32_t* pairs, const int64_t* pair_off, int64_t* pair_counts_out, int64_t* nsamples_out);
int emx_walkers_independent(int32_t device, const double* coords, int64_t n, int32_t ndim, int32_t* independent,
                            double* cond_out);
int emx_walkers_independent_resident(emx_ctx* ctx, int32_t* independent, double* cond_out);

int emx_timer_start(emx_ctx* ctx);
int emx_timer_stop(emx_ctx* ctx, float* ms);
int emx_profile_enable(emx_ctx* ctx, int32_t max_launches);
int emx_profile_read(emx_ctx* ctx, float* ms_out, int32_t* n_inout);

int emx_pipeline_stats(emx_ctx* ctx, double out[6], int64_t* steps_produced, int32_t* finisher_threads);
int emx_pipeline_handovers(emx_ctx* ctx, int64_t* raw_steps, int64_t* regen_steps);

int emx_mtdev_info(emx_ctx* ctx, int64_t out[8]);
int emx_mtdev_debug(emx_ctx* ctx, int32_t what, int64_t arg, void* out, int64_t n);
int emx_mtdev_tok_stats(emx_ctx* ctx, int64_t out[8]);
int emx_host_mt_jump(const uint32_t key[624], uint64_t stride_words, int32_t k, uint32_t out_key[624]);

int emx_persist_info(emx_ctx* ctx, int64_t out[4]);
int emx_persist_local_launches(emx_ctx* ctx, int64_t* n);
int emx_host_persist_shape(int64_t nwalkers, int32_t nsplits, int32_t num_cu, int32_t* waves_per_group, int32_t* groups);

typedef struct emx_mt emx_mt;
emx_mt* emx_mt_create(const uint32_t key[624], int32_t pos, int32_t has_gauss, double cached);
void emx_mt_destroy(emx_mt* m);
void emx_mt_get_state(const emx_mt* m, uint32_t key[624], int32_t* pos, int32_t* has_gauss, double* cached);
void emx_mt_random_sample(emx_mt* m, int64_t n, double* out);
void emx_mt_randint(emx_mt* m, uint64_t bound, int64_t n, int64_t* out);
void emx_mt_randn(emx_mt* m, int64_t n, double* out);
void emx_mt_shuffle_labels(emx_mt* m, int64_t n, int32_t nsplits, int32_t* labels);
int32_t emx_mt_choice_cdf(emx_mt* m, const double* cdf, int32_t n);
int emx_host_plan_mt(emx_mt* m, int64_t nwalkers, int32_t ndim, const emx_move_desc* mv, int32_t* off, int32_t* order,
                     int32_t* p0, int32_t* p1, int32_t* p2, double* s0, double* uacc);
int emx_host_plan_mt_stream(emx_mt* m, int64_t nwalkers, int32_t ndim, int32_t nmoves, const emx_move_desc* moves,
                            const double* cdf, int64_t nsteps, int32_t nworkers, int32_t nsinks, int32_t* moves_out,
                            int32_t* order, int32_t* p0, int32_t* p1, int32_t* p2, double* s0, double* uacc,
                            double* seconds_out);
int emx_host_split_draws(emx_mt* m, int64_t nwalkers, const emx_move_desc* mv, const int32_t* off,
                         const int32_t* order, int32_t split, int32_t* p0, int32_t* p1, int32_t* p2, double* s0);
int emx_host_plan_philox(uint64_t seed, uint64_t step, int64_t nwalkers, const emx_move_desc* mv, int32_t* off,
                         int32_t* order, int32_t* p0, int32_t* p1, int32_t* p2, double* s0, double* uacc);
int32_t emx_host_move_choice_philox(uint64_t seed, uint64_t step, const double* cdf, int32_t n);
int64_t emx_host_walk_kde_draws(uint64_t seed, uint64_t step, int64_t nwalkers, int32_t ndim, const emx_move_desc* mv, int32_t split,
                                int32_t* helpers, double* normals);
int64_t emx_host_pull_capacity(int64_t nwalkers, int32_t world, int32_t nsplits, int32_t partners_per_walker);

typedef struct emx_batch emx_batch;
int emx_batch_check(int64_t nwalkers, int32_t ndim, int32_t target, int32_t nmoves, const emx_move_desc* moves, char* msg,
                    int32_t msglen);
int emx_batch_create(int32_t device, int32_t nbatch, int64_t nwalkers, int32_t ndim, emx_batch** out);
int emx_batch_destroy(emx_batch* b);
const char* emx_batch_last_error(emx_batch* b);
int emx_batch_set_tuning(emx_batch* b, const char* key, int64_t value);
int emx_batch_set_target(emx_batch* b, int32_t kind, const double* p0, const double* p1, const double* scales, int32_t per_member);
typedef int (*emx_batch_log_prob_fn)(void* user, const double* coords_dev, int32_t nbatch, int64_t rows, int32_t ndim,
                                     double* log_prob_dev, void* hip_stream);
int emx_set_batch_target_callback(emx_batch* b, emx_batch_log_prob_fn fn, void* user);
typedef struct emx_fused_launch {
    uint32_t abi;
    uint32_t args_bytes;
    int32_t ndim, movesel, grid, threads;
    uint64_t lds_bytes;
    void* hip_stream;
    const void* args;
    const void* user;
    int32_t nblobs;
    int32_t reserved;
} emx_fused_launch;
typedef int (*emx_fused_batch_fn)(const emx_fused_launch*);
int emx_set_batch_target_fused(emx_batch* b, emx_fused_batch_fn fn, int32_t ndim_compiled, const void* user_dev);
int emx_set_batch_target_fused_blobs(emx_batch* b, emx_fused_batch_fn fn, int32_t ndim_compiled, const void* user_dev, int32_t nblobs);
typedef int (*emx_batch_log_prob_blobs_fn)(void* user, const double* coords_dev, int32_t nbatch, int64_t rows, int32_t ndim,
                                           double* log_prob_dev, int32_t nblobs, double* blobs_dev, void* hip_stream);
int emx_set_batch_target_callback_blobs(emx_batch* b, emx_batch_log_prob_blobs_fn fn, void* user, int32_t nblobs);
typedef struct emx_fused_batch_data_launch {
    uint32_t abi;
    uint32_t args_bytes;
    int32_t ndim, movesel, grid, threads;
    uint64_t lds_bytes;
    void* hip_stream;
    const void* args;
    const void* user;
    int32_t nblobs;
    int32_t reserved;
    const int64_t* ndata;
} emx_fused_batch_data_launch;
typedef int (*emx_fused_batch_data_fn)(const emx_fused_batch_data_launch*);
int emx_set_batch_target_fused_data(emx_batch* b, emx_fused_batch_data_fn fn, int32_t ndim_compiled, const void* user_dev,
                                    const int64_t* ndata_host);
int emx_check_batch_blobs(int64_t nwalkers, int32_t ndim, int32_t target, int32_t nmoves, const emx_move_desc* moves, int32_t nblobs,
                          char* msg, int32_t msglen);
int emx_get_blobs_batch(emx_batch* b, double* out, int32_t* nblobs_out);
int emx_batch_set_moves(emx_batch* b, int32_t nmoves, const emx_move_desc* moves, const double* cdf);
int emx_batch_set_move_scale(emx_batch* b, int32_t move, const double* scale, int32_t n);
int emx_batch_get_move(emx_batch* b, int32_t move, emx_move_desc* out);
int emx_batch_set_philox(emx_batch* b, const uint64_t* seeds, uint64_t step);
int emx_batch_get_philox(emx_batch* b, uint64_t* seeds, uint64_t* step);
int emx_batch_set_state(emx_batch* b, const double* coords, const double* log_prob);
int emx_batch_get_state(emx_batch* b, double* coords, double* log_prob);
int emx_batch_eval_state_log_prob(emx_batch* b);
int emx_batch_chain_config(emx_batch* b, int64_t capacity);
int emx_batch_run(emx_batch* b, int64_t nsteps, int32_t thin_by, int32_t store);
int emx_batch_iteration(emx_batch* b, int64_t* stored, int64_t* proposals);
// ... 68 lines not shown
```

Before: 3.380 billion.

## Carry walker rows in registers across persistent stretch half-steps via arranged plans

Adds a 'carry' form of the persistent stretch kernel. The planner reorders each step's split-0 walker order so that walkers a wave just updated in the previous half-step land on the same wave. The kernel then keeps those rows and log-probs in registers instead of reloading them from global memory, and skips the version checks. A separate arrange kernel, with lookahead precompute for the next batch fused into the plan launch, builds the keep masks and permuted positions. This costs extra planning work, prefix scans and more register and LDS pressure, and it only applies to Philox, even N/D, non-store runs.

New measurement: 3.440 billion (median of 6 runs). 1.02x the previous value.

```diff
diff --git a/emcee_amd/_lib.py b/emcee_amd/_lib.py
--- a/emcee_amd/_lib.py
+++ b/emcee_amd/_lib.py
@@ -173,6 +173,9 @@
     "emx_mtdev_debug": (C.c_int, [_P, C.c_int32, C.c_int64, C.c_void_p, C.c_int64]),
     "emx_mtdev_tok_stats": (C.c_int, [_P, C.POINTER(C.c_int64)]),
     "emx_persist_local_launches": (C.c_int, [_P, C.POINTER(C.c_int64)]),
+    "emx_persist_carry_launches": (C.c_int, [_P, C.POINTER(C.c_int64)]),
+    "emx_plan_arrange": (C.c_int, [C.c_uint64, C.c_uint64, C.c_int32, C.c_int64, C.c_double, C.c_void_p, C.c_void_p, C.c_void_p, C.c_void_p,
+                                   C.c_void_p]),
     "emx_host_mt_jump": (C.c_int, [_u32p, C.c_uint64, C.c_int32, _u32p]),
     "emx_host_persist_shape": (C.c_int, [C.c_int64, C.c_int32, C.c_int32, C.POINTER(C.c_int32), C.POINTER(C.c_int32)]),
     "emx_timer_start": (C.c_int, [_P]),
diff --git a/emcee_amd/csrc/emx.hip b/emcee_amd/csrc/emx.hip
--- a/emcee_amd/csrc/emx.hip
+++ b/emcee_amd/csrc/emx.hip
@@ -361,10 +361,20 @@
     int64_t tune_mt_device_min_regen = 786432;
     int64_t tune_mt_regen_min = 16384;
     int64_t pipe_regen_steps = 0;
+    int64_t tune_persist_carry = 1;
+    int64_t persist_carry_launches = 0;
+    bool plan_tail_ok = false;
+    uint64_t plan_tail_step = 0, plan_tail_seed = 0;
+    int32_t* arr_scr[2] = {nullptr, nullptr};
+    int arr_cur = 0;
+    bool pre_valid = false;
+    uint64_t pre_first = 0, pre_seed = 0;
+    int pre_nb = 0;
     int64_t tune_persist_odd = 1;
     int64_t tune_persist_slab_skew = 1;
     int64_t tune_persist_slab_local_max = 4096;
     int64_t call_steps = 1;
+    bool call_store = false;
     int64_t tune_persist_exact = 1;
     int64_t tune_persist_valu = 1;
     int64_t tune_persist_local_max = 8192;
@@ -382,6 +392,7 @@
     struct Prepared {
         int move, S, slot;
         bool lean;
+        bool arranged;
         int gcol;
         uint64_t step;
         NativeArgs nat;
@@ -395,6 +406,7 @@
         int move = 0, S = 2, slot = 0;
         bool store = false;
         bool native = false;
+        bool arranged = false;
         bool lean = false;
         bool devplan = false;
         int gcol = 0;
@@ -529,6 +541,7 @@
     for (auto it = c->prepared.rbegin(); it != c->prepared.rend(); ++it)
         if (it->move < (int)c->moves.size() && c->moves[it->move].kind == EMX_MOVE_GAUSS) c->moves[it->move].gammas = it->cursor_before;
     c->prepared.clear();
+    c->plan_tail_ok = false;
 }
 
 #define FAIL(ctx, code, ...)                         \
@@ -1358,6 +1371,8 @@
     if (c->persist_bar) hipFree(c->persist_bar);
     if (c->persist_started) hipHostFree(c->persist_started);
     if (c->persist_ver) hipFree(c->persist_ver);
+    for (int q = 0; q < 2; ++q)
+        if (c->arr_scr[q]) hipFree(c->arr_scr[q]);
     if (c->d_desc) hipFree(c->d_desc);
     if (c->d_ctr) hipFree(c->d_ctr);
     if (c->h_ctr) hipHostFree(c->h_ctr);
@@ -1566,6 +1581,11 @@
     if (!strcmp(key, "mt_regen_min_walkers")) {
         PIPE_STOP(c);
         c->tune_mt_regen_min = v < 0 ? 0 : v;
+        return 0;
+    }
+    if (!strcmp(key, "persist_carry")) {
+        NEED(c, v == 0 || v == 1, "tuning persist_carry: 0 or 1");
+        c->tune_persist_carry = v;
         return 0;
     }
     if (!strcmp(key, "persist_rows_late")) {
@@ -2723,6 +2743,7 @@
     return step_begin_impl(c, store, move_index, nullptr, S_out);
 }
 
+static bool persist_carry_plans(const emx_ctx* c);
 static int native_prepare_batch(emx_ctx* c, uint64_t first_step, int nb, int forced_move, hipStream_t st) {
     const int nm = (int)c->moves.size();
     NativeBatchArgs B{};
@@ -2772,11 +2793,38 @@
         B.move[b] = m.kind;
         B.S[b] = m.nsplits;
     }
-    if (only_stretch && B.lean && !B.ablate && !B.desc)
-        hipLaunchKernelGGL(k_native_plan_batch_stretch, dim3((unsigned)((c->N + 255) / 256), (unsigned)nb), dim3(256), 0, st, B);
-    else
+    if (only_stretch && B.lean && !B.ablate && !B.desc) {
+        bool all_two = true;
+        for (int b = 0; b < nb; ++b) all_two = all_two && B.S[b] == 2;
+        const int64_t n0 = c->N / 2;
+        unsigned extra = 0;
+        if (nb > 1 && all_two && persist_carry_plans(c) && st == c->stream && (n0 + 255) / 256 <= PLAN_ARRANGE_MAX_BLOCKS) {
+            B.arrange = 1;
+            B.arr0 = (c->plan_tail_ok && c->plan_tail_seed == c->ph_seed && c->plan_tail_step + 1 == first_step) ? 1 : 0;
+            if (B.arr0) B.kprev0 = make_perm_key((uint64_t)c->N, c->ph_seed, first_step - 1);
+            for (int b = 0; b < nb; ++b) c->prepared[c->prepared.size() - (size_t)nb + (size_t)b].arranged = b > 0 || B.arr0;
+            const size_t words = (size_t)plan_arrange_words(c->N) * NATIVE_BATCH_MAX;
+            for (int q = 0; q < 2; ++q)
+                if (!c->arr_scr[q]) HIPOK(c, hipMalloc((void**)&c->arr_scr[q], words * sizeof(int32_t)));
+            B.arr_scr = c->arr_scr[c->arr_cur];
+            const bool foreseen = B.arr0 && c->pre_valid && c->pre_first == first_step && c->pre_seed == c->ph_seed && c->pre_nb == nb;
+            if (!foreseen) hipLaunchKernelGGL(k_plan_arrange, dim3((unsigned)((n0 + 255) / 256), (unsigned)nb), dim3(256), 0, st, B);
+            B.pre_scr = c->arr_scr[c->arr_cur ^ 1];
+            for (int k = 0; k <= nb; ++k) B.set_pre_key(k, make_perm_key((uint64_t)c->N, c->ph_seed, first_step + (uint64_t)nb - 1 + (uint64_t)k));
+            c->pre_valid = true;
+            c->pre_first = first_step + (uint64_t)nb;
+            c->pre_seed = c->ph_seed;
+            c->pre_nb = nb;
+            c->arr_cur ^= 1;
+            extra = (unsigned)((n0 + 255) / 256);
+        }
+        hipLaunchKernelGGL(k_native_plan_batch_stretch, dim3((unsigned)((c->N + 255) / 256) + extra, (unsigned)nb), dim3(256), 0, st, B);
+    } else
         hipLaunchKernelGGL(k_native_plan_batch, dim3((unsigned)((c->N + 255) / 256), (unsigned)nb), dim3(256), 0, st, B);
     HIPOK(c, hipGetLastError());
+    c->plan_tail_ok = nb > 0 && B.move[nb - 1] == EMX_MOVE_STRETCH && B.S[nb - 1] == 2;
+    c->plan_tail_step = first_step + (uint64_t)nb - 1;
+    c->plan_tail_seed = c->ph_seed;
     return 0;
 }
 
@@ -2787,6 +2835,7 @@
     auto& cur = c->cur;
     cur.store = store != 0;
     cur.native = false;
+    cur.arranged = false;
     cur.devplan = false;
     const int nm = (int)c->moves.size();
     const bool devp = forced_move < 0 && mtdev_eligible(c);
@@ -2860,6 +2909,7 @@
         cur.S = pr.S;
         cur.native = true;
         cur.lean = pr.lean;
+        cur.arranged = pr.arranged;
         cur.gcol = pr.gcol;
         cur.nat = pr.nat;
         cur.slot = pr.slot;
@@ -2912,6 +2962,7 @@
     hipLaunchKernelGGL(k_native_plan_batch, dim3((unsigned)((c->N + 255) / 256), 1u), dim3(256), 0, c->stream, B);
     HIPOK(c, hipGetLastError());
     cur.lean = false;
+    cur.arranged = false;
     return 0;
 }
 
@@ -3684,6 +3735,12 @@
     return sh.G == 8 && sh.V == 2 && sh.CH == (dpb == 1 ? 1 : dpb == 2 ? 2 : 4);
 }
 
+static bool persist_carry_plans(const emx_ctx* c) {
+    if (!c->tune_persist_carry || c->call_store) return false;
+    if (c->rng_mode != EMX_RNG_PHILOX || (c->N & 1) || (c->D & 1) || c->Dp > 64 || !persist_wanted(c)) return false;
+    return persist_shape(c, 2) != 0;
+}
+
 static bool persist_valu_wanted(const emx_ctx* c) {
     if (!c->tune_persist || !c->tune_persist_local || !c->tune_persist_valu) return false;
     if (!(c->rng_mode == EMX_RNG_PHILOX || persist_exact_ok(c)) || c->world != 1 || c->comm || c->sendbuf || c->peers_ready || c->moves.empty()) return false;
@@ -3845,6 +3902,7 @@
     int launch_S = 2;
     bool launch_local = false;
     bool launch_mix = false;
+    bool carry_ok = true;
     double launch_gammas = 0.0;
     int batches_touched = (!mtmode && !c->prepared.empty() && c->prepared.front().step == c->ph_step) ? 1 : 0;
     while (i0 + steps < total) {
@@ -3886,6 +3944,7 @@
         int mvi, S;
         int rc = emx_step_begin(c, st, &mvi, &S);
         if (rc) return rc;
+        if (steps > 0 && !(c->cur.native && c->cur.arranged)) carry_ok = false;
         if (launch_move < 0) {
             launch_move = c->moves[mvi].kind;
             launch_gammas = c->moves[mvi].gammas;
@@ -4009,7 +4068,9 @@
         } else if (c->D & 1) {
             e = launch_persist_dense_odd(c->Dp / 16, launch_move, launch_local ? 1 : 0, grid, block, lds, c->stream, P);
         } else {
-            e = launch_hot_persist_dense(c->Dp / 16, launch_move, launch_local ? 1 : 0, rows_late ? 1 : 0, grid, block, lds, c->stream, P);
+            const bool carry = c->tune_persist_carry && carry_ok && !mtmode && !store && !launch_local && launch_move == EMX_MOVE_STRETCH && launch_S == 2;
+            if (carry) c->persist_carry_launches++;
+            e = launch_hot_persist_dense(c->Dp / 16, launch_move, launch_local ? 1 : 0, carry ? 2 : rows_late ? 1 : 0, grid, block, lds, c->stream, P);
         }
         if (launch_local) c->persist_local_launches++;
         if (e != hipSuccess) FAIL(c, -2, "persistent half-step launch failed: %s", hipGetErrorString(e));
@@ -4215,12 +4276,48 @@
     return 0;
 }
 
+int emx_persist_carry_launches(emx_ctx* c, int64_t* n) {
+    *n = c->persist_carry_launches;
+    return 0;
+}
+
+int emx_plan_arrange(uint64_t seed, uint64_t step, int32_t has_prev, int64_t nwalkers, double a, int32_t* order, int32_t* p0, double* s0,
+                     double* uacc, int32_t* keep_mask) {
+    if (nwalkers < 2 || (nwalkers & 1) || nwalkers > (1ll << 30) || !order || !p0 || !s0 || !uacc || !keep_mask) return -1;
+    if (has_prev && step == 0) return -1;
+    const int64_t N = nwalkers, n0 = N / 2;
+    NativeArgs na{};
+    na.seed = seed;
+    na.step = step;
+    na.pk = make_perm_key((uint64_t)N, seed, step);
+    std::vector<int32_t> pos_of((size_t)n0);
+    if (has_prev) {
+        plan_arrange_host(N, make_perm_key((uint64_t)N, seed, step - 1), na.pk, pos_of.data(), keep_mask);
+    } else {
+        for (int64_t s = 0; s < n0; ++s) pos_of[(size_t)s] = (int32_t)s;
+        for (int64_t tl = 0; tl < (n0 + 15) / 16; ++tl) keep_mask[tl] = 0;
+    }
+    for (int64_t pos = 0; pos < N; ++pos) {
+        const int split = pos < n0 ? 0 : 1;
+        const int t = split ? (int)(pos - n0) : pos_of[(size_t)pos];
+        int i, a0, a1, a2;
+        double z, u;
+        native_slot<MOVE_STRETCH>(na, (int)N, 2, split, t, a, 0.0, 0.0, i, a0, a1, a2, z, u);
+        order[pos] = i;
+        p0[pos] = a0;
+        s0[pos] = z;
+        uacc[pos] = u;
+    }
+    return 0;
+}
+
 int emx_run(emx_ctx* c, int64_t nsteps, int32_t thin_by, int32_t store) {
     HIPOK(c, hipSetDevice(c->device));
     NEED(c, thin_by >= 1, "Invalid thinning argument");
     NEED(c, !c->cur.active, "emx_run: a step begun with emx_step_begin is still open");
     const int64_t total = nsteps * thin_by;
     c->call_steps = total;
+    c->call_store = store != 0;
     const bool devp = mtdev_eligible(c);
     if (c->mtdev && !devp) {
         const int rcm = mtdev_stop(c);
@@ -5262,6 +5359,11 @@
         case 7: *ptr = c->dbg; *nbytes = c->dbg ? c->dbg_blocks * 16 * 8 : 0; return 0;
         case 8: *ptr = c->my_flags; *nbytes = c->my_flags ? EMX_MAX_PEERS * 8 : 0; return 0;
     }
+    if (which >= 16 && which < 16 + PLAN_RING) {
+        *ptr = c->ring[which - 16].order;
+        *nbytes = c->ring[which - 16].order ? c->N * 48 : 0;
+        return 0;
+    }
     FAIL(c, -1, "unknown device pointer id %d", which);
 }
 
diff --git a/emcee_amd/csrc/emx_hot.hip b/emcee_amd/csrc/emx_hot.hip
--- a/emcee_amd/csrc/emx_hot.hip
+++ b/emcee_amd/csrc/emx_hot.hip
@@ -9,9 +9,9 @@
     return launch_one<8, 2, 4, MOVE_STRETCH, 4, 1>(grid, block, lds, st, a);
 }
 
-template <int G, int V, int CH, int DPB, int MOVE, bool LOCAL = false, bool ROWS_LATE = false>
+template <int G, int V, int CH, int DPB, int MOVE, bool LOCAL = false, bool ROWS_LATE = false, bool CARRY = false>
 static hipError_t launch_persist(dim3 grid, dim3 block, size_t lds, hipStream_t st, const PersistArgs& P) {
-    auto kern = k_persist<G, V, CH, DPB, MOVE, LOCAL, ROWS_LATE>;
+    auto kern = k_persist<G, V, CH, DPB, MOVE, LOCAL, ROWS_LATE, CARRY>;
     static size_t lds_granted[MAX_DEVICES] = {};
     int dev = 0;
     if (lds > 48 * 1024 && hipGetDevice(&dev) == hipSuccess && dev >= 0 && dev < MAX_DEVICES && lds > lds_granted[dev]) {
@@ -23,7 +23,16 @@
     return hipGetLastError();
 }
 
-hipError_t launch_hot_persist_dense(int dpb, int move, int local, int rows_late, dim3 grid, dim3 block, size_t lds, hipStream_t st, const PersistArgs& P) {
+hipError_t launch_hot_persist_dense(int dpb, int move, int local, int form, dim3 grid, dim3 block, size_t lds, hipStream_t st, const PersistArgs& P) {
+    const bool rows_late = form == 1;
+    if (form == 2) {
+        if (move != MOVE_STRETCH || local) return hipErrorInvalidValue;
+#define EMX_CCASE(b, ch) \
+    if (dpb == b) return launch_persist<8, 2, ch, b, MOVE_STRETCH, false, false, true>(grid, block, lds, st, P);
+        EMX_CCASE(1, 1) EMX_CCASE(2, 2) EMX_CCASE(3, 4) EMX_CCASE(4, 4)
+#undef EMX_CCASE
+        return hipErrorInvalidValue;
+    }
     if (rows_late && move == MOVE_STRETCH) {
 #define EMX_SCASE(b, ch)                                                                                       \
     if (dpb == b)                                                                                              \
diff --git a/emcee_amd/csrc/emx_kernels.hpp b/emcee_amd/csrc/emx_kernels.hpp
--- a/emcee_amd/csrc/emx_kernels.hpp
+++ b/emcee_amd/csrc/emx_kernels.hpp
@@ -1254,9 +1254,10 @@
     return ok_s != 0;
 }
 
-template <int G, int V, int CH, int DPB, int MOVE = MOVE_STRETCH, bool LOCAL = false, bool ROWS_LATE = false>
+template <int G, int V, int CH, int DPB, int MOVE = MOVE_STRETCH, bool LOCAL = false, bool ROWS_LATE = false, bool CARRY = false>
 static __global__ __launch_bounds__(512) void k_persist(const PersistArgs P) {
     static_assert(MOVE == MOVE_STRETCH || MOVE == MOVE_DE || MOVE == MOVE_SNOOKER, "the red / blue moves");
+    static_assert(!CARRY || (MOVE == MOVE_STRETCH && !LOCAL && !ROWS_LATE), "CARRY: the device-wide stretch form without stored rows");
     if (LOCAL && (blockIdx.x & 7u) != 0u) return;
     const unsigned bid = LOCAL ? blockIdx.x >> 3 : blockIdx.x, ngroups = LOCAL ? gridDim.x >> 3 : gridDim.x;
     constexpr int CPOL = EMX_CPOL_SC1;
@@ -1294,6 +1295,7 @@
     const int wave = (int)bid * (blockDim.x >> 6) + wib;
     const int t0 = wave * 16;
     unsigned long long pst[6] = {0, 0, 0, 0, 0, 0}, pt = 0;
+    unsigned long long pstb[2] = {0, 0};
     const bool prof = EMX_OPT_STAMPS && A.dbg && wib == EMX_STAMP_WAVE;
     if (prof) {
         pt = __builtin_readcyclecounter();
@@ -1373,7 +1375,14 @@
             my_i_n = J.order[pbase + myrow];
             my_logu_n = J.logu[pbase + myrow];
         }
-        if (prof) { asm volatile("s_waitcnt vmcnt(0)" ::: "memory"); }
+        unsigned keep_n = 0u;
+        if constexpr (CARRY) {
+            if (more && !pre) keep_n = (unsigned)J.p1[wave];
+        }
+        if (prof) {
+            asm volatile("s_waitcnt vmcnt(0)" ::: "memory");
+            if (n > 0) pstb[I.split == 0 ? 0 : 1] += __builtin_readcyclecounter() - pt;
+        }
         EMX_PSTAMP(0);
         Row<G, V, CH> qk[PF];
 #pragma unroll
@@ -1416,10 +1425,16 @@
             }
         }
         double my_lpo_n = 0.0;
-        if (!ROWS_LATE && more) {
+        if (!ROWS_LATE && !CARRY && more) {
 #pragma unroll
             for (int k = 0; k < PF; ++k) load_row_agent<G, V, CH, CPOL>(xi[k], Xr, wi_n[k], D, gl);
             my_lpo_n = load_agent(A.lp + my_i_n);
+        }
+        if (CARRY && more) {
+#pragma unroll
+            for (int k = 0; k < PF; ++k)
+                if (!((keep_n >> (k * WPW + sub)) & 1u)) load_row_agent<G, V, CH, CPOL>(xi[k], Xr, wi_n[k], D, gl);
+            if (!((keep_n >> myrow) & 1u)) my_lpo_n = load_agent(A.lp + my_i_n);
         }
         EMX_WAVE_SYNC();
         EMX_PSTAMP(1);
@@ -1452,11 +1467,13 @@
         if (prof) { asm volatile("s_nop 0" ::: "memory"); }
         EMX_PSTAMP(2);
         bool acc = false;
+        double lp_kept = my_lpo;
         if (mine) {
             const double lpn = -0.5 * my_qf;
             if (lpn != lpn) raise_status(A.status, ST_NAN_LOGP);
             const double lnpdiff = facS[myrow] + lpn - my_lpo;
             acc = lnpdiff > my_logu;
+            if (CARRY && acc) lp_kept = lpn;
             store_scope<LOCAL>(A.acc + my_i, (uint8_t)(acc ? 1 : 0));
             if (acc) {
                 store_scope<LOCAL>(A.lp + my_i, lpn);
@@ -1517,7 +1534,15 @@
         my_i = my_i_n;
         my_logu = my_logu_n;
         my_lpo = my_lpo_n;
-        if (!pre) {
+        if constexpr (CARRY) {
+#pragma unroll
+            for (int k = 0; k < PF; ++k) {
+                const int row = k * WPW + sub;
+                if (((keep_n >> row) & 1u) && ((am64 >> ((row & 3) * 16 + (row >> 2))) & 1ull)) xi[k] = qk[k];
+            }
+            if ((keep_n >> myrow) & 1u) my_lpo = lp_kept;
+        }
+        if (!CARRY && !pre) {
             unsigned vk[PF];
 #pragma unroll
             for (int k = 0; k < PF; ++k) vk[k] = load_agent(P.ver + wi[k]);
@@ -1538,6 +1563,8 @@
 #pragma unroll
         for (int k = 0; k < 6; ++k) o[k] = pst[k];
         o[6] = (unsigned long long)P.niter;
+        o[7] = pstb[0];
+        o[8] = pstb[1];
         o[12] = wall_clock64();
     }
 #undef EMX_PSTAMP
@@ -2605,12 +2632,153 @@
     int32_t lean;
     int32_t ablate;
     const StepDesc* desc;
+    int32_t arrange, arr0;
+    PermKey kprev0;
+    int32_t* arr_scr;
+    int32_t* pre_scr;
+    struct KeyWords {
+        uint32_t m1, c1, m2, c2, m3, c3, m1inv, m2inv, m3inv;
+    } pre_keys[NATIVE_BATCH_MAX + 1];
+    __host__ __device__ PermKey pre_key(int k) const {
+        PermKey K = nat[0].pk;
+        const KeyWords& w = pre_keys[k];
+        K.m1 = w.m1; K.c1 = w.c1; K.m2 = w.m2; K.c2 = w.c2; K.m3 = w.m3; K.c3 = w.c3;
+        K.m1inv = w.m1inv; K.m2inv = w.m2inv; K.m3inv = w.m3inv;
+        return K;
+    }
+    void set_pre_key(int k, const PermKey& K) { pre_keys[k] = KeyWords{K.m1, K.c1, K.m2, K.c2, K.m3, K.c3, K.m1inv, K.m2inv, K.m3inv}; }
 };
+static_assert(sizeof(NativeBatchArgs) <= 4096, "kernel arguments of the plan kernels");
+
+inline void plan_arrange_host(int64_t N, const PermKey& Kp, const PermKey& K, int32_t* pos_of, int32_t* keep_mask) {
+    const int64_t n0 = N / 2;
+    for (int64_t tl = 0; tl < (n0 + 15) / 16; ++tl) keep_mask[tl] = 0;
+    int64_t p = 0;
+    for (int64_t s = 0; s < n0; ++s) {
+        const uint32_t a = perm_inv((uint32_t)(2 * s + 1), Kp), pa = perm_fwd(a, K);
+        if (!(pa & 1u)) {
+            pos_of[s] = (int32_t)(pa >> 1);
+            keep_mask[s >> 4] |= 1 << (s & 15);
+        } else {
+            while (perm_fwd(perm_inv((uint32_t)(2 * p), K), Kp) & 1u) ++p;
+            pos_of[s] = (int32_t)p++;
+        }
+    }
+}
+
+__host__ __device__ inline int64_t plan_arrange_words(int64_t N) {
+    const int64_t n0 = N / 2;
+    return 2 * n0 + 2 * ((n0 + 255) / 256) + (n0 + 15) / 16;
+}
+static __device__ __forceinline__ void plan_arrange_block(int N, const PermKey& Kp, const PermKey& K, int32_t* scr, int bx) {
+    const int n0 = N / 2, nblk = (n0 + 255) / 256;
+    const int s = bx * 256 + threadIdx.x, lane = threadIdx.x & 63, wv = threadIdx.x >> 6;
+    bool keep = false, fill = false;
+    uint32_t pa = 0;
+    if (s < n0) {
+        pa = perm_fwd(perm_inv((uint32_t)(2 * s + 1), Kp), K);
+        keep = !(pa & 1u);
+        fill = !(perm_fwd(perm_inv((uint32_t)(2 * s), K), Kp) & 1u);
+    }
+    const bool hole = s < n0 && !keep;
+    const unsigned long long mh = __ballot(hole), mf = __ballot(fill), mk = __ballot(keep);
+    __shared__ int wh[4], wf[4];
+    if (lane == 0) {
+        wh[wv] = __popcll(mh);
+        wf[wv] = __popcll(mf);
+    }
+    __syncthreads();
+    int hb = 0, fb = 0;
+    for (int w = 0; w < wv; ++w) {
+        hb += wh[w];
+        fb += wf[w];
+    }
+    const unsigned long long below = (1ull << lane) - 1ull;
+    if (s < n0) scr[s] = keep ? (int32_t)(pa >> 1) : -1 - (hb + __popcll(mh & below));
+    if (fill) scr[n0 + bx * 256 + fb + __popcll(mf & below)] = s;
+    if (threadIdx.x == 0) {
+        scr[2 * n0 + 2 * bx] = wh[0] + wh[1] + wh[2] + wh[3];
+        scr[2 * n0 + 2 * bx + 1] = wf[0] + wf[1] + wf[2] + wf[3];
+    }
+    if ((lane & 15) == 0 && s < n0) scr[2 * n0 + 2 * nblk + (s >> 4)] = (int32_t)((mk >> lane) & 0xffffull);
+}
+static __global__ __launch_bounds__(256) void k_plan_arrange(const NativeBatchArgs B) {
+    const int b = blockIdx.y;
+    if (b == 0 && !B.arr0) return;
+    const PermKey K = B.nat[b].pk, Kp = b ? B.nat[b - 1].pk : B.kprev0;
+    plan_arrange_block(B.N, Kp, K, B.arr_scr + (size_t)b * plan_arrange_words(B.N), blockIdx.x);
+}
+constexpr int PLAN_ARRANGE_MAX_BLOCKS = 1024;
+
+static __device__ __forceinline__ int plan_arranged_pos(const NativeBatchArgs& B, int b, int pos) {
+    __shared__ int hpre[PLAN_ARRANGE_MAX_BLOCKS], fpre[PLAN_ARRANGE_MAX_BLOCKS], wth[4], wtf[4];
+    const int n0 = B.N / 2, nblk = (n0 + 255) / 256, E = (nblk + 255) / 256;
+    const int tid = threadIdx.x, lane = tid & 63, wv = tid >> 6;
+    const int32_t* scr = B.arr_scr + (size_t)b * plan_arrange_words(B.N);
+    int hs = 0, fs = 0;
+    for (int e = 0; e < E; ++e) {
+        const int k = tid * E + e;
+        if (k < nblk) {
+            hs += scr[2 * n0 + 2 * k];
+            fs += scr[2 * n0 + 2 * k + 1];
+        }
+    }
+    int hi = hs, fi = fs;
+    for (int d = 1; d < 64; d <<= 1) {
+        const int h2 = __shfl_up(hi, d), f2 = __shfl_up(fi, d);
+        if (lane >= d) {
+            hi += h2;
+            fi += f2;
+        }
+    }
+    if (lane == 63) {
+        wth[wv] = hi;
+        wtf[wv] = fi;
+    }
+    __syncthreads();
+    int hx = hi - hs, fx = fi - fs;
+    for (int w = 0; w < wv; ++w) {
+        hx += wth[w];
+        fx += wtf[w];
+    }
+    for (int e = 0; e < E; ++e) {
+        const int k = tid * E + e;
+        if (k < nblk) {
+            hpre[k] = hx;
+            fpre[k] = fx;
+            hx += scr[2 * n0 + 2 * k];
+            fx += scr[2 * n0 + 2 * k + 1];
+        }
+    }
+    __syncthreads();
+    if (pos >= n0) return -1;
+    if ((pos & 15) == 0) B.p1[b][pos >> 4] = scr[2 * n0 + 2 * nblk + (pos >> 4)];
+    int w = scr[pos];
+    if (w < 0) {
+        const int r = hpre[blockIdx.x] + (-1 - w);
+        int lo = 0, hi2 = nblk - 1;
+        while (lo < hi2) {
+            const int mid = (lo + hi2 + 1) >> 1;
+            if (fpre[mid] <= r) lo = mid; else hi2 = mid - 1;
+        }
+        w = scr[n0 + min(max(lo * 256 + (r - fpre[lo]), 0), n0 - 1)];
+    }
+    return w;
+}
 
 template <bool ONLY_STRETCH>
 static __device__ __forceinline__ void native_plan_batch_body(const NativeBatchArgs& B) {
     const int b = blockIdx.y;
     const int pos = blockIdx.x * blockDim.x + threadIdx.x;
+    int t_arr = -1;
+    if constexpr (ONLY_STRETCH) {
+        const int nplan = (B.N + 255) / 256;
+        if ((int)blockIdx.x >= nplan) {
+            if (B.pre_scr) plan_arrange_block(B.N, B.pre_key(b), B.pre_key(b + 1), B.pre_scr + (size_t)b * plan_arrange_words(B.N), (int)blockIdx.x - nplan);
+            return;
+        }
+        if (B.arrange && (b > 0 || B.arr0) && (int)(blockIdx.x * blockDim.x) < B.N / 2) t_arr = plan_arranged_pos(B, b, pos);
+    }
     if (pos >= B.N || (EMX_EXPERIMENTS && !ONLY_STRETCH && (B.ablate & 4))) return;
     const int N = B.N, S = B.S[b];
     int split = 0, t = pos;
@@ -2620,6 +2788,7 @@
         if (t < n) { split = s; break; }
         t -= n;
     }
+    if (ONLY_STRETCH && t_arr >= 0) t = t_arr;
     int i, a0, a1, a2;
     double z, u;
     const int mv = ONLY_STRETCH ? MOVE_STRETCH : B.move[b];
diff --git a/emcee_amd/csrc/emx_launch.hpp b/emcee_amd/csrc/emx_launch.hpp
--- a/emcee_amd/csrc/emx_launch.hpp
+++ b/emcee_amd/csrc/emx_launch.hpp
@@ -22,7 +22,7 @@
 }
 
 hipError_t launch_hot_stretch_dense64(int lean, dim3 grid, dim3 block, size_t lds, hipStream_t st, const HalfStepArgs& a);
-hipError_t launch_hot_persist_dense(int dpb, int move, int local, int rows_late, dim3 grid, dim3 block, size_t lds, hipStream_t st, const PersistArgs& P);
+hipError_t launch_hot_persist_dense(int dpb, int move, int local, int form, dim3 grid, dim3 block, size_t lds, hipStream_t st, const PersistArgs& P);
 hipError_t hot_persist_occupancy(int dpb, int move, int threads, size_t lds, int* per_cu);
 hipError_t launch_hot_persist_gauss(int dpb, dim3 grid, dim3 block, size_t lds, hipStream_t st, const PersistGaussArgs& P);
 hipError_t launch_persist_mix(int dpb, int local, dim3 grid, dim3 block, size_t lds, hipStream_t st, const PersistArgs& P);
diff --git a/emcee_amd/device.py b/emcee_amd/device.py
--- a/emcee_amd/device.py
+++ b/emcee_amd/device.py
@@ -654,8 +654,10 @@
         self._ck(self.lib.emx_persist_info(self.ctx, out))
         loc = C.c_int64(0)
         self._ck(self.lib.emx_persist_local_launches(self.ctx, C.byref(loc)))
+        car = C.c_int64(0)
+        self._ck(self.lib.emx_persist_carry_launches(self.ctx, C.byref(car)))
         return {"qualifies": bool(out[0]), "launches": int(out[1]), "halfsteps": int(out[2]), "recovered": int(out[3]),
-                "local_launches": int(loc.value)}
+                "local_launches": int(loc.value), "carry_launches": int(car.value)}
 
     def small_info(self):
         out = (C.c_int64 * 4)()
diff --git a/include/emx.h b/include/emx.h
--- a/include/emx.h
+++ b/include/emx.h
@@ -223,6 +223,9 @@
 
 int emx_persist_info(emx_ctx* ctx, int64_t out[4]);
 int emx_persist_local_launches(emx_ctx* ctx, int64_t* n);
+int emx_persist_carry_launches(emx_ctx* ctx, int64_t* n);
+int emx_plan_arrange(uint64_t seed, uint64_t step, int32_t has_prev, int64_t nwalkers, double a, int32_t* order, int32_t* p0, double* s0,
+                     double* uacc, int32_t* keep_mask);
 int emx_host_persist_shape(int64_t nwalkers, int32_t nsplits, int32_t num_cu, int32_t* waves_per_group, int32_t* groups);
 
 typedef struct emx_mt emx_mt;
```
